# MoseleyBioinformaticsLab/pdb_eda

Measured on AMD Instinct MI355X. Metric: Mvoxels/s blob-labelled, higher is better.
Workload: dtype f32; 1 GPU; configs[1]: 256^3 synthetic CCP4 grid (gaussian-filtered noise, sigma_filter 1.5 voxels), fused green/red blob labelling at +-(mean+1.5*std), per-blob fp64 stats + dense int32 labels of both signs, map resident in HBM; labels=True, entries_per_rank=1

## Files before the change

### pdb_eda_amd/csrc/pdbeda_hip.hip

```cpp
#include <hip/hip_runtime.h>
#include <fcntl.h>
#include <sys/mman.h>
#include <sys/stat.h>
#include <unistd.h>
#include <cerrno>

#include <algorithm>
#include <chrono>
#include <thread>
#include <atomic>
#include <random>
#include <climits>
#include <cmath>
#include <cstdarg>
#include <cstdio>
#include <cstring>
#include <condition_variable>
#include <deque>
#include <map>
#include <mutex>
#include <string>
#include <vector>

#include "pdbeda_kernels.h"
// ... 808 lines not shown
    if (e != hipSuccess || why) {
        arena_put(ctx, m->arena);
        delete m;
        return why ? fail(ctx, PDBEDA_ERR_ARGUMENT, "reading %s: %s", path, why) : fail(ctx, PDBEDA_ERR_DEVICE, "map upload from file: %s", hipGetErrorString(e));
    }
    if (with_stats) {
        range_apply(m, range);
        if (mean) *mean = host[0];
        if (std) *std = host[1];
    }
    ctx->live_handles++;
    *out = m;
    return PDBEDA_OK;
}

extern "C" int pdbeda_map_upload_file(pdbeda_ctx *ctx, const char *path, int64_t offset, int byteswap, const pdbeda_geometry *geom, pdbeda_map **out) {
    return upload_file_impl(ctx, path, offset, byteswap, geom, out, nullptr, nullptr);
}
extern "C" int pdbeda_map_upload_file_stats(pdbeda_ctx *ctx, const char *path, int64_t offset, int byteswap, const pdbeda_geometry *geom, pdbeda_map **out,
                                            double *mean, double *std) {
    return upload_file_impl(ctx, path, offset, byteswap, geom, out, mean, std);
}

extern "C" int pdbeda_map_combine(pdbeda_map *a, pdbeda_map *b, double alpha, pdbeda_map **out) {
    if (!a || !b || !out) return PDBEDA_ERR_ARGUMENT;
    *out = nullptr;
    pdbeda_ctx *ctx = a->ctx;
    if (b->ctx != ctx) return fail(ctx, PDBEDA_ERR_ARGUMENT, "maps of different contexts");
    if (a->n_vox != b->n_vox || memcmp(a->geom.ncrs, b->geom.ncrs, sizeof a->geom.ncrs) != 0)
        return fail(ctx, PDBEDA_ERR_ARGUMENT, "maps of different shapes");
    HIP_TRY(ctx, hipSetDevice(ctx->device));
    pdbeda_map *m = new pdbeda_map();
    m->ctx = ctx;
    m->geom = a->geom;
    m->n_vox = a->n_vox;
    float *d = nullptr;
    int rc = arena_carve(ctx, "map combine", &m->arena, [&](Carver &cv) { cv.take(m->geom_dev, 1); cv.take(d, (size_t)m->n_vox); });
    if (rc) { delete m; return rc; }
    hipError_t e = h2d_one(ctx, m->geom_dev, &m->geom, sizeof(Geom));
    if (e == hipSuccess) {
        hipLaunchKernelGGL(k_map_combine, dim3(grid_for(m->n_vox / 4 + 1, 256, 4096)), dim3(256), 0, ctx->stream, a->dens, b->dens, alpha, m->n_vox, d);
        e = hipGetLastError();
    }
    if (e == hipSuccess) e = ctx_sync(ctx);
    if (e != hipSuccess) {
        arena_put(ctx, m->arena);
        delete m;
        return fail(ctx, PDBEDA_ERR_DEVICE, "map combine: %s", hipGetErrorString(e));
    }
    m->dens = d;
    m->own_dens = true;
    ctx->live_handles++;
    *out = m;
    return PDBEDA_OK;
}

extern "C" int pdbeda_map_download(pdbeda_map *m, float *density_out) {
    if (!m || !density_out) return PDBEDA_ERR_ARGUMENT;
    pdbeda_ctx *ctx = m->ctx;
    HIP_TRY(ctx, hipSetDevice(ctx->device));
    HIP_TRY(ctx, d2h(ctx, density_out, m->dens, sizeof(float) * (size_t)m->n_vox));
    HIP_TRY(ctx, ctx_sync(ctx));
    return PDBEDA_OK;
}

extern "C" int pdbeda_map_free(pdbeda_map *m) {
    if (!m) return PDBEDA_ERR_ARGUMENT;
    pdbeda_ctx *ctx = m->ctx;
    arena_put(ctx, m->arena);
    ctx->live_handles--;
    delete m;
    return PDBEDA_OK;
}

static int reduce_launch(pdbeda_map *m, int mode, const double *mean_dev, double cutoff, double scale, int take_sqrt, double *out_dev) {
    pdbeda_ctx *ctx = m->ctx;
    hipLaunchKernelGGL(k_reduce_partials, dim3(N_PARTIAL), dim3(256), 0, ctx->stream, m->dens, m->n_vox, mode, mean_dev, cutoff, ctx->partials);
    hipLaunchKernelGGL(k_reduce_final, dim3(1), dim3(256), 0, ctx->stream, ctx->partials, N_PARTIAL, scale, take_sqrt, out_dev);
    HIP_TRY(ctx, hipGetLastError());
    return 0;
}

static int range_enqueue(pdbeda_map *m, double *range_host ) {
    pdbeda_ctx *ctx = m->ctx;
    double *res = ctx->partials + 2 * N_PARTIAL + 4;
    { PROF(ctx, "k_range_partials"); hipLaunchKernelGGL(k_range_partials, dim3(N_PARTIAL), dim3(256), 0, ctx->stream, m->dens, m->n_vox, ctx->partials, ctx->partials + N_PARTIAL); }
    hipLaunchKernelGGL(k_range_final, dim3(1), dim3(256), 0, ctx->stream, ctx->partials, ctx->partials + N_PARTIAL, N_PARTIAL, res);
    HIP_TRY(ctx, hipGetLastError());
    if (range_host) HIP_TRY(ctx, d2h(ctx, range_host, res, 2 * sizeof(double)));
    return 0;
}
static void range_apply(pdbeda_map *m, const double range[2]) {
    if (!std::isfinite(range[0]) || !std::isfinite(range[1])) { m->fix_refused = true; return; }
    const double bound = std::max(range[0], 4194304.0 * range[1]);
    int S = 40;
    if (bound > 0.0 && std::isfinite(bound)) {
        int e = 0;
        (void)frexp(bound, &e);
        S = 61 - e;
    }
    S = std::max(-900, std::min(S, 900));
    m->fix_mul = ldexp(1.0, S);
}
static int map_fix_mul(pdbeda_map *m) {
    pdbeda_ctx *ctx = m->ctx;
    if (m->fix_mul == 0.0 && !m->fix_refused) {
        double range[2] = {0.0, 0.0};
        const int rc = range_enqueue(m, range);
        if (rc) return rc;
        HIP_TRY(ctx, ctx_sync(ctx));
        range_apply(m, range);
    }
    if (m->fix_refused) return fail(ctx, PDBEDA_ERR_ARGUMENT, "the map holds non-finite density values: blob sums are undefined");
    return 0;
}

extern "C" int pdbeda_map_invalidate(pdbeda_map *m) {
    if (!m) return PDBEDA_ERR_ARGUMENT;
    m->fix_mul = 0.0;
    m->fix_refused = false;
    return PDBEDA_OK;
}

static int stats_enqueue(pdbeda_map *m, double *chunk_sums, double host[2], double range[2], bool want_range, bool with_geom) {
    pdbeda_ctx *ctx = m->ctx;
    double *res = ctx->partials + 2 * N_PARTIAL;
    const int64_t n_full = m->n_vox / NP_CHUNK;
    const int64_t n_chunks = std::max<int64_t>(n_full, 1);
    hipStream_t st = ctx->stream;
    double *host_out = nullptr;
    if (want_range && copy_kernels()) host_out = reinterpret_cast<double *>(pinned_take(ctx, 6 * sizeof(double)));
    if (host_out) {
        pinned_deliver(ctx, (char *)host_out, host, 2 * sizeof(double));
        pinned_deliver(ctx, (char *)(host_out + 4), range, 2 * sizeof(double));
    }
    double *r_sum = want_range ? chunk_sums + n_chunks : nullptr, *r_max = want_range ? chunk_sums + 2 * n_chunks : nullptr;
    for (int mode = 0; mode < 2; ++mode) {
        const bool with_range = want_range && mode == 0;
        if (n_full > 0) { PROF(ctx, "k_np_chunk_sums"); hipLaunchKernelGGL(k_np_chunk_sums, dim3((unsigned)std::min<int64_t>(n_full, 1 << 16)), dim3(256), 0, st, m->dens, n_full, mode, res, chunk_sums,
                                                                           with_range ? r_sum : (double *)nullptr, with_range ? r_max : (double *)nullptr,
                                                                           m->geom, with_geom && mode == 0 ? m->geom_dev : (Geom *)nullptr); }
        { PROF(ctx, "k_np_final"); hipLaunchKernelGGL(k_np_final, dim3(1), dim3(256), 0, st, m->dens, m->n_vox, n_full, mode, res, chunk_sums, mode, res + mode,
                                                      with_range && n_full > 0 ? r_sum : (const double *)nullptr, with_range && n_full > 0 ? r_max : (const double *)nullptr,
                                                      with_range ? res + 4 : (double *)nullptr, want_range && mode == 1 ? res + 4 : (const double *)nullptr, mode == 1 ? host_out : (double *)nullptr); }
    }
    HIP_TRY(ctx, hipGetLastError());
    if (host_out) return 0;
    if (!want_range) {
        HIP_TRY(ctx, d2h(ctx, host, res, 2 * sizeof(double)));
        return 0;
    }
    if (char *stage = pinned_take(ctx, 6 * sizeof(double))) {
        HIP_TRY(ctx, stage_copy(ctx, stage, res, 6 * sizeof(double), false));
        pinned_deliver(ctx, stage, host, 2 * sizeof(double));
        pinned_deliver(ctx, stage + 4 * sizeof(double), range, 2 * sizeof(double));
        return 0;
    }
    HIP_TRY(ctx, d2h(ctx, host, res, 2 * sizeof(double)));
    HIP_TRY(ctx, d2h(ctx, range, res + 4, 2 * sizeof(double)));
    return 0;
}

extern "C" int pdbeda_map_stats(pdbeda_map *m, double *mean, double *std) {
    if (!m) return PDBEDA_ERR_ARGUMENT;
    pdbeda_ctx *ctx = m->ctx;
    HIP_TRY(ctx, hipSetDevice(ctx->device));
    const int64_t n_full = m->n_vox / NP_CHUNK;
    double host[2], range[2] = {0.0, 0.0};
    const bool want_range = m->fix_mul == 0.0 && !m->fix_refused;
    int rc = with_scratch(ctx, 24 * (size_t)std::max<int64_t>(n_full, 1), [&](char *base) -> int {
        return stats_enqueue(m, reinterpret_cast<double *>(base), host, range, want_range);
    });
    if (rc) return rc;
    if (want_range) range_apply(m, range);
    if (mean) *mean = host[0];
    if (std) *std = host[1];
    return PDBEDA_OK;
}

extern "C" int pdbeda_sum_of_abs(pdbeda_map *m, float cutoff, double *out) {
    if (!m || !out) return PDBEDA_ERR_ARGUMENT;
    pdbeda_ctx *ctx = m->ctx;
    HIP_TRY(ctx, hipSetDevice(ctx->device));
    double *res = ctx->partials + N_PARTIAL + 2;
    int rc = reduce_launch(m, 2, nullptr, (double)cutoff, 1.0, 0, res);
    if (rc) return rc;
    HIP_TRY(ctx, d2h(ctx, out, res, sizeof(double)));
    HIP_TRY(ctx, ctx_sync(ctx));
    return PDBEDA_OK;
}

extern "C" int pdbeda_abs_select_hist(pdbeda_map *a, pdbeda_map *b, double alpha, double cut_a, double cut_b, int which, int shift,
                                      unsigned long long prefix, unsigned long long prefix_mask, uint32_t *hist) {
    if (!a || !hist || shift < 0 || shift > 48 || (which != 0 && which != 1) || (which == 1 && !b)) return PDBEDA_ERR_ARGUMENT;
    pdbeda_ctx *ctx = a->ctx;
    if (b && (b->ctx != ctx || b->n_vox != a->n_vox || memcmp(a->geom.ncrs, b->geom.ncrs, sizeof a->geom.ncrs) != 0))
        return fail(ctx, PDBEDA_ERR_ARGUMENT, "maps of different contexts or shapes");
    HIP_TRY(ctx, hipSetDevice(ctx->device));
    const int64_t n = (int64_t)a->geom.unique_ncrs[0] * a->geom.unique_ncrs[1] * a->geom.unique_ncrs[2];
    return with_scratch(ctx, 65536 * sizeof(uint32_t), [&](char *base) -> int {
        unsigned int *d_hist = reinterpret_cast<unsigned int *>(base);
        HIP_TRY(ctx, hipMemsetAsync(d_hist, 0, 65536 * sizeof(uint32_t), ctx->stream));
        hipLaunchKernelGGL(k_abs_select_hist, dim3(grid_for(n, 256, 4096)), dim3(256), 0, ctx->stream, a->geom_dev, a->dens, b ? b->dens : nullptr,
                           alpha, cut_a, cut_b, which, shift, prefix, prefix_mask, d_hist);
        HIP_TRY(ctx, hipGetLastError());
        HIP_TRY(ctx, d2h(ctx, hist, d_hist, 65536 * sizeof(uint32_t)));
        return 0;
    });
}

extern "C" int pdbeda_point_density(pdbeda_map *m, const int32_t *crs, int64_t n, double *out) {
    if (!m || (n > 0 && (!crs || !out)) || n < 0) return PDBEDA_ERR_ARGUMENT;
    if (n == 0) return PDBEDA_OK;
    pdbeda_ctx *ctx = m->ctx;
    HIP_TRY(ctx, hipSetDevice(ctx->device));
    int32_t *d_crs = nullptr;
    double *d_out = nullptr;
    return with_scratch(ctx, "point density", [&](Carver &cv) { cv.take(d_crs, 3 * n); cv.take(d_out, n); }, [&]() -> int {
        const int32_t *in = pinned_in(ctx, crs, (size_t)(3 * n));
        if (!in) { HIP_TRY(ctx, h2d_one(ctx, d_crs, crs, (size_t)(12 * n))); in = d_crs; }
        double *res = pinned_out(ctx, out, (size_t)n);
        hipLaunchKernelGGL(k_point_density, dim3(grid_for(n, 256)), dim3(256), 0, ctx->stream, m->geom_dev, m->dens, in, n, res ? res : d_out, (uint8_t *)nullptr);
        if (!res) HIP_TRY(ctx, d2h(ctx, out, d_out, 8 * n));
        return 0;
    });
}

extern "C" int pdbeda_valid_crs(pdbeda_map *m, const int32_t *crs, int64_t n, uint8_t *out) {
    if (!m || (n > 0 && (!crs || !out)) || n < 0) return PDBEDA_ERR_ARGUMENT;
    if (n == 0) return PDBEDA_OK;
    pdbeda_ctx *ctx = m->ctx;
    HIP_TRY(ctx, hipSetDevice(ctx->device));
    int32_t *d_crs = nullptr;
    uint8_t *d_out = nullptr;
    return with_scratch(ctx, "valid crs", [&](Carver &cv) { cv.take(d_crs, 3 * n); cv.take(d_out, n); }, [&]() -> int {
        const int32_t *in = pinned_in(ctx, crs, (size_t)(3 * n));
        if (!in) { HIP_TRY(ctx, h2d_one(ctx, d_crs, crs, (size_t)(12 * n))); in = d_crs; }
        uint8_t *res = pinned_out(ctx, out, (size_t)n);
        hipLaunchKernelGGL(k_point_density, dim3(grid_for(n, 256)), dim3(256), 0, ctx->stream, m->geom_dev, m->dens, in, n, (double *)nullptr, res ? res : d_out);
        if (!res) HIP_TRY(ctx, d2h(ctx, out, d_out, n));
        return 0;
    });
}

extern "C" int pdbeda_crs2xyz(pdbeda_map *m, const int32_t *crs, int64_t n, double *xyz) {
    if (!m || (n > 0 && (!crs || !xyz)) || n < 0) return PDBEDA_ERR_ARGUMENT;
    if (n == 0) return PDBEDA_OK;
    pdbeda_ctx *ctx = m->ctx;
    HIP_TRY(ctx, hipSetDevice(ctx->device));
    int32_t *d_crs = nullptr;
    double *d_xyz = nullptr;
    return with_scratch(ctx, "crs2xyz", [&](Carver &cv) { cv.take(d_crs, 3 * n); cv.take(d_xyz, 3 * n); }, [&]() -> int {
        const int32_t *in = pinned_in(ctx, crs, (size_t)(3 * n));
        if (!in) { HIP_TRY(ctx, h2d_one(ctx, d_crs, crs, (size_t)(12 * n))); in = d_crs; }
        double *res = pinned_out(ctx, xyz, (size_t)(3 * n));
        hipLaunchKernelGGL(k_crs2xyz, dim3(grid_for(n, 256)), dim3(256), 0, ctx->stream, m->geom_dev, in, n, res ? res : d_xyz);
        if (!res) HIP_TRY(ctx, d2h(ctx, xyz, d_xyz, 24 * n));
        return 0;
    });
}

extern "C" int pdbeda_xyz2crs(pdbeda_map *m, const double *xyz, int64_t n, int32_t *crs) {
    if (!m || (n > 0 && (!crs || !xyz)) || n < 0) return PDBEDA_ERR_ARGUMENT;
    if (n == 0) return PDBEDA_OK;
    pdbeda_ctx *ctx = m->ctx;
    HIP_TRY(ctx, hipSetDevice(ctx->device));
    double *d_xyz = nullptr;
    int32_t *d_crs = nullptr;
    return with_scratch(ctx, "xyz2crs", [&](Carver &cv) { cv.take(d_xyz, 3 * n); cv.take(d_crs, 3 * n); }, [&]() -> int {
        const double *in = pinned_in(ctx, xyz, (size_t)(3 * n));
        if (!in) { HIP_TRY(ctx, h2d_one(ctx, d_xyz, xyz, (size_t)(24 * n))); in = d_xyz; }
        int32_t *res = pinned_out(ctx, crs, (size_t)(3 * n));
        hipLaunchKernelGGL(k_xyz2crs, dim3(grid_for(n, 256)), dim3(256), 0, ctx->stream, m->geom_dev, in, n, res ? res : d_crs);
        if (!res) HIP_TRY(ctx, d2h(ctx, crs, d_crs, 12 * n));
        return 0;
    });
}

static void job_carve(Job &job, Carver &cv, int n_vols, int64_t total_words, int64_t total_keys, int64_t max_runs,
                        int64_t max_blobs, size_t extra_labels, int32_t **labels_out, int64_t n_tiles = 0, int64_t max_comps = -1) {
    if (max_comps < 0) max_comps = max_runs;
    job.run_cap = (uint32_t)max_runs; job.comp_cap = (uint32_t)max_comps; job.blob_cap = (uint32_t)std::min<int64_t>(max_blobs, 0xffffffffll);
    job.n_vols = n_vols;
    job.total_words = total_words;
    job.key_words = (total_keys + 63) / 64;
    job.n_fine = (int32_t)((job.key_words + KEY_FINE - 1) / KEY_FINE);
    job.fine_shift = 4;
    while (((int64_t)KEY_GROUPS << job.fine_shift) < job.n_fine) job.fine_shift++;
    job.fine_per_group = 1 << job.fine_shift;
    job.n_groups = (job.n_fine + job.fine_per_group - 1) / job.fine_per_group;
    job.vols = cv.take<VolDesc>(std::max(n_vols, 1));
    job.ctr = cv.take<Counters>(1);
    job.mask = cv.take<uint64_t>(total_words);
    job.key_bits = cv.take<uint64_t>((size_t)(job.key_words + KEY_FINE - 1) / KEY_FINE * KEY_FINE);
    job.n_fine_alloc = (int32_t)((job.n_fine + job.fine_per_group - 1) / job.fine_per_group * job.fine_per_group);
    job.fine_count = cv.take<uint32_t>((size_t)std::max(job.n_fine_alloc / 2, 8));
    job.mid_count = cv.take<uint32_t>((size_t)(job.key_words + KEY_FINE - 1) / KEY_FINE * (KEY_FINE / 16));
    job.group_count = (n_tiles && job.fine_shift > 4) ? cv.take<uint32_t>(KEY_GROUPS) : nullptr;
    job.run_base = cv.take<uint32_t>(total_words);
    job.comps_are_runs = n_tiles ? 0 : 1;
    job.comp_of_run = n_tiles ? cv.take<uint32_t>(max_runs) : nullptr;
    job.label_of_comp = n_tiles ? cv.take<int32_t>(max_comps) : nullptr;
    job.word_comps = n_tiles ? cv.take<uint8_t>((size_t)n_tiles * 2 * 256 * 8) : nullptr;
    job.unit_done = n_tiles ? cv.take<uint32_t>((size_t)n_tiles) : nullptr;
    job.unit_flag = n_tiles ? cv.take<uint32_t>(4) : nullptr;
    job.tile_mode = n_tiles ? cv.take<uint8_t>(n_tiles) : nullptr;
    job.tile_runs = n_tiles ? cv.take<uint32_t>(n_tiles) : nullptr;
    job.root_mask = n_tiles ? cv.take<uint64_t>((size_t)n_tiles * 4) : nullptr;
    job.n_tiles = (int32_t)n_tiles;
    if (n_tiles) {
        const int64_t nt = n_tiles, nfc = job.n_fine_alloc / 2, nmid = (job.key_words + KEY_FINE - 1) / KEY_FINE * (KEY_FINE / 16);
        job.clear_bits = (int32_t)((job.key_words + nt - 1) / nt);
        job.clear_fine = (int32_t)((nfc + nt - 1) / nt);
        job.clear_mid = (int32_t)((nmid + nt - 1) / nt);
    }
    job.inbox = n_tiles ? cv.take<InboxEntry>((size_t)n_tiles * INBOX_CAP) : nullptr;
    job.inbox_count = n_tiles ? cv.take<uint32_t>((size_t)n_tiles * INBOX_STRIDE) : nullptr;
    job.vol_sign[0] = job.vol_sign[1] = 1;
    job.parent = cv.take<int32_t>(max_comps);
    job.kpar = n_tiles ? cv.take<unsigned long long>(max_comps) : nullptr;
    job.r_n = cv.take<uint32_t>(max_comps);
    job.r_sum = cv.take<long long>((size_t)7 * max_comps);
    job.r_sum_stride = max_comps;
    job.r_c = cv.take<long long>(max_comps);
    job.r_r = cv.take<long long>(max_comps);
    job.r_s = cv.take<long long>(max_comps);
    job.r_key = cv.take<unsigned long long>(max_comps);
    job.r_rank = cv.take<uint32_t>(max_comps);
    job.b_n = cv.take<int64_t>(max_blobs);
    job.b_key = cv.take<int64_t>(max_blobs);
    job.b_total = cv.take<double>(max_blobs);
    job.b_centroid = cv.take<double>(3 * max_blobs);
    job.b_center = cv.take<double>(3 * max_blobs);
    job.b_volume = cv.take<double>(max_blobs);
    job.b_group = cv.take<int32_t>(max_blobs);
    int32_t *lab = extra_labels ? cv.take<int32_t>(extra_labels) : nullptr;
    if (labels_out) *labels_out = lab;
}

static int engine_enqueue(pdbeda_ctx *ctx, pdbeda_map *m, Job &job, int64_t max_runs, bool labelled = false, bool unordered = false) {
    hipStream_t st = ctx->stream;
    const unsigned run_grid = grid_for(max_runs, 256, 2048);
    if (job.total_words > 0 && !labelled) {
        {
            PROF(ctx, "k_run_index");
            static const int force_wpb = [] { const char *e = getenv("PDBEDA_RUNINDEX_WPB"); return e ? atoi(e) : 0; }();
            if (force_wpb != 256 && (force_wpb == 64 || (job.total_words < 256ll * 2048 && job.total_words > 64ll * job.n_vols))) hipLaunchKernelGGL(k_run_index<64>, dim3(grid_for(job.total_words, 64, 1ll << 30)), dim3(256), 0, st, job, m->dens, m->geom_dev);
            else hipLaunchKernelGGL(k_run_index<256>, dim3(grid_for(job.total_words, 256, 1ll << 30)), dim3(256), 0, st, job, m->dens, m->geom_dev);
        }
        { PROF(ctx, "k_union"); hipLaunchKernelGGL(k_union, dim3(grid_for(job.total_words * 4, 256, 1ll << 30)), dim3(256), 0, st, job); }
        { PROF(ctx, "k_resolve"); hipLaunchKernelGGL(k_resolve, dim3(run_grid), dim3(256), 0, st, job, unordered ? 1 : 0); }
        if (!unordered) { PROF(ctx, "k_paint_keys"); hipLaunchKernelGGL(k_paint_keys, dim3(run_grid), dim3(256), 0, st, job); }
    }
    if (!unordered) { PROF(ctx, "k_emit"); hipLaunchKernelGGL(k_emit, dim3(job.total_words > 0 ? std::min(run_grid, 512u) : 1u), dim3(256), 0, st, job, m->geom_dev); }
    HIP_TRY(ctx, hipGetLastError());
    return 0;
}

static pdbeda_bloblist *new_list(pdbeda_ctx *ctx, pdbeda_map *m) {
    pdbeda_bloblist *bl = new pdbeda_bloblist();
    bl->ctx = ctx;
    bl->map = m;
    ctx->live_handles++;
    return bl;
}

template <int CW>
static void launch_tile_label(pdbeda_ctx *ctx, unsigned n_tiles, const Job &job, const float *dens, const Geom *geom_dev, const TileDims &td,
                              const JobInit &init, int pair_slots) {
    { PROF(ctx, "k_tile_label"); hipLaunchKernelGGL((k_tile_label<CW>), dim3(td.ctiles, td.rtiles, td.stiles), dim3(512), 0, ctx->stream, job, dens, geom_dev, td, init); }
    {
        PROF(ctx, "k_face_merge");
        if (td.ctiles > 1) hipLaunchKernelGGL((k_face_merge<CW, FM_THREADS_WIDE>), dim3(td.ctiles, td.rtiles, td.stiles), dim3(FM_THREADS_WIDE), 0, ctx->stream, job, dens, geom_dev, td, pair_slots);
        else hipLaunchKernelGGL((k_face_merge<CW, FM_THREADS>), dim3(td.ctiles, td.rtiles, td.stiles), dim3(FM_THREADS), 0, ctx->stream, job, dens, geom_dev, td, pair_slots);
    }
    if (job.unit_form) {
        { PROF(ctx, "k_unit_label"); hipLaunchKernelGGL((k_unit_label<CW>), dim3(td.ctiles, td.rtiles, td.stiles), dim3(512), 0, ctx->stream, job, dens, geom_dev, td); }
        { PROF(ctx, "k_unit_pairs"); hipLaunchKernelGGL((k_unit_pairs<CW>), dim3(td.ctiles, td.rtiles, td.stiles), dim3(512), 0, ctx->stream, job, td); }
    }
}

template <bool FUSED>
static void launch_labels(pdbeda_ctx *ctx, const Job &job, const TileDims &td, int32_t *labels_dev, const Geom *geom_dev) {
    switch (td.cw) {
        case 1: hipLaunchKernelGGL((k_labels_tiles<1, FUSED>), dim3(td.ctiles, td.rtiles, td.stiles), dim3(PDBEDA_LABELS_NT_THREADS), 0, ctx->stream, job, td, labels_dev, geom_dev); break;
        case 2: hipLaunchKernelGGL((k_labels_tiles<2, FUSED>), dim3(td.ctiles, td.rtiles, td.stiles), dim3(PDBEDA_LABELS_NT_THREADS), 0, ctx->stream, job, td, labels_dev, geom_dev); break;
        case 3: hipLaunchKernelGGL((k_labels_tiles<3, FUSED>), dim3(td.ctiles, td.rtiles, td.stiles), dim3(PDBEDA_LABELS_NT_THREADS), 0, ctx->stream, job, td, labels_dev, geom_dev); break;
        default: hipLaunchKernelGGL((k_labels_tiles<4, FUSED>), dim3(td.ctiles, td.rtiles, td.stiles), dim3(PDBEDA_LABELS_NT_THREADS), 0, ctx->stream, job, td, labels_dev, geom_dev); break;
    }
}

struct WholeMapJob {
    Job job;
    Arena arena;
    TileDims td;
    int32_t *labels_dev = nullptr;
    bool labels = false;
    size_t bytes = 0;
};
static int whole_map_enqueue(pdbeda_map *m, float cut_pos, float cut_neg, bool want_pos, bool want_neg, uint32_t flags, int tier, int unit_form, WholeMapJob *out) {
    pdbeda_ctx *ctx = m->ctx;
    HIP_TRY(ctx, hipSetDevice(ctx->device));
    const Geom &g = m->geom;
    const int n_planes = (want_pos ? 1 : 0) + (want_neg ? 1 : 0);
    const int uc = g.unique_ncrs[0], ur = g.unique_ncrs[1], us = g.unique_ncrs[2];
    const int row_words = (uc + 63) / 64;
    const int64_t words_pp = (int64_t)row_words * ur * us;
    const int64_t keys_pp = (int64_t)uc * ur * us;
    const int64_t total_words = words_pp * n_planes, total_keys = keys_pp * n_planes;
    const int64_t worst_blobs = (int64_t)((uc + 1) / 2) * ((ur + 1) / 2) * ((us + 1) / 2) * n_planes + 1;
    const bool labels = (flags & PDBEDA_FLAG_LABELS) != 0;
    const size_t lab_elems = labels ? (size_t)keys_pp : 0;

    TileDims td;
    td.ctiles = (row_words + 3) / 4;
    td.cw = (row_words + td.ctiles - 1) / td.ctiles;
    td.rtiles = (ur + TILE_R - 1) / TILE_R;
    td.stiles = (us + TILE_S - 1) / TILE_S;
    td.n_planes = n_planes;
    td.uc = uc; td.ur = ur; td.us = us; td.row_words = row_words;
    td.nc = g.ncrs[0]; td.nr = g.ncrs[1];
    td.cut[0] = want_pos ? cut_pos : cut_neg;
    td.sign[0] = want_pos ? 1 : -1;
    td.cut[1] = cut_neg;
    td.sign[1] = -1;
    const int64_t tiles_pp = (int64_t)td.ctiles * td.rtiles * td.stiles;
    if (tiles_pp >= (1ll << 31) || keys_pp >= (1ll << 31)) return fail(ctx, PDBEDA_ERR_ARGUMENT, "grid too large");
    if (td.rtiles > 65535 || td.stiles > 65535) return fail(ctx, PDBEDA_ERR_ARGUMENT, "grid too large");
    const int64_t tile_runs = tiles_pp * td.cw * 64 * 32, tile_comps = tiles_pp * CCAP;
    const int64_t worst_unit = (int64_t)((uc + 1) / 2) * ur * us * n_planes + 1;
    if (tile_runs + worst_unit >= (1ll << 31))
        return fail(ctx, PDBEDA_ERR_ARGUMENT, "grid too large for whole-map labelling: %d x %d x %d voxels need %lld run ids (limit 2^31: about 1100^3 for a fused job)",
                    uc, ur, us, (long long)(tile_runs + worst_unit));
    const int64_t unit_ids = tier == 0 ? std::min<int64_t>(worst_unit, std::max<int64_t>(65536, tile_runs / 4)) : worst_unit;
    const int64_t max_blobs = tier == 0 ? std::min<int64_t>(worst_blobs, std::max<int64_t>(4096, total_keys / 32)) : worst_blobs;
    const int64_t max_runs = tile_runs + unit_ids, max_comps = tile_comps + unit_ids;

    int rc_fix = map_fix_mul(m);
    if (rc_fix) return rc_fix;
    Job job;
    memset(&job, 0, sizeof job);
    job.fix_mul = m->fix_mul;
    size_t need = 0;
    Arena arena;
    int32_t *labels_dev = nullptr;
    int rc = arena_carve(ctx, "whole-map labelling", &arena, [&](Carver &cv) {
        job_carve(job, cv, n_planes, total_words, total_keys, max_runs, max_blobs, lab_elems, &labels_dev, tiles_pp, max_comps);
        need = cv.off;
    });
    if (rc) return rc;
    job.vol_sign[0] = td.sign[0];
    job.vol_sign[1] = td.sign[1];
    job.unit_form = unit_form;
    static std::atomic<uint32_t> g_epoch{[] {
        uint32_t seed;
        try { seed = (uint32_t)std::random_device{}(); }
        catch (...) { seed = (uint32_t)std::chrono::steady_clock::now().time_since_epoch().count() ^ ((uint32_t)getpid() * 2654435761u); }
        return seed | 1u;
    }()};
    do { job.epoch = g_epoch.fetch_add(1u); } while (job.epoch == 0u || job.epoch == 0xffffffffu);

    JobInit init;
    memset(&init, 0, sizeof init);
    for (int p = 0; p < n_planes; ++p) {
        VolDesc &v = init.v[p];
        v.dim[0] = uc; v.dim[1] = ur; v.dim[2] = us;
        v.org[0] = v.org[1] = v.org[2] = 0;
        v.row_words = row_words;
        v.group = p;
        v.word_base = words_pp * p;
        v.key_base = keys_pp * p;
    }
    init.runs0 = (unsigned)tile_runs;
    init.comps0 = (unsigned)tile_comps;
    hipStream_t st = ctx->stream;
    int pair_slots = PAIR_SLOTS;
    if (ctx->debug_edge_cap > 0) { pair_slots = 1; while (pair_slots * 2 <= std::min<int64_t>(ctx->debug_edge_cap, PAIR_SLOTS)) pair_slots *= 2; }
    switch (td.cw) {
        case 1: launch_tile_label<1>(ctx, (unsigned)tiles_pp, job, m->dens, m->geom_dev, td, init, pair_slots); break;
        case 2: launch_tile_label<2>(ctx, (unsigned)tiles_pp, job, m->dens, m->geom_dev, td, init, pair_slots); break;
        case 3: launch_tile_label<3>(ctx, (unsigned)tiles_pp, job, m->dens, m->geom_dev, td, init, pair_slots); break;
        default: launch_tile_label<4>(ctx, (unsigned)tiles_pp, job, m->dens, m->geom_dev, td, init, pair_slots); break;
    }
    { PROF(ctx, "k_resolve_tiles"); hipLaunchKernelGGL(k_resolve_tiles, dim3((unsigned)tiles_pp + 64u), dim3(256), 0, st, job, (int)tiles_pp); }
    if (job.group_count) { PROF(ctx, "k_group_counts"); hipLaunchKernelGGL(k_group_counts, dim3((unsigned)(job.n_groups + 255) / 256u), dim3(256), 0, st, job); }
    if (labels) {
        PROF(ctx, "k_labels_tiles");
        launch_labels<true>(ctx, job, td, labels_dev, m->geom_dev);
    } else {
        PROF(ctx, "k_emit_tiles");
        hipLaunchKernelGGL(k_emit_tiles, dim3(std::min<unsigned>(512u, ((unsigned)tiles_pp + 1u) / 2u)), dim3(256), 0, st, job, m->geom_dev);
    }
    hipError_t e = hipGetLastError();
    if (e != hipSuccess) { arena_put(ctx, arena); return fail(ctx, PDBEDA_ERR_DEVICE, "whole-map labelling launch: %s", hipGetErrorString(e)); }
    out->job = job; out->arena = arena; out->td = td; out->labels_dev = labels_dev; out->labels = labels; out->bytes = need;
    return PDBEDA_OK;
}

static int full_blobs_impl(pdbeda_map *m, float cut_pos, float cut_neg, bool want_pos, bool want_neg, uint32_t flags,
                           pdbeda_bloblist **out_pos, pdbeda_bloblist **out_neg) {
    pdbeda_ctx *ctx = m->ctx;
    WholeMapJob wj;
    const int tier = ctx->debug_worst_case_arena ? 1 : 0, form = tier;
    int rc = whole_map_enqueue(m, cut_pos, cut_neg, want_pos, want_neg, flags, tier, form, &wj);
    if (rc) return rc;
    const int n_planes = (want_pos ? 1 : 0) + (want_neg ? 1 : 0);
    pdbeda_bloblist *first = nullptr;
    for (int p = 0; p < n_planes; ++p) {
        pdbeda_bloblist *bl = new_list(ctx, m);
        bl->job = wj.job;
        bl->td = wj.td;
        bl->vol_lo = p;
        bl->vol_hi = p + 1;
        bl->whole_map = true;
        bl->sign = wj.td.sign[p];
        if (p == 0) { bl->arena = wj.arena; bl->owns_arena = true; first = bl; }
        else { bl->owns_arena = false; bl->sibling = first; first->sibling = bl; }
        bl->labels_dev = wj.labels_dev;
        bl->labels_done = wj.labels;
        bl->cut_pos = cut_pos; bl->cut_neg = cut_neg; bl->want_pos = want_pos; bl->want_neg = want_neg; bl->flags = flags; bl->tier = tier; bl->unit_form = form;
        bl->job_bytes = wj.bytes;
        if (bl->sign > 0) *out_pos = bl; else *out_neg = bl;
    }
    return PDBEDA_OK;
}

extern "C" int pdbeda_full_blobs(pdbeda_map *m, float cutoff, uint32_t flags, pdbeda_bloblist **out) {
    if (!m || !out) return PDBEDA_ERR_ARGUMENT;
    *out = nullptr;
    if (cutoff == 0.0f || cutoff != cutoff) return fail(m->ctx, PDBEDA_ERR_ARGUMENT, "cutoff must be non-zero (the reference returns None)");
    pdbeda_bloblist *dummy = nullptr;
    if (cutoff > 0) return full_blobs_impl(m, cutoff, 0.0f, true, false, flags, out, &dummy);
    return full_blobs_impl(m, 0.0f, cutoff, false, true, flags, &dummy, out);
}

extern "C" int pdbeda_full_blobs_pm(pdbeda_map *m, float cutoff_pos, float cutoff_neg, uint32_t flags, pdbeda_bloblist **green,
                                    pdbeda_bloblist **red) {
    if (!m || !green || !red) return PDBEDA_ERR_ARGUMENT;
    *green = *red = nullptr;
    if (!(cutoff_pos > 0.0f) || !(cutoff_neg < 0.0f)) return fail(m->ctx, PDBEDA_ERR_ARGUMENT, "need cutoff_pos > 0 > cutoff_neg");
    return full_blobs_impl(m, cutoff_pos, cutoff_neg, true, true, flags, green, red);
}

static pdbeda_bloblist *owner_of(pdbeda_bloblist *bl) { return bl->owns_arena ? bl : bl->sibling; }
static const int64_t SPEC_ROWS = 2048;
static int list_resolve_counts(pdbeda_bloblist *bl) {
    if (bl->have_counts) return 0;
    pdbeda_ctx *ctx = bl->ctx;
    HIP_TRY(ctx, hipSetDevice(ctx->device));
    Counters ctr;
    auto fetch = [&]() -> int {
        pdbeda_bloblist *ow = bl->whole_map ? owner_of(bl) : nullptr;
        const int64_t g = ow ? std::min<int64_t>((int64_t)bl->job.blob_cap, SPEC_ROWS) : 0;
        if (g > 0) {
            const Job &job = bl->job;
            ow->spec_rows = 0;
            ow->spec_n.resize((size_t)g); ow->spec_key.resize((size_t)g); ow->spec_total.resize((size_t)g); ow->spec_centroid.resize(3 * (size_t)g);
            ow->spec_center.resize(3 * (size_t)g); ow->spec_volume.resize((size_t)g); ow->spec_group.resize((size_t)g);
            const D2HItem parts[8] = {{&ctr, job.ctr, sizeof ctr}, {ow->spec_n.data(), job.b_n, (size_t)(8 * g)}, {ow->spec_total.data(), job.b_total, (size_t)(8 * g)},
                                      {ow->spec_centroid.data(), job.b_centroid, (size_t)(24 * g)}, {ow->spec_center.data(), job.b_center, (size_t)(24 * g)},
                                      {ow->spec_volume.data(), job.b_volume, (size_t)(8 * g)}, {ow->spec_key.data(), job.b_key, (size_t)(8 * g)},
                                      {ow->spec_group.data(), job.b_group, (size_t)(4 * g)}};
            HIP_TRY(ctx, d2h_many(ctx, parts, 8));
            HIP_TRY(ctx, ctx_sync(ctx));
            ow->spec_rows = g;
            return 0;
        }
        HIP_TRY(ctx, d2h(ctx, &ctr, bl->job.ctr, sizeof ctr));
        HIP_TRY(ctx, ctx_sync(ctx));
        return 0;
    };
    {
        const int rc_fetch = fetch();
        if (rc_fetch) return rc_fetch;
    }
    while (bl->whole_map && ctr.overflow != 0u) {
        pdbeda_bloblist *ow = owner_of(bl);
        if (!ow) return fail(ctx, PDBEDA_ERR_STATE, "whole-map labelling: a list without its job");
        const int tier = 1, form = 1;
        if (tier == ow->tier && form == ow->unit_form) return fail(ctx, PDBEDA_ERR_STATE, "whole-map labelling overflowed its worst-case arena");
        if (ow->voxels_done || bl->voxels_done) return fail(ctx, PDBEDA_ERR_STATE, "whole-map labelling: overflow noticed after the voxel lists were made");
        WholeMapJob wj;
        arena_put(ctx, ow->arena);
        int rc = whole_map_enqueue(ow->map, ow->cut_pos, ow->cut_neg, ow->want_pos, ow->want_neg, ow->flags, tier, form, &wj);
        if (rc) { ow->arena.base = nullptr; ow->arena.cap = 0; return rc; }
        ow->arena = wj.arena;
        pdbeda_bloblist *both[2] = {ow, ow->sibling};
        for (pdbeda_bloblist *l : both) {
            if (!l) continue;
            l->job = wj.job; l->td = wj.td; l->labels_dev = wj.labels_dev; l->labels_done = wj.labels;
            l->tier = tier; l->unit_form = form; l->reruns += 1; l->have_counts = false; l->job_bytes = wj.bytes; l->spec_rows = 0;
        }
        const int rc_fetch = fetch();
        if (rc_fetch) return rc_fetch;
    }
    if (!bl->whole_map && ctr.unit_wait_failed) return fail(ctx, PDBEDA_ERR_DEVICE, "sphere batch: the device's volumes outgrew what the host sized the job for");
    if (bl->vol_lo == 0 && bl->vol_hi == bl->job.n_vols) { bl->rank_lo = 0; bl->rank_hi = ctr.n_blobs; }
    else if (bl->whole_map && bl->job.n_vols == 2 && bl->vol_hi == bl->vol_lo + 1) {
        bl->rank_lo = bl->vol_lo == 0 ? 0 : ctr.n_blobs_vol0;
        bl->rank_hi = bl->vol_lo == 0 ? ctr.n_blobs_vol0 : ctr.n_blobs;
    } else return fail(ctx, PDBEDA_ERR_STATE, "blob list covers an unexpected volume range");
    bl->job_blobs = ctr.n_blobs;
    bl->have_counts = true;
    if (bl->whole_map && bl->job.n_vols == 2) {
        pdbeda_bloblist *ow = owner_of(bl);
        pdbeda_bloblist *both[2] = {ow, ow ? ow->sibling : nullptr};
        for (pdbeda_bloblist *l : both) {
            if (!l || l == bl || l->freed || l->have_counts || l->job.ctr != bl->job.ctr || l->vol_hi != l->vol_lo + 1) continue;
            l->rank_lo = l->vol_lo == 0 ? 0 : ctr.n_blobs_vol0;
            l->rank_hi = l->vol_lo == 0 ? ctr.n_blobs_vol0 : ctr.n_blobs;
            l->job_blobs = ctr.n_blobs;
            l->have_counts = true;
        }
    }
    return 0;
}

extern "C" int pdbeda_bloblist_counters(pdbeda_bloblist *bl, int64_t *out) {
    if (!bl || bl->freed || !out) return PDBEDA_ERR_ARGUMENT;
    pdbeda_ctx *ctx = bl->ctx;
    HIP_TRY(ctx, hipSetDevice(ctx->device));
    Counters c;
    HIP_TRY(ctx, d2h(ctx, &c, bl->job.ctr, sizeof c));
    HIP_TRY(ctx, ctx_sync(ctx));
    out[0] = c.n_runs; out[1] = c.n_comps; out[2] = bl->reruns; out[3] = c.n_blobs;
    out[4] = out[5] = out[6] = 0;
    out[7] = (int64_t)(bl->job_bytes ? bl->job_bytes : owner_of(bl)->arena.cap);
    if (bl->whole_map && bl->job.tile_mode) {
        const int64_t n_tiles = (int64_t)bl->td.ctiles * bl->td.rtiles * bl->td.stiles;
        std::vector<uint8_t> mode(n_tiles);
        HIP_TRY(ctx, d2h(ctx, mode.data(), bl->job.tile_mode, n_tiles));
        HIP_TRY(ctx, ctx_sync(ctx));
        for (uint8_t v : mode) { if (v == 1) ++out[4]; else if (v == 2) ++out[5]; else if (v == 3) ++out[6]; }
    }
    return PDBEDA_OK;
}


extern "C" int64_t pdbeda_bloblist_count(pdbeda_bloblist *bl) {
    if (!bl || bl->freed) return PDBEDA_ERR_ARGUMENT;
    int rc = list_resolve_counts(bl);
    if (rc) return rc;
    return bl->rank_hi - bl->rank_lo;
}

extern "C" int pdbeda_bloblist_stats(pdbeda_bloblist *bl, int64_t *n, double *total_density, double *centroid, double *coord_center,
                                     double *volume, int64_t *first_key, int32_t *group) {
    if (!bl || bl->freed) return PDBEDA_ERR_ARGUMENT;
    int rc = list_resolve_counts(bl);
    if (rc) return rc;
    pdbeda_ctx *ctx = bl->ctx;
    const Job &job = bl->job;
    const int64_t lo = bl->rank_lo, cnt = bl->rank_hi - bl->rank_lo;
    if (cnt == 0) return PDBEDA_OK;
    if (bl->whole_map) {
        const pdbeda_bloblist *ow = owner_of(bl);
        if (ow && ow->spec_rows >= lo + cnt && ow->job.ctr == job.ctr) {
            if (n) memcpy(n, ow->spec_n.data() + lo, (size_t)(8 * cnt));
            if (total_density) memcpy(total_density, ow->spec_total.data() + lo, (size_t)(8 * cnt));
            if (centroid) memcpy(centroid, ow->spec_centroid.data() + 3 * lo, (size_t)(24 * cnt));
            if (coord_center) memcpy(coord_center, ow->spec_center.data() + 3 * lo, (size_t)(24 * cnt));
            if (volume) memcpy(volume, ow->spec_volume.data() + lo, (size_t)(8 * cnt));
            if (first_key) memcpy(first_key, ow->spec_key.data() + lo, (size_t)(8 * cnt));
            if (group) memcpy(group, ow->spec_group.data() + lo, (size_t)(4 * cnt));
            return PDBEDA_OK;
        }
    }
    const D2HItem columns[7] = {{n, job.b_n + lo, (size_t)(8 * cnt)}, {total_density, job.b_total + lo, (size_t)(8 * cnt)},
                                {centroid, job.b_centroid + 3 * lo, (size_t)(24 * cnt)}, {coord_center, job.b_center + 3 * lo, (size_t)(24 * cnt)},
                                {volume, job.b_volume + lo, (size_t)(8 * cnt)}, {first_key, job.b_key + lo, (size_t)(8 * cnt)},
                                {group, job.b_group + lo, (size_t)(4 * cnt)}};
    HIP_TRY(ctx, d2h_many(ctx, columns, 7));
    HIP_TRY(ctx, ctx_sync(ctx));
    return PDBEDA_OK;
}

static int list_stats_one_trip(pdbeda_bloblist *bl, int64_t guess, std::vector<int64_t> &n, std::vector<double> &tot, std::vector<double> &cen,
                               std::vector<int32_t> &grp, const D2HItem *extra = nullptr) {
    pdbeda_ctx *ctx = bl->ctx;
    const Job &job = bl->job;
    guess = std::min<int64_t>(guess, (int64_t)job.blob_cap);
    const bool whole_job = !bl->whole_map && bl->vol_lo == 0 && bl->vol_hi == job.n_vols;
    const int64_t extra_bytes = extra ? (int64_t)extra->bytes + 64 : 0;
    if (!bl->have_counts && whole_job && guess > 0 && 44 * guess + 4096 + extra_bytes < (int64_t)pinned_room(ctx)) {
        HIP_TRY(ctx, hipSetDevice(ctx->device));
        n.resize((size_t)guess); tot.resize((size_t)guess); cen.resize(3 * (size_t)guess); grp.resize((size_t)guess);
        Counters ctr;
        const D2HItem parts[6] = {{&ctr, job.ctr, sizeof ctr}, {n.data(), job.b_n, (size_t)(8 * guess)}, {tot.data(), job.b_total, (size_t)(8 * guess)},
                                  {cen.data(), job.b_centroid, (size_t)(24 * guess)}, {grp.data(), job.b_group, (size_t)(4 * guess)},
                                  extra ? *extra : D2HItem{nullptr, nullptr, 0}};
        HIP_TRY(ctx, d2h_many(ctx, parts, 6));
        HIP_TRY(ctx, ctx_sync(ctx));
        if (ctr.unit_wait_failed) return fail(ctx, PDBEDA_ERR_DEVICE, "sphere batch: the device's volumes outgrew what the host sized the job for");
        bl->rank_lo = 0; bl->rank_hi = ctr.n_blobs; bl->job_blobs = ctr.n_blobs; bl->have_counts = true;
        if ((int64_t)ctr.n_blobs <= guess) {
            const size_t nb = ctr.n_blobs;
            n.resize(nb); tot.resize(nb); cen.resize(3 * nb); grp.resize(nb);
            return PDBEDA_OK;
        }
        extra = nullptr;
    }
    if (extra && extra->dst && extra->bytes) HIP_TRY(ctx, d2h(ctx, extra->dst, extra->src, extra->bytes));
    const int64_t nb = pdbeda_bloblist_count(bl);
    if (nb < 0) return (int)nb;
    n.resize((size_t)nb); tot.resize((size_t)nb); cen.resize(3 * (size_t)nb); grp.resize((size_t)nb);
    return pdbeda_bloblist_stats(bl, n.data(), tot.data(), cen.data(), nullptr, nullptr, nullptr, grp.data());
}


static int list_materialise_voxels(pdbeda_bloblist *bl) {
    pdbeda_bloblist *ow = owner_of(bl);
    if (ow->voxels_done) return 0;
    pdbeda_ctx *ctx = bl->ctx;
    HIP_TRY(ctx, hipSetDevice(ctx->device));
    {
        const int rc_counts = list_resolve_counts(bl);
        if (rc_counts) return rc_counts;
        ow = owner_of(bl);
    }
    Job &job = ow->job;
    const int64_t nb = bl->job_blobs;
    const int64_t max_vox = job.key_words * 64;
    int rc = arena_carve(ctx, "voxel lists", &ow->vox_arena, [&](Carver &cv) {
        cv.take(ow->offsets_dev, nb + 1);
        cv.take(ow->cursor_dev, std::max<int64_t>(nb, 1));
        cv.take(ow->crs_dev, 3 * std::max<int64_t>(max_vox, 1));
    });
    if (rc) return rc;
    hipStream_t st = ctx->stream;
    hipLaunchKernelGGL(k_blob_offsets, dim3(1), dim3(1024), 0, st, job, ow->offsets_dev, ow->cursor_dev);
    if (job.total_words > 0)
        hipLaunchKernelGGL(k_voxel_lists, dim3(grid_for(job.total_words * 64, 256, 8192)), dim3(256), 0, st, job, ow->offsets_dev,
                           ow->cursor_dev, ow->crs_dev);
    HIP_TRY(ctx, hipGetLastError());
    ow->voxels_done = true;
    return 0;
}

extern "C" int64_t pdbeda_bloblist_num_voxels(pdbeda_bloblist *bl) {
    if (!bl || bl->freed) return PDBEDA_ERR_ARGUMENT;
    int rc = list_resolve_counts(bl);
    if (rc) return rc;
    if (bl->n_voxels >= 0) return bl->n_voxels;
    rc = list_materialise_voxels(bl);
    if (rc) return rc;
    pdbeda_ctx *ctx = bl->ctx;
    pdbeda_bloblist *ow = owner_of(bl);
    int64_t off[2] = {0, 0};
    HIP_TRY(ctx, d2h(ctx, &off[0], ow->offsets_dev + bl->rank_lo, 8));
    HIP_TRY(ctx, d2h(ctx, &off[1], ow->offsets_dev + bl->rank_hi, 8));
    HIP_TRY(ctx, ctx_sync(ctx));
    bl->n_voxels = off[1] - off[0];
    return bl->n_voxels;
}

extern "C" int pdbeda_bloblist_voxels(pdbeda_bloblist *bl, int32_t *crs, int64_t *blob_offsets) {
    if (!bl || bl->freed) return PDBEDA_ERR_ARGUMENT;
    int64_t nv = pdbeda_bloblist_num_voxels(bl);
    if (nv < 0) return (int)nv;
    pdbeda_ctx *ctx = bl->ctx;
    pdbeda_bloblist *ow = owner_of(bl);
    const int64_t cnt = bl->rank_hi - bl->rank_lo;
    std::vector<int64_t> off(cnt + 1);
    HIP_TRY(ctx, d2h(ctx, off.data(), ow->offsets_dev + bl->rank_lo, 8 * (cnt + 1))); HIP_TRY(ctx, ctx_sync(ctx));
    const int64_t base = off[0];
    if (blob_offsets)
        for (int64_t i = 0; i <= cnt; ++i) blob_offsets[i] = off[i] - base;
    if (crs && nv > 0) HIP_TRY(ctx, d2h(ctx, crs, ow->crs_dev + 3 * base, 12 * nv)); HIP_TRY(ctx, ctx_sync(ctx));
    return PDBEDA_OK;
}

static int list_moments_compute(pdbeda_bloblist *bl) {
    const int64_t nv = pdbeda_bloblist_num_voxels(bl);
    if (nv < 0) return (int)nv;
    pdbeda_ctx *ctx = bl->ctx;
    const int64_t cnt = bl->rank_hi - bl->rank_lo;
    if (cnt == 0 || nv == 0) { bl->shape_done = true; return PDBEDA_OK; }
    if (cnt >= (1ll << 31) || nv >= (1ll << 31)) return fail(ctx, PDBEDA_ERR_ARGUMENT, "blob moments: a list of 2^31 blobs or voxels, or more");
    if (!bl->whole_map && nv >= (1ll << 24)) return fail(ctx, PDBEDA_ERR_ARGUMENT, "blob moments: a sphere / list batch of 2^24 voxels or more");
    pdbeda_map *m = bl->map;
    HIP_TRY(ctx, hipSetDevice(ctx->device));
    if (int rc = map_fix_mul(m)) return rc;
    pdbeda_bloblist *ow = owner_of(bl);
    const size_t nb = (size_t)cnt;
    BlobShapeArgs a;
    unsigned long long *d_widest = nullptr;
    int32_t *d_i = nullptr;
    long long *d_l = nullptr;
// ... 1826 lines not shown
```

### pdb_eda_amd/csrc/pdbeda_kernels.h

```cpp
#pragma once
#include "pdbeda_device.h"

namespace pdbeda {

struct VolDesc {
    int32_t dim[3];
    int32_t org[3];
    int32_t row_words;
    int32_t group;
    int64_t word_base;
    int64_t key_base;
};

struct FixSums {
    long long rho, c_lo, c_hi, r_lo, r_hi, s_lo, s_hi;
};
__device__ inline long long fix_of(double v, double mul) { return __double2ll_rn(v * mul); }
__device__ inline void fix_limbs(__int128 v, long long &lo, long long &hi) {
    lo = (long long)(unsigned long long)((unsigned __int128)v & 0xffffffffu);
    hi = (long long)(v >> 32);
}
__device__ inline double fix_moment(long long lo, long long hi) { return (double)hi * 4294967296.0 + (double)lo; }
__device__ inline FixSums fix_sums(long long F, long long m_c, long long m_r, long long m_s, long long c0, long long r0, long long s0) {
    FixSums o;
    o.rho = F;
    fix_limbs((__int128)F * c0 + m_c, o.c_lo, o.c_hi);
    fix_limbs((__int128)F * r0 + m_r, o.r_lo, o.r_hi);
    fix_limbs((__int128)F * s0 + m_s, o.s_lo, o.s_hi);
    return o;
}
__device__ inline void fix_add(FixSums &a, const FixSums &b) {
    a.rho += b.rho; a.c_lo += b.c_lo; a.c_hi += b.c_hi; a.r_lo += b.r_lo; a.r_hi += b.r_hi; a.s_lo += b.s_lo; a.s_hi += b.s_hi;
}
__device__ inline void fix_atomic_add(FixSums *dst, const FixSums &v) {
    atomicAdd((unsigned long long *)&dst->rho, (unsigned long long)v.rho);
    atomicAdd((unsigned long long *)&dst->c_lo, (unsigned long long)v.c_lo);
    atomicAdd((unsigned long long *)&dst->c_hi, (unsigned long long)v.c_hi);
    atomicAdd((unsigned long long *)&dst->r_lo, (unsigned long long)v.r_lo);
    atomicAdd((unsigned long long *)&dst->r_hi, (unsigned long long)v.r_hi);
    atomicAdd((unsigned long long *)&dst->s_lo, (unsigned long long)v.s_lo);
    atomicAdd((unsigned long long *)&dst->s_hi, (unsigned long long)v.s_hi);
}
template <typename JobRef> __device__ inline FixSums fix_load(const JobRef &job, uint32_t i) {
    const long long *p = job.r_sum + i;
    const int64_t s = job.r_sum_stride;
    FixSums o;
    o.rho = p[0]; o.c_lo = p[s]; o.c_hi = p[2 * s]; o.r_lo = p[3 * s]; o.r_hi = p[4 * s]; o.s_lo = p[5 * s]; o.s_hi = p[6 * s];
    return o;
}
template <typename JobRef> __device__ inline void fix_store(const JobRef &job, uint32_t i, const FixSums &v) {
    long long *p = job.r_sum + i;
    const int64_t s = job.r_sum_stride;
    p[0] = v.rho; p[s] = v.c_lo; p[2 * s] = v.c_hi; p[3 * s] = v.r_lo; p[4 * s] = v.r_hi; p[5 * s] = v.s_lo; p[6 * s] = v.s_hi;
}
template <typename JobRef> __device__ inline void fix_fold(const JobRef &job, uint32_t i, const FixSums &v) {
    unsigned long long *p = (unsigned long long *)(job.r_sum + i);
    const int64_t s = job.r_sum_stride;
    atomicAdd(p, (unsigned long long)v.rho);
    atomicAdd(p + s, (unsigned long long)v.c_lo); atomicAdd(p + 2 * s, (unsigned long long)v.c_hi);
    atomicAdd(p + 3 * s, (unsigned long long)v.r_lo); atomicAdd(p + 4 * s, (unsigned long long)v.r_hi);
    atomicAdd(p + 5 * s, (unsigned long long)v.s_lo); atomicAdd(p + 6 * s, (unsigned long long)v.s_hi);
}
__device__ inline FixSums fix_zero() { FixSums z; z.rho = z.c_lo = z.c_hi = z.r_lo = z.r_hi = z.s_lo = z.s_hi = 0; return z; }

struct Counters {
    unsigned int n_runs;
    unsigned int n_comps;
    unsigned int n_blobs;
    unsigned int n_blobs_vol0;
    unsigned int unit_wait_failed;
    unsigned int unit_tiles[3];
    unsigned int overflow;
    unsigned long long n_voxels;
    long long total_words;
    long long total_keys;
};

struct Job {
    VolDesc *vols;
    int32_t n_vols;
    int64_t total_words;
    int64_t key_words;
    uint64_t *mask;
    uint32_t *run_base;
    uint64_t *key_bits;
    uint32_t *fine_count;
    int32_t n_fine, n_fine_alloc, fine_per_group;
    Counters *ctr;
    int32_t comps_are_runs;
    uint32_t *comp_of_run;
    int32_t *label_of_comp;
    uint8_t *word_comps;
    uint32_t *unit_done;
    uint32_t *unit_flag;
    uint32_t epoch;
    uint8_t *tile_mode;
    uint32_t *tile_runs;
    struct InboxEntry *inbox;
    uint32_t *inbox_count;
    int32_t vol_sign[2];
    int32_t *parent;
    uint32_t *r_n;
    long long *r_sum;
    int64_t r_sum_stride;
    double fix_mul;
    long long *r_c, *r_r, *r_s;
    unsigned long long *r_key;
    uint32_t *r_rank;
    int64_t *b_n, *b_key;
    double *b_total, *b_centroid, *b_center, *b_volume;
    int32_t *b_group;
    uint64_t *root_mask;
    int32_t n_tiles;
    unsigned long long *kpar;
    uint32_t *mid_count;
    int32_t fine_shift, n_groups;
    uint32_t run_cap, comp_cap, blob_cap;
    int32_t clear_bits, clear_fine, clear_mid;
    uint32_t *group_count;
    int32_t unit_form;
};

struct InboxEntry {
    uint32_t local, n;
    FixSums sum;
    unsigned long long c, r, s;
};
constexpr int INBOX_STRIDE = 32;
constexpr int INBOX_CAP = 192;

constexpr int TILE_COMPS = 256;
constexpr int KEY_FINE = 32;
constexpr int KEY_GROUPS = 1024;
constexpr int WAVE = 64;

__device__ inline int lane_id() { return threadIdx.x & 63; }

__device__ inline int find_vol(const VolDesc *vols, int n, int64_t word) {
    int lo = 0, hi = n - 1;
    while (lo < hi) {
        int mid = (lo + hi + 1) >> 1;
        if (vols[mid].word_base <= word) lo = mid; else hi = mid - 1;
    }
    return lo;
}
__device__ inline int find_vol_by_key(const VolDesc *vols, int n, int64_t key) {
    int lo = 0, hi = n - 1;
    while (lo < hi) {
        int mid = (lo + hi + 1) >> 1;
        if (vols[mid].key_base <= key) lo = mid; else hi = mid - 1;
    }
    return lo;
}


__device__ inline double wave_incl_scan(double x, int lane) {
#pragma unroll
    for (int d = 1; d < 64; d <<= 1) {
        double y = __shfl_up(x, d);
        if (lane >= d) x += y;
    }
    return x;
}

template <typename JobRef>
__device__ inline void word_run_records_of(const JobRef &job, const VolDesc &vd, uint64_t mw, int lane, double rho, int cl0, int rl, int sl,
                                           int rawc0, int rawr, int raws, uint32_t rec0);
template <typename JobRef>
__device__ inline void word_run_records(const JobRef &job, const Geom &g, const float *__restrict__ dens, const VolDesc &vd, uint64_t mw,
                                        int lane, int cl0, int rl, int sl, int rawc0, int rawr, int raws, uint32_t rec0) {
    const bool bit = (mw >> lane) & 1ull;
    const double rho = bit ? (double)fetch_wrapped(g, dens, rawc0 + lane, rawr, raws) : 0.0;
    word_run_records_of(job, vd, mw, lane, rho, cl0, rl, sl, rawc0, rawr, raws, rec0);
}
template <typename JobRef>
__device__ inline void word_run_records_of(const JobRef &job, const VolDesc &vd, uint64_t mw, int lane, double rho, int cl0, int rl, int sl,
                                           int rawc0, int rawr, int raws, uint32_t rec0) {
    const double rl_ = rho * (double)lane;
    const double p1 = wave_incl_scan(rho, lane);
    const double p2 = wave_incl_scan(rl_, lane);
    const uint64_t starts = run_starts(mw);
    const bool is_start = (starts >> lane) & 1ull;
    const int e = is_start ? run_end_of(mw, lane) : lane;
    const double p1e = __shfl(p1, e);
    const double p2e = __shfl(p2, e);
    if (is_start) {
        const int len = e - lane + 1;
        const double s_rho = p1e - (p1 - rho);
        const double s_rl = p2e - (p2 - rl_);
        const uint32_t idx = rec0 + (uint32_t)popc64(starts & bits_below(lane));
        job.parent[idx] = (int32_t)idx;
        job.r_n[idx] = (uint32_t)len;
        fix_store(job, idx, fix_sums(fix_of(s_rho, job.fix_mul), fix_of(s_rl, job.fix_mul), 0, 0, rawc0, rawr, raws));
        const long long a = (long long)rawc0 + lane;
        job.r_c[idx] = (long long)len * a + (long long)len * (len - 1) / 2;
        job.r_r[idx] = (long long)len * rawr;
        job.r_s[idx] = (long long)len * raws;
        const int64_t key_in = ((int64_t)(cl0 + lane) * vd.dim[1] + rl) * vd.dim[2] + sl;
        job.r_key[idx] = (unsigned long long)(vd.key_base + key_in);
        if (job.kpar) job.kpar[idx] = ((unsigned long long)(((uint32_t)vd.group << 31) | (uint32_t)key_in) << 32) | idx;
    }
}

constexpr int NARROW_ROW = 16;
template <typename JobRef>
__device__ inline void narrow_run_records(const JobRef &job, const Geom &g, const float *__restrict__ dens, const VolDesc &vd, uint64_t mw,
                                          int rl, int sl, uint32_t rec0) {
    const int rawc0 = vd.org[0], rawr = vd.org[1] + rl, raws = vd.org[2] + sl;
    float v[NARROW_ROW];
#pragma unroll
    for (int k = 0; k < NARROW_ROW; ++k) v[k] = ((mw >> k) & 1ull) ? fetch_wrapped(g, dens, rawc0 + k, rawr, raws) : 0.0f;
    uint64_t todo = run_starts(mw);
    uint32_t idx = rec0;
    while (todo) {
        const int a = ctz64(todo);
        todo &= todo - 1;
        const int b = run_end_of(mw, a), len = b - a + 1;
        double s_rho = 0.0, s_rl = 0.0;
#pragma unroll
        for (int k = 0; k < NARROW_ROW; ++k)
            if (k >= a && k <= b) { s_rho += (double)v[k]; s_rl += (double)v[k] * (double)k; }
        job.parent[idx] = (int32_t)idx;
        job.r_n[idx] = (uint32_t)len;
        fix_store(job, idx, fix_sums(fix_of(s_rho, job.fix_mul), fix_of(s_rl, job.fix_mul), 0, 0, rawc0, rawr, raws));
        const long long first = (long long)rawc0 + a;
        job.r_c[idx] = (long long)len * first + (long long)len * (len - 1) / 2;
        job.r_r[idx] = (long long)len * rawr;
        job.r_s[idx] = (long long)len * raws;
        const int64_t key_in = ((int64_t)a * vd.dim[1] + rl) * vd.dim[2] + sl;
        job.r_key[idx] = (unsigned long long)(vd.key_base + key_in);
        if (job.kpar) job.kpar[idx] = ((unsigned long long)(((uint32_t)vd.group << 31) | (uint32_t)key_in) << 32) | idx;
        ++idx;
    }
}

constexpr int SPARSE_BITS = 16;
template <typename JobRef>
__device__ inline void sparse_run_records(const JobRef &job, const Geom &g, const float *__restrict__ dens, const VolDesc &vd, uint64_t mw,
                                          int wq, int rl, int sl, uint32_t rec0) {
    const int rawc0 = vd.org[0] + wq * 64, rawr = vd.org[1] + rl, raws = vd.org[2] + sl;
    float v[SPARSE_BITS];
    int pos[SPARSE_BITS];
    {
        uint64_t t = mw;
#pragma unroll
        for (int k = 0; k < SPARSE_BITS; ++k) {
            const bool have = t != 0ull;
            pos[k] = have ? ctz64(t) : 64;
            v[k] = have ? fetch_wrapped(g, dens, rawc0 + pos[k], rawr, raws) : 0.0f;
            t &= t - 1ull;
        }
    }
    uint32_t idx = rec0;
    int first = -1, prev = -2;
    double s_rho = 0.0, s_rl = 0.0;
    auto flush = [&]() {
        const int len = prev - first + 1;
        job.parent[idx] = (int32_t)idx;
        job.r_n[idx] = (uint32_t)len;
        fix_store(job, idx, fix_sums(fix_of(s_rho, job.fix_mul), fix_of(s_rl, job.fix_mul), 0, 0, rawc0, rawr, raws));
        const long long a0 = (long long)rawc0 + first;
        job.r_c[idx] = (long long)len * a0 + (long long)len * (len - 1) / 2;
        job.r_r[idx] = (long long)len * rawr;
        job.r_s[idx] = (long long)len * raws;
        const int64_t key_in = ((int64_t)(wq * 64 + first) * vd.dim[1] + rl) * vd.dim[2] + sl;
        job.r_key[idx] = (unsigned long long)(vd.key_base + key_in);
        if (job.kpar) job.kpar[idx] = ((unsigned long long)(((uint32_t)vd.group << 31) | (uint32_t)key_in) << 32) | idx;
        ++idx;
    };
#pragma unroll
    for (int k = 0; k < SPARSE_BITS; ++k) {
        if (pos[k] < 64) {
            if (pos[k] != prev + 1) {
                if (first >= 0) flush();
                first = pos[k]; s_rho = 0.0; s_rl = 0.0;
            }
            s_rho += (double)v[k];
            s_rl += (double)v[k] * (double)pos[k];
            prev = pos[k];
        }
    }
    if (first >= 0) flush();
}

template <int WPB>
__global__ void __launch_bounds__(256) k_run_index(Job job, const float *__restrict__ dens, const Geom *__restrict__ gp) {
    static_assert(WPB == 256 || WPB == 64, "a word per thread of the block, or of its first wave");
    constexpr int SCAN_WAVES = WPB / 64, PER_WAVE = WPB / 4;
    __shared__ uint64_t s_mask[WPB];
    __shared__ uint32_t s_off[WPB];
    __shared__ VolDesc s_vd[WPB];
    __shared__ int s_row[WPB][3];
    __shared__ uint32_t s_wsum[4];
    __shared__ uint32_t s_base;
    const int tid = threadIdx.x, lane = tid & 63, wv = tid >> 6;
    const int64_t chunk0 = (int64_t)blockIdx.x * WPB;
    const int64_t w = chunk0 + tid;
    const bool mine = tid < WPB && w < job.total_words;
    const uint64_t m = mine ? job.mask[w] : 0ull;
    const uint32_t cnt = (uint32_t)popc64(run_starts(m));
    uint32_t x = cnt;
#pragma unroll
    for (int d = 1; d < 64; d <<= 1) {
        uint32_t y = __shfl_up(x, d);
        if (lane >= d) x += y;
    }
    if (lane == 63) s_wsum[wv] = x;
    if (tid < WPB) s_mask[tid] = m;
    __syncthreads();
    if (tid == 0) {
        uint32_t tot = 0;
        for (int k = 0; k < SCAN_WAVES; ++k) tot += s_wsum[k];
        s_base = tot ? atomicAdd(&job.ctr->n_runs, tot) : 0u;
    }
    __syncthreads();
    uint32_t wpre = 0;
    for (int k = 0; k < wv && k < SCAN_WAVES; ++k) wpre += s_wsum[k];
    const uint32_t off = s_base + wpre + x - cnt;
    if (mine) job.run_base[w] = off;
    VolDesc my_vd;
    int wq = 0, rl = 0, sl = 0;
    bool narrow = false, sparse = false;
    if (m != 0ull) {
        my_vd = job.vols[find_vol(job.vols, job.n_vols, w)];
        const int64_t rem = w - my_vd.word_base;
        wq = (int)(rem % my_vd.row_words);
        const int64_t row = rem / my_vd.row_words;
        rl = (int)(row % my_vd.dim[1]);
        sl = (int)(row / my_vd.dim[1]);
        narrow = my_vd.dim[0] <= NARROW_ROW;
        sparse = !narrow && popc64(m) <= SPARSE_BITS;
        if (narrow || sparse) s_mask[tid] = 0ull;
        else { s_off[tid] = off; s_vd[tid] = my_vd; s_row[tid][0] = wq; s_row[tid][1] = rl; s_row[tid][2] = sl; }
    }
    __syncthreads();

    const Geom &g = *gp;
    if (narrow) narrow_run_records(job, g, dens, my_vd, m, rl, sl, off);
    else if (sparse) sparse_run_records(job, g, dens, my_vd, m, wq, rl, sl, off);
    uint64_t todo = 0ull;
    {
        const bool live = lane < PER_WAVE && s_mask[wv * PER_WAVE + lane] != 0ull;
        todo = __ballot(live);
    }
    auto fetch = [&](int slot) -> double {
        const uint64_t mw = s_mask[slot];
        const VolDesc &vd = s_vd[slot];
        return ((mw >> lane) & 1ull) ? (double)fetch_wrapped(g, dens, vd.org[0] + s_row[slot][0] * 64 + lane, vd.org[1] + s_row[slot][1], vd.org[2] + s_row[slot][2]) : 0.0;
    };
    double rho_next = todo ? fetch(wv * PER_WAVE + ctz64(todo)) : 0.0;
    while (todo) {
        const int slot = wv * PER_WAVE + ctz64(todo);
        todo &= todo - 1;
        const double rho = rho_next;
        if (todo) rho_next = fetch(wv * PER_WAVE + ctz64(todo));
        const VolDesc &vd = s_vd[slot];
        const int q = s_row[slot][0], r = s_row[slot][1], t = s_row[slot][2];
        word_run_records_of(job, vd, s_mask[slot], lane, rho, q * 64, r, t, vd.org[0] + q * 64, vd.org[1] + r, vd.org[2] + t, s_off[slot]);
    }
}

__device__ inline int uf_load(const int32_t *p, int x) {
    return __hip_atomic_load(p + x, __ATOMIC_RELAXED, __HIP_MEMORY_SCOPE_WORKGROUP);
}
__device__ inline int uf_find(int32_t *p, int x) {
    int q;
    while ((q = uf_load(p, x)) != x) {
        const int gp = uf_load(p, q);
        if (gp != q) atomicMin(p + x, gp);
        x = gp;
    }
    return x;
}
__device__ inline void uf_unite2(int32_t *p, int a, int b) {
    while (true) {
        int qa = uf_load(p, a), qb = uf_load(p, b);
        while (qa != a || qb != b) {
            const int ga = qa != a ? uf_load(p, qa) : qa, gb = qb != b ? uf_load(p, qb) : qb;
            if (qa != a && ga != qa) atomicMin(p + a, ga);
            if (qb != b && gb != qb) atomicMin(p + b, gb);
            a = ga; b = gb;
            qa = uf_load(p, a); qb = uf_load(p, b);
        }
        if (a == b) return;
        if (a < b) { const int t = a; a = b; b = t; }
        const int old = atomicMin(p + a, b);
        if (old == a) return;
        a = old;
    }
}

__device__ inline void uf_hook(int32_t *p, int a, int b) {
#pragma unroll
    for (int level = 0; level < 4; ++level) {
        if (a == b) return;
        if (a < b) { const int t = a; a = b; b = t; }
        const int old = atomicMin(p + a, b);
        if (old == a || old == b) return;
        a = old;
    }
    uf_unite2(p, a, b);
}

__device__ inline void uf_unite(int32_t *p, int a, int b) {
    while (true) {
        a = uf_find(p, a);
        b = uf_find(p, b);
        if (a == b) return;
        if (a < b) { int t = a; a = b; b = t; }
        int old = atomicMin(p + a, b);
        if (old == a) return;
        a = old;
    }
}

typedef unsigned long long kp_t;
constexpr kp_t KP_UNUSED = ~0ull;
__device__ __forceinline__ uint32_t kp_id(kp_t v) { return (uint32_t)v; }
__device__ inline kp_t kuf_load(const kp_t *p, uint32_t id) {
    return __hip_atomic_load(p + id, __ATOMIC_RELAXED, __HIP_MEMORY_SCOPE_WORKGROUP);
}
__device__ inline kp_t kuf_find_from(kp_t *p, kp_t x) {
    kp_t q;
    while ((q = kuf_load(p, kp_id(x))) != x) {
        const kp_t gp = kuf_load(p, kp_id(q));
        if (gp != q) atomicMin(p + kp_id(x), gp);
        x = gp;
    }
    return x;
}
__device__ inline void kuf_unite_vals(kp_t *p, kp_t a, kp_t b) {
    while (true) {
        kp_t qa = kuf_load(p, kp_id(a)), qb = kuf_load(p, kp_id(b));
        while (qa != a || qb != b) {
            const kp_t ga = qa != a ? kuf_load(p, kp_id(qa)) : qa, gb = qb != b ? kuf_load(p, kp_id(qb)) : qb;
            if (qa != a && ga != qa) atomicMin(p + kp_id(a), ga);
            if (qb != b && gb != qb) atomicMin(p + kp_id(b), gb);
            a = ga; b = gb;
            qa = kuf_load(p, kp_id(a)); qb = kuf_load(p, kp_id(b));
        }
        if (a == b) return;
        if (a < b) { const kp_t t = a; a = b; b = t; }
        const kp_t old = atomicMin(p + kp_id(a), b);
        if (old == a) return;
        a = old;
    }
}
__device__ inline void kuf_hook_vals(kp_t *p, kp_t a, kp_t b) {
#pragma unroll
    for (int level = 0; level < 4; ++level) {
        if (a == b) return;
        if (a < b) { const kp_t t = a; a = b; b = t; }
        const kp_t old = atomicMin(p + kp_id(a), b);
        if (old == a || old == b) return;
        a = old;
    }
    kuf_unite_vals(p, a, b);
}
__device__ inline void kuf_unite(kp_t *p, uint32_t ia, uint32_t ib) {
    kuf_unite_vals(p, kuf_load(p, ia), kuf_load(p, ib));
}

__device__ inline uint32_t run_of_bit(uint64_t nm, uint32_t base, int p, int *start_out) {
    int st = run_start_of(nm, p);
    *start_out = st;
    return base + (uint32_t)popc64(run_starts(nm) & bits_below(st));
}

__global__ void __launch_bounds__(256) k_union(Job job) {
    const int64_t t = (int64_t)blockIdx.x * blockDim.x + threadIdx.x;
    const int64_t w = t >> 2;
    const int nb = (int)(t & 3);
    if (w >= job.total_words) return;
    const uint64_t m = job.mask[w];
    if (m == 0ull) return;
    const VolDesc vd = job.vols[find_vol(job.vols, job.n_vols, w)];
    const int64_t rem = w - vd.word_base;
    const int wq = (int)(rem % vd.row_words);
    const int64_t row = rem / vd.row_words;
    const int rl = (int)(row % vd.dim[1]);
    const int sl = (int)(row / vd.dim[1]);
    uint64_t nmask[3];
    uint32_t nbase[3];
    {
        const int dr = nb == 3 ? 1 : (nb == 2 ? 0 : -1), ds = nb == 0 ? 0 : -1;
        const int r2 = rl + dr, s2 = sl + ds;
        const bool row_ok = r2 >= 0 && r2 < vd.dim[1] && s2 >= 0;
        const int64_t rowbase = vd.word_base + ((int64_t)(row_ok ? s2 : sl) * vd.dim[1] + (row_ok ? r2 : rl)) * vd.row_words;
#pragma unroll
        for (int d = 0; d < 3; ++d) {
            const int w2 = wq + d - 1;
            const bool ok = row_ok && w2 >= 0 && w2 < vd.row_words;
            const int64_t at = ok ? rowbase + w2 : w;
            const uint64_t v = job.mask[at];
            nbase[d] = job.run_base[at];
            nmask[d] = ok ? v : 0ull;
        }
    }
    const bool with_prev = nb == 0 && wq > 0;
    const uint64_t pm = with_prev ? job.mask[w - 1] : 0ull;
    const uint32_t pbase = job.run_base[with_prev ? w - 1 : w];
    const uint32_t base = job.run_base[w];
    if (!(nmask[0] | nmask[1] | nmask[2] | (pm >> 63))) return;
    uint64_t todo = run_starts(m);
    uint32_t k = 0;
    while (todo) {
        const int a = ctz64(todo);
        todo &= todo - 1;
        const int b = run_end_of(m, a);
        const int me = (int)(base + k);
        ++k;
        if (a == 0 && (pm >> 63)) {
            int st;
            uf_unite2(job.parent, me, (int)run_of_bit(pm, pbase, 63, &st));
        }
#pragma unroll
        for (int d = 0; d < 3; ++d) {
            const uint64_t nm = nmask[d];
            int lo = a - 1 - 64 * (d - 1), hi = b + 1 - 64 * (d - 1);
            if (nm == 0ull || hi < 0 || lo > 63) continue;
            if (lo < 0) lo = 0;
            if (hi > 63) hi = 63;
            uint64_t hit = nm & (bits_below(hi + 1) & ~bits_below(lo));
            while (hit) {
                const int p = ctz64(hit);
                int st;
                const uint32_t other = run_of_bit(nm, nbase[d], p, &st);
                uf_unite2(job.parent, me, (int)other);
                hit &= ~bits_below(run_end_of(nm, st) + 1);
            }
        }
    }
}

template <typename JobRef>
__device__ inline uint32_t n_components(const JobRef &job) { return job.comps_are_runs ? job.ctr->n_runs : job.ctr->n_comps; }

__device__ inline void resolve_wave(const Job &job, uint32_t i, bool valid, int lane, bool slots = false) {
    int root = -1;
    bool is_root = false;
    if (valid) {
        root = uf_find(job.parent, (int)i);
        if (root == (int)i) { root = -1; is_root = true; } else job.parent[i] = root;
    }
    if (slots) {
        const unsigned long long roots = __ballot(is_root);
        if (roots) {
            uint32_t first = 0;
            if (lane == ctz64(roots)) first = atomicAdd(&job.ctr->n_blobs, (uint32_t)popc64(roots));
            first = __shfl(first, ctz64(roots));
            if (is_root) job.r_rank[i] = first + (uint32_t)popc64(roots & bits_below(lane));
        }
    }
    uint32_t n = 0;
    FixSums sum = fix_zero();
    unsigned long long c = 0, r = 0, sv = 0, key = ~0ull;
    if (root >= 0) {
        n = job.r_n[i]; sum = fix_load(job, i);
        c = (unsigned long long)job.r_c[i]; r = (unsigned long long)job.r_r[i]; sv = (unsigned long long)job.r_s[i]; key = job.r_key[i];
    }
    unsigned long long todo = __ballot(root >= 0);
    while (todo) {
        const int first = ctz64(todo);
        const int r0 = __shfl(root, first);
        const bool mine = root == r0;
        const unsigned long long group = __ballot(mine);
        todo &= ~group;
        uint32_t gn = mine ? n : 0u;
        FixSums g_sum = mine ? sum : fix_zero();
        unsigned long long g_c = mine ? c : 0ull, g_r = mine ? r : 0ull, g_s = mine ? sv : 0ull, g_key = mine ? key : ~0ull;
        if (group & (group - 1)) {
#pragma unroll
            for (int d = 32; d > 0; d >>= 1) {
                gn += __shfl_xor(gn, d);
                g_sum.rho += __shfl_xor(g_sum.rho, d);
                g_sum.c_lo += __shfl_xor(g_sum.c_lo, d); g_sum.c_hi += __shfl_xor(g_sum.c_hi, d);
                g_sum.r_lo += __shfl_xor(g_sum.r_lo, d); g_sum.r_hi += __shfl_xor(g_sum.r_hi, d);
                g_sum.s_lo += __shfl_xor(g_sum.s_lo, d); g_sum.s_hi += __shfl_xor(g_sum.s_hi, d);
                g_c += __shfl_xor(g_c, d); g_r += __shfl_xor(g_r, d); g_s += __shfl_xor(g_s, d);
                const unsigned long long k2 = __shfl_xor(g_key, d);
                g_key = k2 < g_key ? k2 : g_key;
            }
        }
        if (lane == first) {
            atomicAdd(&job.r_n[r0], gn);
            fix_fold(job, (uint32_t)r0, g_sum);
            atomicAdd((unsigned long long *)&job.r_c[r0], g_c);
            atomicAdd((unsigned long long *)&job.r_r[r0], g_r);
            atomicAdd((unsigned long long *)&job.r_s[r0], g_s);
            atomicMin(&job.r_key[r0], g_key);
        }
    }
}
__global__ void __launch_bounds__(256) k_resolve(Job job, int slots) {
    const uint32_t n_runs = n_components(job);
    const int lane = lane_id();
    const uint32_t stride = gridDim.x * blockDim.x;
    for (uint32_t i0 = blockIdx.x * blockDim.x + (threadIdx.x & ~63u); i0 < n_runs; i0 += stride)
        resolve_wave(job, i0 + (uint32_t)lane, i0 + (uint32_t)lane < n_runs, lane, slots != 0);
}

template <typename JobRef>
__device__ __forceinline__ void paint_key(const JobRef &job, unsigned long long key) {
    const uint32_t f = (uint32_t)((key >> 6) / KEY_FINE);
    const uint32_t cell = (uint32_t)(key >> 8);
    atomicOr((unsigned long long *)&job.key_bits[key >> 6], 1ull << (key & 63));
    atomicAdd(&job.mid_count[cell >> 2], 1u << ((cell & 3u) * 8u));
    atomicAdd(&job.fine_count[f >> 1], 1u << ((f & 1u) * 16u));
}

__global__ void __launch_bounds__(256) k_paint_keys(Job job) {
    const uint32_t n_runs = n_components(job);
    for (uint32_t i = blockIdx.x * blockDim.x + threadIdx.x; i < n_runs; i += gridDim.x * blockDim.x) {
        const int32_t par = job.parent[i];
        const uint32_t cnt = job.r_n[i];
        const unsigned long long key = job.r_key[i];
        if (par != (int32_t)i || cnt == 0u) continue;
        paint_key(job, key);
    }
}

template <int CTRL, int ROW_MASK = 0xf>
__device__ __forceinline__ uint32_t dpp0(uint32_t x) {
    return (uint32_t)__builtin_amdgcn_update_dpp(0, (int)x, CTRL, ROW_MASK, 0xf, true);
}
constexpr int DPP_ROW_SHR = 0x110, DPP_WAVE_SHR1 = 0x138, DPP_ROW_BCAST15 = 0x142, DPP_ROW_BCAST31 = 0x143;
__device__ __forceinline__ uint32_t half_scan(uint32_t x) {
    x += dpp0<DPP_ROW_SHR + 1>(x);
    x += dpp0<DPP_ROW_SHR + 2>(x);
    x += dpp0<DPP_ROW_SHR + 4>(x);
    x += dpp0<DPP_ROW_SHR + 8>(x);
    x += dpp0<DPP_ROW_BCAST15, 0xa>(x);
    return x;
}

__device__ __forceinline__ uint32_t wave_scan(uint32_t x) {
    x = half_scan(x);
    x += dpp0<DPP_ROW_BCAST31, 0xc>(x);
    return x;
}
__device__ __forceinline__ uint32_t sum_u16x8(const uint4 q) {
    const uint32_t a = (q.x & 0xffffu) + (q.x >> 16), b = (q.y & 0xffffu) + (q.y >> 16), c = (q.z & 0xffffu) + (q.z >> 16), d = (q.w & 0xffffu) + (q.w >> 16);
    return (a + b) + (c + d);
}
__device__ __forceinline__ uint32_t sum_u16_first(const uint4 q, int take) {
    const uint32_t w[4] = {q.x, q.y, q.z, q.w};
    uint32_t acc = 0;
#pragma unroll
    for (int k = 0; k < 4; ++k) acc += (2 * k < take ? (w[k] & 0xffffu) : 0u) + (2 * k + 1 < take ? (w[k] >> 16) : 0u);
    return acc;
}

template <int NT>
struct RankTableLoads {
    static constexpr int PER = KEY_GROUPS / NT;
    uint4 q[2 * PER];
    uint32_t v[PER];
    bool summed;
};
template <int NT = 256, typename JobRef = Job>
__device__ __forceinline__ void rank_table_issue(const JobRef &job, RankTableLoads<NT> &ld) {
    constexpr int PER = KEY_GROUPS / NT;
    const int tid = threadIdx.x;
    const int G = job.fine_per_group, n_groups = job.n_groups, Q = G / 8;
    const uint4 *fine4 = reinterpret_cast<const uint4 *>(job.fine_count);
    ld.summed = Q != 2;
    if (Q == 2) {
#pragma unroll
        for (int k = 0; k < PER; ++k) {
            const int e = tid * PER + k;
            ld.q[2 * k] = e < n_groups ? fine4[(size_t)e * 2] : make_uint4(0, 0, 0, 0);
            ld.q[2 * k + 1] = e < n_groups ? fine4[(size_t)e * 2 + 1] : make_uint4(0, 0, 0, 0);
        }
    } else if (job.group_count) {
        const uint32_t *gc = job.group_count;
#pragma unroll
        for (int k = 0; k < PER; ++k) {
            const int e = tid * PER + k;
            ld.v[k] = e < n_groups ? gc[e] : 0u;
        }
    } else {
#pragma unroll
        for (int k = 0; k < PER; ++k) {
            const int e = tid * PER + k;
            uint32_t acc = 0;
            if (e < n_groups)
                for (int j = 0; j < Q; ++j) acc += sum_u16x8(fine4[(size_t)e * Q + j]);
            ld.v[k] = acc;
        }
    }
}
template <int NT = 256>
__device__ __forceinline__ uint32_t rank_table_finish(RankTableLoads<NT> &ld, uint32_t *s_pre , uint32_t *s_wave ) {
    constexpr int PER = KEY_GROUPS / NT;
    const int tid = threadIdx.x, lane = tid & 63, wv = tid >> 6;
    if (!ld.summed) {
#pragma unroll
        for (int k = 0; k < PER; ++k) ld.v[k] = sum_u16x8(ld.q[2 * k]) + sum_u16x8(ld.q[2 * k + 1]);
    }
    uint32_t mine = 0;
#pragma unroll
    for (int k = 0; k < PER; ++k) mine += ld.v[k];
    const uint32_t x = wave_scan(mine);
    if (lane == 63) s_wave[wv] = x;
    __syncthreads();
    uint32_t pre = x - mine, total = 0;
#pragma unroll
    for (int k = 0; k < NT / 64; ++k) { const uint32_t w = s_wave[k]; pre += k < wv ? w : 0u; total += w; }
#pragma unroll
    for (int k = 0; k < PER; ++k) { s_pre[tid * PER + k] = pre; pre += ld.v[k]; }
    __syncthreads();
    return total;
}
template <int NT = 256, typename JobRef = Job>
__device__ inline uint32_t rank_table_lds(const JobRef &job, uint32_t *s_pre , uint32_t *s_wave ) {
    RankTableLoads<NT> ld;
    rank_table_issue<NT>(job, ld);
    return rank_table_finish<NT>(ld, s_pre, s_wave);
}

__global__ void __launch_bounds__(256) k_group_counts(Job job) {
    const int e = (int)(blockIdx.x * blockDim.x + threadIdx.x);
    if (e >= job.n_groups) return;
    const int Q = job.fine_per_group / 8;
    const uint4 *fine4 = reinterpret_cast<const uint4 *>(job.fine_count) + (size_t)e * Q;
    uint32_t acc = 0;
    for (int j = 0; j < Q; j += 4) {
        const uint4 a = fine4[j], b = fine4[j + 1], c = fine4[j + 2], d = fine4[j + 3];
        acc += (sum_u16x8(a) + sum_u16x8(b)) + (sum_u16x8(c) + sum_u16x8(d));
    }
    job.group_count[e] = acc;
}

struct RankLoads {
    uint4 q0, q1;
    uint2 mid;
    ulonglong2 b0, b1;
};
template <typename JobRef>
__device__ __forceinline__ void rank_issue(const JobRef &job, unsigned long long key, RankLoads &ld) {
    const uint32_t kw = (uint32_t)(key >> 6), f = kw / (uint32_t)KEY_FINE, e = f >> 4;
    const uint4 *fine4 = reinterpret_cast<const uint4 *>(job.fine_count) + (size_t)e * 2;
    ld.q0 = fine4[0]; ld.q1 = fine4[1];
    ld.mid = reinterpret_cast<const uint2 *>(job.mid_count)[f];
    const ulonglong2 *bits2 = reinterpret_cast<const ulonglong2 *>(job.key_bits + (kw & ~3u));
    ld.b0 = bits2[0]; ld.b1 = bits2[1];
}
__device__ __forceinline__ uint32_t rank_finish(const uint32_t *s_pre, unsigned long long key, const RankLoads &ld) {
    const uint32_t kw = (uint32_t)(key >> 6), f = kw / (uint32_t)KEY_FINE, e = f >> 4;
    const int nf = (int)(f & 15u), cell = (int)((kw & (uint32_t)(KEY_FINE - 1)) >> 2), wi = (int)(kw & 3u);
    uint32_t rank = s_pre[e] + sum_u16_first(ld.q0, nf) + sum_u16_first(ld.q1, nf - 8);
    const uint32_t lo = cell >= 4 ? ld.mid.x : (ld.mid.x & ((1u << (8 * cell)) - 1u));
    const uint32_t hi = cell > 4 ? (ld.mid.y & ((1u << (8 * (cell - 4))) - 1u)) : 0u;
    rank += __builtin_amdgcn_sad_u8(lo, 0u, 0u) + __builtin_amdgcn_sad_u8(hi, 0u, 0u);
    const uint64_t below = bits_below((int)(key & 63));
    const uint64_t w[4] = {ld.b0.x, ld.b0.y, ld.b1.x, ld.b1.y};
#pragma unroll
    for (int k = 0; k < 4; ++k) rank += (uint32_t)popc64(k < wi ? w[k] : (k == wi ? w[k] & below : 0ull));
    return rank;
}
template <typename JobRef>
__device__ inline uint32_t rank_of_key(const JobRef &job, const uint32_t *s_pre, unsigned long long key) {
    const int shift = job.fine_shift;
    if (shift == 4) {
        RankLoads ld;
        rank_issue(job, key, ld);
        return rank_finish(s_pre, key, ld);
    }
    const uint32_t kw = (uint32_t)(key >> 6), f = kw / (uint32_t)KEY_FINE, e = f >> shift;
    const int Q = 1 << (shift - 3);
    uint32_t rank = s_pre[e];
    const uint4 *fine4 = reinterpret_cast<const uint4 *>(job.fine_count) + (size_t)e * Q;
    const int nf = (int)(f - (e << shift));
    const uint2 mid = reinterpret_cast<const uint2 *>(job.mid_count)[f];
    const ulonglong2 *bits2 = reinterpret_cast<const ulonglong2 *>(job.key_bits + (kw & ~3u));
    const int cell = (int)((kw & (uint32_t)(KEY_FINE - 1)) >> 2);
    const int wi = (int)(kw & 3u);
    const ulonglong2 b0 = bits2[0], b1 = bits2[1];
    for (int k = 0; k * 8 < nf; ++k) rank += sum_u16_first(fine4[k], nf - k * 8);
    {
        const uint32_t lo = cell >= 4 ? mid.x : (mid.x & ((1u << (8 * cell)) - 1u));
        const uint32_t hi = cell > 4 ? (mid.y & ((1u << (8 * (cell - 4))) - 1u)) : 0u;
        rank += __builtin_amdgcn_sad_u8(lo, 0u, 0u) + __builtin_amdgcn_sad_u8(hi, 0u, 0u);
    }
    const uint64_t below = bits_below((int)(key & 63));
    const uint64_t w[4] = {b0.x, b0.y, b1.x, b1.y};
#pragma unroll
    for (int k = 0; k < 4; ++k) rank += (uint32_t)popc64(k < wi ? w[k] : (k == wi ? w[k] & below : 0ull));
    return rank;
}

__device__ __forceinline__ int nth_set_bit(uint64_t m, int k) {
    int pos = 0;
#pragma unroll
    for (int w = 32; w > 0; w >>= 1) {
        const int c = popc64(m & ((1ull << w) - 1ull));
        if (k >= c) { k -= c; m >>= w; pos += w; }
    }
    return pos;
}

template <typename JobRef>
__device__ __forceinline__ void emit_row_ranked(const JobRef &job, const Geom &g, bool whole_map, int64_t key_base1, uint32_t id, uint32_t n_vox,
                                                unsigned long long first_key, const FixSums &fs, long long ic, long long ir, long long is, uint32_t rank) {
    const double tot_q = (double)fs.rho, rc = fix_moment(fs.c_lo, fs.c_hi), rr = fix_moment(fs.r_lo, fs.r_hi), rs = fix_moment(fs.s_lo, fs.s_hi);
    const double tot = tot_q / job.fix_mul;
    const int vi = whole_map ? ((int64_t)first_key >= key_base1 ? 1 : 0) : find_vol_by_key(job.vols, job.n_vols, (int64_t)first_key);
    if (whole_map) job.label_of_comp[id] = job.vol_sign[vi] > 0 ? 1 + (int32_t)rank : -1 - (int32_t)rank;
    const VolDesc vd = job.vols[vi];
    job.r_rank[id] = rank;
    if (rank >= job.blob_cap) return;
    const double n = (double)n_vox;
    double wc[3] = {rc / tot_q, rr / tot_q, rs / tot_q};
    double cc[3] = {(double)ic / n, (double)ir / n, (double)is / n};
    double xyz[3];
    crs2xyz_frac(g, wc, xyz);
    job.b_centroid[3 * rank + 0] = xyz[0];
    job.b_centroid[3 * rank + 1] = xyz[1];
    job.b_centroid[3 * rank + 2] = xyz[2];
    crs2xyz_frac(g, cc, xyz);
    job.b_center[3 * rank + 0] = xyz[0];
    job.b_center[3 * rank + 1] = xyz[1];
    job.b_center[3 * rank + 2] = xyz[2];
    job.b_n[rank] = (int64_t)n_vox;
    job.b_total[rank] = tot;
    job.b_volume[rank] = g.unit_volume * n;
    job.b_key[rank] = (int64_t)first_key - vd.key_base;
    job.b_group[rank] = vd.group;
}
template <typename JobRef>
__device__ __forceinline__ void emit_row(const JobRef &job, const Geom &g, const uint32_t *s_pre, bool whole_map, int64_t key_base1, uint32_t id,
                                         uint32_t n_vox, unsigned long long first_key, const FixSums &fs, long long ic, long long ir, long long is) {
    emit_row_ranked(job, g, whole_map, key_base1, id, n_vox, first_key, fs, ic, ir, is, rank_of_key(job, s_pre, first_key));
}

template <typename JobRef>
__device__ inline void emit_ids(const JobRef &job, const Geom &g, const uint32_t *s_pre, bool whole_map, int64_t key_base1, uint32_t first, uint32_t n_comp,
                                uint32_t block, uint32_t n_blocks) {
    const uint32_t stride = n_blocks * blockDim.x;
    uint32_t i = first + block * blockDim.x + threadIdx.x;
    int32_t par = i < n_comp ? job.parent[i] : -1;
    uint32_t cnt = i < n_comp ? job.r_n[i] : 0u;
    unsigned long long key = i < n_comp ? job.r_key[i] : 0ull;
    for (; i < n_comp; i += stride) {
        const bool root = par == (int32_t)i && cnt != 0u;
        const uint32_t nx = i + stride;
        const int32_t par_next = nx < n_comp ? job.parent[nx] : -1;
        const uint32_t cnt_next = nx < n_comp ? job.r_n[nx] : 0u;
        const unsigned long long key_next = nx < n_comp ? job.r_key[nx] : 0ull;
        if (root) emit_row(job, g, s_pre, whole_map, key_base1, i, cnt, key, fix_load(job, i), job.r_c[i], job.r_r[i], job.r_s[i]);
        par = par_next;
        cnt = cnt_next;
        key = key_next;
    }
}

__global__ void __launch_bounds__(256) k_emit(Job job, const Geom *__restrict__ gp) {
    __shared__ uint32_t s_pre[KEY_GROUPS];
    __shared__ uint32_t s_wave[4];
    const uint32_t total = rank_table_lds(job, s_pre, s_wave);
    emit_ids(job, *gp, s_pre, false, INT64_MAX, 0u, n_components(job), blockIdx.x, gridDim.x);
    if (blockIdx.x == 0 && threadIdx.x == 0) {
        job.ctr->n_blobs = total;
        job.ctr->n_blobs_vol0 = total;
        if (total > job.blob_cap) atomicOr(&job.ctr->overflow, 2u);
    }
}

__global__ void __launch_bounds__(256) k_emit_tiles(Job job, const Geom *__restrict__ gp) {
    __shared__ uint32_t s_pre[KEY_GROUPS];
    __shared__ uint32_t s_wave[4];
    __shared__ unsigned long long s_acc[2][10][TILE_COMPS];
    __shared__ uint32_t s_accn[2][TILE_COMPS];
    const int half = threadIdx.x >> 7, k0 = threadIdx.x & 127;
    const int n_tiles = job.n_tiles;
    int tile = (int)blockIdx.x * 2 + half;
    uint64_t rm[4] = {0ull, 0ull, 0ull, 0ull};
    uint32_t n_in = 0;
    if (tile < n_tiles) {
#pragma unroll
        for (int q = 0; q < 4; ++q) rm[q] = job.root_mask[(size_t)tile * 4 + q];
        n_in = job.inbox_count[(size_t)tile * INBOX_STRIDE];
    }
    const int64_t key_base1 = job.n_vols > 1 ? job.vols[1].key_base : INT64_MAX;
    const uint32_t total = rank_table_lds(job, s_pre, s_wave);
    const Geom &g = *gp;
    for (int t0 = (int)blockIdx.x * 2; t0 < n_tiles; t0 += (int)gridDim.x * 2) {
        tile = t0 + half;
        n_in = min(n_in, (uint32_t)INBOX_CAP);
        const int next = tile + (int)gridDim.x * 2;
        uint64_t nm[4] = {0ull, 0ull, 0ull, 0ull};
        uint32_t n_in_next = 0;
        if (next < n_tiles) {
#pragma unroll
            for (int q = 0; q < 4; ++q) nm[q] = job.root_mask[(size_t)next * 4 + q];
            n_in_next = job.inbox_count[(size_t)next * INBOX_STRIDE];
        }
        InboxEntry e0, e1;
        const bool have0 = (uint32_t)k0 < n_in, have1 = (uint32_t)k0 + 128u < n_in;
        if (have0) e0 = job.inbox[(size_t)tile * INBOX_CAP + k0];
        if (have1) e1 = job.inbox[(size_t)tile * INBOX_CAP + k0 + 128];
        if (n_in != 0u) {
#pragma unroll
            for (int f = 0; f < 10; ++f) { s_acc[half][f][k0] = 0ull; s_acc[half][f][k0 + 128] = 0ull; }
            s_accn[half][k0] = 0u; s_accn[half][k0 + 128] = 0u;
        }
        __syncthreads();
        auto absorb = [&](const InboxEntry &e) {
            const uint32_t l = e.local;
            atomicAdd(&s_accn[half][l], e.n);
            atomicAdd(&s_acc[half][0][l], (unsigned long long)e.sum.rho);
// ... 1308 lines not shown
```

### pdb_eda_amd/csrc/pdbeda_tile.h

```cpp
#pragma once
#include "pdbeda_kernels.h"
#include <type_traits>

namespace pdbeda {

constexpr int TILE_R = 8, TILE_S = 8;
constexpr int RCAP = 1408;
constexpr int RCAP_DENSE = 4096;
constexpr int CCAP = 256;
static_assert(CCAP == TILE_COMPS, "k_emit walks the tiles' component ranges");
constexpr int VCAP = 3584;
constexpr int FACE_K = 7;

struct TileDims {
    int cw;
    int ctiles, rtiles, stiles;
    int n_planes;
    int uc, ur, us, row_words;
    int nc, nr;
    float cut[2];
    int sign[2];
};

__host__ __device__ inline int64_t tile_index(const TileDims &td, int plane, int wq, int r, int s) {
    return (((int64_t)plane * td.stiles + (s >> 3)) * td.rtiles + (r >> 3)) * td.ctiles + wq / td.cw;
}

struct JobInit {
    VolDesc v[2];
    unsigned int runs0, comps0;
};

__device__ inline uint32_t mbcnt_lt(uint64_t mask) {
    return __builtin_amdgcn_mbcnt_hi((uint32_t)(mask >> 32), __builtin_amdgcn_mbcnt_lo((uint32_t)mask, 0u));
}

__device__ inline uint32_t mbcnt_lt_add(uint64_t mask, uint32_t add) {
    return __builtin_amdgcn_mbcnt_hi((uint32_t)(mask >> 32), __builtin_amdgcn_mbcnt_lo((uint32_t)mask, add));
}

__device__ __forceinline__ uint32_t wave_writelane(uint32_t old, uint32_t sval, int sel) {
    asm("v_writelane_b32 %0, %1, %2" : "+v"(old) : "s"(__builtin_amdgcn_readfirstlane((int)sval)), "n"(sel));
    return old;
}

__device__ __forceinline__ void wave_lds_sync() {
    __builtin_amdgcn_fence(__ATOMIC_RELEASE, "wavefront");
    __builtin_amdgcn_wave_barrier();
    __builtin_amdgcn_fence(__ATOMIC_ACQUIRE, "wavefront");
}

__device__ __forceinline__ void lds_barrier() { asm volatile("s_waitcnt lgkmcnt(0)\n\ts_barrier" ::: "memory"); }

template <typename JobRef>
__device__ inline void mark_comps_unused(const JobRef &job, uint32_t cb, uint32_t from, int tid, int nt) {
    unsigned long long *kpar = job.kpar;
    uint32_t *r_n = job.r_n;
    for (uint32_t i = from + tid; i < (uint32_t)CCAP; i += nt) {
        kpar[cb + i] = KP_UNUSED;
        r_n[cb + i] = 0u;
    }
}

typedef const Job __attribute__((address_space(4))) *JobKernarg;
#define PDBEDA_LATE_JOB(name)                                                      \
    JobKernarg name##_p = (JobKernarg)__builtin_amdgcn_kernarg_segment_ptr();      \
    asm volatile("" : "+s"(name##_p));                                             \
    const Job __attribute__((address_space(4))) &name = *name##_p

__device__ __forceinline__ void kernarg_prefetch() {
    JobKernarg ka = (JobKernarg)__builtin_amdgcn_kernarg_segment_ptr();
    uint32_t d0, d1, d2, d3, d4, d5, d6, d7;
    asm volatile("s_load_dword %0, %8, 0x0\n\ts_load_dword %1, %8, 0x40\n\ts_load_dword %2, %8, 0x80\n\ts_load_dword %3, %8, 0xc0\n\t"
                 "s_load_dword %4, %8, 0x100\n\ts_load_dword %5, %8, 0x140\n\ts_load_dword %6, %8, 0x180\n\ts_load_dword %7, %8, 0x1c0\n\t"
                 "s_waitcnt lgkmcnt(0)"
                 : "=&s"(d0), "=&s"(d1), "=&s"(d2), "=&s"(d3), "=&s"(d4), "=&s"(d5), "=&s"(d6), "=&s"(d7) : "s"(ka) : "memory");
}
static_assert(sizeof(Job) + sizeof(TileDims) + 16 > 0x1c0 && sizeof(Job) + sizeof(TileDims) + 16 <= 0x200, "eight 64-byte lines of kernel arguments");

template <int CW, typename JobRef>
__device__ void unit_label_tile(const JobRef &job, const float *__restrict__ dens, const Geom *__restrict__ gp, const TileDims &td,
                                int w0, int r0, int s0, unsigned char *scratch) {
    constexpr int QU = 16 * CW;
    uint64_t *s_m = reinterpret_cast<uint64_t *>(scratch);
    uint32_t *s_off = reinterpret_cast<uint32_t *>(scratch + 512);
    uint32_t *s_base = reinterpret_cast<uint32_t *>(scratch + 768);
    const int tid = threadIdx.x, lane = tid & 63, wv = tid >> 6, n_waves = (int)(blockDim.x >> 6);
    const Geom &g = *gp;
    const int ur = td.ur, us = td.us, row_words = td.row_words;
    const int64_t plane_words = (int64_t)row_words * ur * us;
    for (int q = 0; q < td.n_planes; ++q) {
        const VolDesc vd = job.vols[q];
        for (int quarter = 0; quarter < 4; ++quarter) {
            const int u = quarter * QU + tid;
            const int my_wl = u % CW, my_rowl = (u / CW) & 63;
            const int my_rl = my_rowl & 7, my_sl = my_rowl >> 3;
            const bool my_valid = (tid < QU) && (r0 + my_rl < ur) && (s0 + my_sl < us) && (w0 + my_wl < row_words);
            const int64_t my_word = (int64_t)q * plane_words + ((int64_t)(s0 + my_sl) * ur + (r0 + my_rl)) * row_words + (w0 + my_wl);
            const uint64_t m = my_valid ? job.mask[my_word] : 0ull;
            const uint32_t cnt = (uint32_t)popc64(run_starts(m));
            uint32_t x = (wv == 0) ? cnt : 0u;
#pragma unroll
            for (int d = 1; d < 64; d <<= 1) {
                const uint32_t y = __shfl_up(x, d);
                if (lane >= d) x += y;
            }
            if (tid < 64) { s_m[tid] = (tid < QU) ? m : 0ull; s_off[tid] = x - cnt; }
            if (tid == 63) {
                s_base[0] = x ? atomicAdd(&job.ctr->n_runs, x) : 0u;
                s_base[1] = x ? atomicAdd(&job.ctr->n_comps, x) : 0u;
                s_base[2] = (s_base[0] + x > job.run_cap || s_base[1] + x > job.comp_cap) ? 1u : 0u;
                if (s_base[2]) atomicOr(&job.ctr->overflow, 1u);
            }
            __syncthreads();
            const uint32_t run_first = s_base[0], comp_first = s_base[1];
            const bool no_room = s_base[2] != 0u;
            if (my_valid) job.run_base[my_word] = no_room ? 0u : run_first + s_off[tid];
            for (int j = wv; j < QU && !no_room; j += n_waves) {
                const uint64_t mw = s_m[j];
                if (mw == 0ull) continue;
                const int uu = quarter * QU + j;
                const int wl = uu % CW, rowl = (uu / CW) & 63;
                const int r = r0 + (rowl & 7), s = s0 + (rowl >> 3), c0 = (w0 + wl) * 64;
                const uint32_t run0 = run_first + s_off[j], comp0 = comp_first + s_off[j];
                word_run_records(job, g, dens, vd, mw, lane, c0, r, s, c0, r, s, comp0);
                const uint64_t starts = run_starts(mw);
                if ((starts >> lane) & 1ull) {
                    const uint32_t k = (uint32_t)popc64(starts & bits_below(lane));
                    job.comp_of_run[run0 + k] = comp0 + k;
                }
            }
            __syncthreads();
        }
    }
}

template <int CW>
__global__ void __launch_bounds__(512, 8) k_tile_label(Job job, const float *__restrict__ dens, const Geom *__restrict__ gp, TileDims td, JobInit init) {
    constexpr int NT = 512, NW = 8;
    constexpr int NU = 64 * CW;
    constexpr int USEC = 8 * CW;
    constexpr int CHU = USEC < 16 ? USEC : ((CW == 3) ? 12 : 16);
    constexpr int VREG = VCAP / NW;
    constexpr uint32_t ROOT16 = 0x8000u;
    static_assert(USEC % CHU == 0 && CHU % CW == 0, "chunks are whole rows");
    const int tid = threadIdx.x, lane = tid & 63, wv = tid >> 6;
    const int wvs = __builtin_amdgcn_readfirstlane(wv);
    __shared__ uint64_t s_mask[2][256];
    __shared__ __attribute__((aligned(16))) uint32_t s_pv[RCAP + VCAP];
    static_assert(RCAP_DENSE <= RCAP + VCAP && RCAP_DENSE <= 32768 && RCAP_DENSE <= 64 * 4 * 32, "parent slots of a dense tile; 15-bit component numbers; the tile's own run id range");
    uint32_t *s_parent = s_pv;
    float *s_val = reinterpret_cast<float *>(s_pv + RCAP);
    __shared__ __attribute__((aligned(16))) unsigned char s_blob[CCAP * 48];
    unsigned long long *s_rho = reinterpret_cast<unsigned long long *>(s_blob), *s_rho_c = s_rho + CCAP, *s_rho_r = s_rho + 2 * CCAP, *s_rho_s = s_rho + 3 * CCAP;
    unsigned long long *s_pk = reinterpret_cast<unsigned long long *>(s_rho + 4 * CCAP);
    uint32_t *s_crel = reinterpret_cast<uint32_t *>(s_pk + CCAP), *s_key = s_crel + CCAP;
    __shared__ __attribute__((aligned(16))) uint32_t s_wtot[NW];
    __shared__ uint32_t s_ub[2][256];
    __shared__ uint32_t s_ncomp;
    __shared__ uint64_t s_sg[2][64];
    __shared__ uint16_t s_nb[2][64];
    __shared__ uint32_t s_gtot[2];

    const int uc = td.uc, ur = td.ur, us = td.us;
    const int nc = td.nc, nr = td.nr;
    const int ct = (int)blockIdx.x, rt = (int)blockIdx.y, st = (int)blockIdx.z;
    const uint32_t bid = ((uint32_t)st * (uint32_t)td.rtiles + (uint32_t)rt) * (uint32_t)td.ctiles + (uint32_t)ct;
    const int w0 = ct * CW, r0 = rt * TILE_R, s0 = st * TILE_S;
    const int row_words = (uc + 63) >> 6;
    const int n_planes = td.n_planes;

    {
        PDBEDA_LATE_JOB(pj);
        if (tid == 0) s_ncomp = 0;
        if (bid == 0 && tid == 0) {
            pj.vols[0] = init.v[0];
            if (td.n_planes > 1) pj.vols[1] = init.v[1];
            Counters c;
            memset(&c, 0, sizeof c);
            c.n_runs = init.runs0;
            c.n_comps = init.comps0;
            *pj.ctr = c;
            __hip_atomic_store(&pj.unit_flag[1], pj.epoch, __ATOMIC_RELEASE, __HIP_MEMORY_SCOPE_AGENT);
        }
    }
    for (int i = tid; i < RCAP; i += NT) s_parent[i] = (uint32_t)i;

    const uint64_t t_in = __builtin_amdgcn_s_memrealtime();
    __builtin_amdgcn_s_setprio(3);
    {
        const bool interior = (r0 + TILE_R <= ur) && (s0 + TILE_S <= us) && ((w0 + CW) * 64 <= uc);
        uint32_t vcnt = 0;
        uint32_t rtot = 0;
        const uint32_t vreg = (uint32_t)wvs * VREG;
        const float c0 = td.cut[0], c1 = td.cut[1];
        auto stream = [&](auto interior_tag, auto pos_tag, auto two_tag) {
            constexpr bool INTERIOR = decltype(interior_tag)::value, POS = decltype(pos_tag)::value, TWO = decltype(two_tag)::value;
#pragma unroll 1
            for (int chunk = 0; chunk < USEC / CHU; ++chunk) {
                const int u0 = wvs * USEC + chunk * CHU;
                const int rowl0 = u0 / CW;
                const float *cbase = dens + ((int64_t)(s0 + (rowl0 >> 3)) * nr + (r0 + (rowl0 & 7))) * nc + w0 * 64 + lane;
                float v[CHU];
#pragma unroll
                for (int jj = 0; jj < CHU; ++jj) {
                    const float *ptr = cbase + (int64_t)(jj / CW) * nc + (jj % CW) * 64;
                    if (INTERIOR) {
                        v[jj] = *ptr;
                    } else {
                        const int rowl = rowl0 + jj / CW;
                        const bool in = (r0 + (rowl & 7) < ur) && (s0 + (rowl >> 3) < us) && ((w0 + jj % CW) * 64 + lane < uc);
                        v[jj] = in ? *ptr : 0.0f;
                    }
                }
                uint32_t k0lo = 0, k0hi = 0, k1lo = 0, k1hi = 0;
#pragma unroll
                for (int jj = 0; jj < CHU; ++jj) {
                    const int u = u0 + jj;
                    const int wl = u % CW, rowl = u / CW;
                    const float x = v[jj];
                    bool hit0 = POS ? x >= c0 : x <= c0;
                    bool hit1 = TWO && x <= c1;
                    if (!INTERIOR) {
                        const bool in = (r0 + (rowl & 7) < ur) && (s0 + (rowl >> 3) < us) && ((w0 + wl) * 64 + lane < uc);
                        hit0 = hit0 && in;
                        hit1 = hit1 && in;
                    }
                    const uint64_t b0 = __ballot(hit0);
                    const uint64_t b1 = __ballot(hit1);
                    const uint64_t bb = b0 | b1;
                    const uint32_t nv = (uint32_t)popc64(bb);
                    if (hit0 || hit1) s_val[vreg + min(mbcnt_lt_add(bb, vcnt), (uint32_t)(VREG - 1))] = x;
                    vcnt += nv;
                    k0lo = wave_writelane(k0lo, (uint32_t)b0, jj);
                    k0hi = wave_writelane(k0hi, (uint32_t)(b0 >> 32), jj);
                    k1lo = wave_writelane(k1lo, (uint32_t)b1, jj);
                    k1hi = wave_writelane(k1hi, (uint32_t)(b1 >> 32), jj);
                }
                if (lane < CHU) {
                    const uint64_t k0 = ((uint64_t)k0hi << 32) | k0lo, k1 = ((uint64_t)k1hi << 32) | k1lo;
                    s_mask[0][u0 + lane] = k0;
                    s_mask[1][u0 + lane] = k1;
                    rtot += (uint32_t)popc64(run_starts(k0)) + (uint32_t)popc64(run_starts(k1));
                }
            }
        };
        const bool pos = td.sign[0] > 0;
        if (n_planes > 1) {
            if (interior) stream(std::true_type{}, std::true_type{}, std::true_type{}); else stream(std::false_type{}, std::true_type{}, std::true_type{});
        } else if (interior) {
            if (pos) stream(std::true_type{}, std::true_type{}, std::false_type{}); else stream(std::true_type{}, std::false_type{}, std::false_type{});
        } else {
            if (pos) stream(std::false_type{}, std::true_type{}, std::false_type{}); else stream(std::false_type{}, std::false_type{}, std::false_type{});
        }
        rtot += dpp0<DPP_ROW_SHR + 1>(rtot);
        rtot += dpp0<DPP_ROW_SHR + 2>(rtot);
        rtot += dpp0<DPP_ROW_SHR + 4>(rtot);
        rtot += dpp0<DPP_ROW_SHR + 8>(rtot);
        if (lane == 15) s_wtot[wvs] = rtot | (vcnt > (uint32_t)VREG ? 0x80000000u : 0u);
    }
    __syncthreads();
    {
        const uint32_t dt = (uint32_t)(__builtin_amdgcn_s_memrealtime() - t_in);
        if (dt > 1000u) __builtin_amdgcn_s_setprio(3);
        else if (dt > 850u) __builtin_amdgcn_s_setprio(2);
        else if (dt > 650u) __builtin_amdgcn_s_setprio(1);
        else __builtin_amdgcn_s_setprio(0);
    }

    const int q = lane >> 5, usec = lane & 31;
    const bool act = usec < USEC;
    const int rl = usec / CW, wl = usec % CW;
    const int u = wvs * USEC + (act ? usec : 0);
    uint32_t wbase = 0, n_runs = 0;
    bool from_global = false;
    {
        const uint32_t raw = lane < NW ? s_wtot[lane] : 0u;
        const uint32_t v = (raw & 0x7fffffffu) | ((raw >> 31) << 16);
        uint32_t x = v;
        x += dpp0<DPP_ROW_SHR + 1>(x);
        x += dpp0<DPP_ROW_SHR + 2>(x);
        x += dpp0<DPP_ROW_SHR + 4>(x);
        const uint32_t all = (uint32_t)__builtin_amdgcn_readlane((int)x, NW - 1);
        const uint32_t upto = (uint32_t)__builtin_amdgcn_readlane((int)x, wvs), mine = (uint32_t)__builtin_amdgcn_readlane((int)v, wvs);
        n_runs = all & 0xffffu;
        from_global = (all >> 16) != 0u;
        wbase = (upto - mine) & 0xffffu;
    }
    const uint64_t m = act ? s_mask[q][u] : 0ull, mo = act ? s_mask[q ^ 1][u] : 0ull;
    const bool my_valid = act && q < n_planes && (r0 + rl < ur) && (s0 + wvs < us) && (w0 + wl < row_words);
    const int64_t plane_words = (int64_t)row_words * ur * us;
    const int64_t my_word = (int64_t)q * plane_words + ((int64_t)(s0 + wvs) * ur + (r0 + rl)) * row_words + (w0 + wl);
    const int64_t tile_id = (int64_t)bid;

    if (n_runs > (uint32_t)RCAP && n_runs <= (uint32_t)RCAP_DENSE) {
        from_global = true;
        for (uint32_t i = (uint32_t)RCAP + tid; i < n_runs; i += NT) s_parent[i] = i;
        __syncthreads();
    }
    if (n_runs == 0 || n_runs > (uint32_t)RCAP_DENSE) {
        PDBEDA_LATE_JOB(lj);
        if (my_valid) { lj.mask[my_word] = m; lj.run_base[my_word] = 0u; }
        if (tid == 0) { lj.tile_mode[tile_id] = n_runs ? 1 : 0; lj.tile_runs[bid] = 0u; if (n_runs) { lj.unit_flag[0] = lj.epoch; lj.unit_flag[2] = lj.epoch; } }
        mark_comps_unused(lj, (uint32_t)bid * CCAP, 0u, tid, NT);
        return;
    }

    const uint64_t SA = run_starts(m);
    const uint32_t packed = (uint32_t)popc64(SA) | ((uint32_t)popc64(m | mo) << 22);
    const uint32_t incl = half_scan(packed), excl = incl - packed;
    const uint32_t half0 = (uint32_t)__builtin_amdgcn_readlane((int)incl, 31);
    const uint32_t my_base = wbase + (q ? (half0 & 0x7ffu) : 0u) + (excl & 0x7ffu);
    const uint32_t vb = (uint32_t)wvs * VREG + (excl >> 22);

    const int gq = wvs >> 2, grel = wvs & 3;
    if (gq < n_planes) {
        constexpr int ECAPW = CCAP * 48 / 4 / NW;
        uint32_t *g_edge = reinterpret_cast<uint32_t *>(s_blob) + wvs * ECAPW;
        const int gi = lane / CW, gwl = lane % CW;
        const bool gact = gi < 16;
        const int R = gi & 3, S = (gi >> 2) & 3;
        auto MK = [&](int sec, int row) -> uint64_t { return s_mask[gq][sec * USEC + row * CW + gwl]; };
        const uint64_t a = gact ? MK(2 * S, 2 * R) : 0ull, b = gact ? MK(2 * S, 2 * R + 1) : 0ull;
        const uint64_t c = gact ? MK(2 * S + 1, 2 * R) : 0ull, d = gact ? MK(2 * S + 1, 2 * R + 1) : 0ull;
        const uint64_t G = (a | b) | (c | d);
        const uint64_t SG = run_starts(G);
        const uint32_t gcnt = (uint32_t)popc64(SG);
        const uint32_t gincl = wave_scan(gcnt);
        const uint32_t gtot = (uint32_t)__builtin_amdgcn_readlane((int)gincl, 63);
        const uint32_t nbase = (gq ? n_runs - gtot : 0u) + gincl - gcnt;
        if (grel == 0) {
            s_sg[gq][lane] = SG;
            s_nb[gq][lane] = (uint16_t)nbase;
            if (lane == 0) s_gtot[gq] = gtot;
        }
        const int dR = grel == 1 ? 0 : (grel == 3 ? 1 : -1), dS = grel == 0 ? 0 : -1;
        const int R2 = R + dR, S2 = S + dS;
        const bool has = gact && R2 >= 0 && R2 < 4 && S2 >= 0;
        const int R2c = has ? R2 : R, S2c = has ? S2 : S;
        uint64_t a2 = MK(2 * S2c, 2 * R2c), b2 = MK(2 * S2c, 2 * R2c + 1), c2 = MK(2 * S2c + 1, 2 * R2c), d2 = MK(2 * S2c + 1, 2 * R2c + 1);
        if (!has) { a2 = 0ull; b2 = 0ull; c2 = 0ull; d2 = 0ull; }
        const uint64_t SG2 = run_starts((a2 | b2) | (c2 | d2));
        const uint32_t nbase2 = (uint32_t)__shfl((int)nbase, lane + (dS * 4 + dR) * CW);
        const uint64_t FA = grel == 0 ? (a | c) : (grel == 1 ? (a | b) : (grel == 2 ? a : b));
        const uint64_t FB = grel == 0 ? (b2 | d2) : (grel == 1 ? (c2 | d2) : (grel == 2 ? d2 : c2));
        const uint32_t hbits = (uint32_t)(G >> 63) | ((uint32_t)(FA >> 63) << 1) | ((uint32_t)(FB >> 63) << 2);
        const uint32_t upb = dpp0<DPP_WAVE_SHR1>(hbits);
        const uint32_t car = gwl > 0 ? upb : 0u;
        const uint64_t E = (run_starts(FA) & (FB | (FB << 1) | (uint64_t)((car >> 2) & 1u))) | (run_starts(FB) & ((FA << 1) | (uint64_t)((car >> 1) & 1u)));
        const bool same_row = grel == 3 && (G & 1ull) && (car & 1u);
        const uint32_t ecount = (uint32_t)popc64(E) + (same_row ? 1u : 0u);
        const uint32_t eincl = wave_scan(ecount);
        const uint32_t etot = (uint32_t)__builtin_amdgcn_readlane((int)eincl, 63);
        const uint32_t mb1 = nbase - 1u, bb1 = nbase2 - 1u;
        if (etot <= (uint32_t)ECAPW) {
            uint32_t epos = eincl - ecount;
            if (same_row) g_edge[epos++] = (nbase << 16) | mb1;
            uint64_t todo = E;
            while (todo) {
                const uint64_t below = todo - 1, upto = todo ^ below;
                todo &= below;
                g_edge[epos++] = ((mb1 + (uint32_t)popc64(SG & upto)) << 16) | (bb1 + (uint32_t)popc64(SG2 & upto));
            }
            wave_lds_sync();
            for (uint32_t e = lane; e < etot; e += 64) {
                const uint32_t pk = g_edge[e], x = pk >> 16, y = pk & 0xffffu;
                const uint32_t old = atomicMin(&s_parent[x], y);
                if (old != x) lds_unite(s_parent, old, y);
            }
        } else {
            if (same_row) lds_unite(s_parent, nbase, mb1);
            uint64_t todo = E;
            while (todo) {
                const uint64_t below = todo - 1, upto = todo ^ below;
                todo &= below;
                lds_unite(s_parent, mb1 + (uint32_t)popc64(SG & upto), bb1 + (uint32_t)popc64(SG2 & upto));
            }
        }
    } else if (grel == 0 && lane == 0) {
        s_gtot[1] = 0u;
    }
    __syncthreads();
    for (uint32_t i = tid; i < (uint32_t)CCAP; i += NT) {
        s_rho[i] = 0ull; s_rho_c[i] = 0ull; s_rho_r[i] = 0ull; s_rho_s[i] = 0ull;
        s_pk[i] = 0ull; s_crel[i] = 0u; s_key[i] = 0xffffffffu;
    }
    uint16_t *s_half = reinterpret_cast<uint16_t *>(s_parent);
    const uint32_t n_node0 = s_gtot[0], n_nodes = n_node0 + s_gtot[1], node_skip = n_runs - n_nodes;
    for (uint32_t i = tid; i < n_nodes; i += NT) {
        const uint32_t id = i < n_node0 ? i : i + node_skip;
        if (s_half[2 * id] == id) s_half[2 * id] = (uint16_t)(ROOT16 | atomicAdd(&s_ncomp, 1u));
    }
    {
        const uint32_t dw = (uint32_t)u | ((uint32_t)q << 8);
        uint64_t todo = SA;
        uint32_t id = my_base;
        while (todo) {
            s_half[2 * id + 1] = (uint16_t)(dw | ((uint32_t)ctz64(todo) << 9));
            todo &= todo - 1;
            ++id;
        }
        if (act) s_ub[q][u] = vb | (my_base << 16);
    }
    PDBEDA_LATE_JOB(lj);
    const uint32_t cb = (uint32_t)bid * CCAP, rb = (uint32_t)bid * (uint32_t)(NU * 32);
    {
        if (my_valid) { lj.mask[my_word] = m; lj.run_base[my_word] = rb + my_base; }
    }
    __syncthreads();
    const uint32_t n_comp = s_ncomp;
    const bool wide = n_comp > (uint32_t)CCAP;
    uint32_t gb = cb;
    if (wide) {
        uint32_t *s_gb = s_wtot;
        if (tid == 0) {
            unsigned spins = 0;
            bool ready = true;
            while (__hip_atomic_load(&lj.unit_flag[1], __ATOMIC_ACQUIRE, __HIP_MEMORY_SCOPE_AGENT) != lj.epoch) {
                if (++spins > (1u << 16)) { ready = false; break; }
                __builtin_amdgcn_s_sleep(8);
            }
            uint32_t first = 0xffffffffu;
            if (ready) {
                first = atomicAdd(&lj.ctr->n_comps, n_comp);
                if (first + n_comp > lj.comp_cap) { atomicOr(&lj.ctr->overflow, 1u); first = 0xffffffffu; }
            }
            s_gb[0] = first;
        }
        __syncthreads();
        gb = s_gb[0];
        if (gb == 0xffffffffu) {
            if (my_valid) lj.run_base[my_word] = 0u;
            if (tid == 0) { lj.tile_mode[tile_id] = 3; lj.tile_runs[bid] = 0u; lj.unit_flag[0] = lj.epoch; lj.unit_flag[2] = lj.epoch; }
            mark_comps_unused(lj, cb, 0u, tid, NT);
            return;
        }
    }
    uint32_t *comp_of_run = lj.comp_of_run + rb;
    uint8_t *word_comps = lj.word_comps + (size_t)bid * (2 * 256 * 8);
    const int64_t keys_pp = (int64_t)uc * ur * us;
    for (uint32_t pass0 = 0;; pass0 += (uint32_t)CCAP) {
        {
            const int ctile = w0 * 64;
            const uint32_t urus = (uint32_t)ur * (uint32_t)us;
            const double fix_mul = lj.fix_mul;
            for (uint32_t i = tid; i < n_runs; i += NT) {
                const uint32_t desc = s_half[2 * i + 1];
                const int ru = (int)(desc & 0xffu), rq = (int)((desc >> 8) & 1u), a = (int)(desc >> 9);
                const int rsl = ru / USEC, rrl = (ru % USEC) / CW, rwl = ru % CW;
                const int gl = ((rsl >> 1) * 4 + (rrl >> 1)) * CW + rwl;
                uint32_t x = (uint32_t)s_nb[rq][gl] + (uint32_t)popc64(s_sg[rq][gl] & ((2ull << a) - 1ull)) - 1u;
                do x = s_half[2 * x]; while (!(x & ROOT16));
                const uint32_t comp_all = x & 0x7fffu;
                if (wide && comp_all - pass0 >= (uint32_t)CCAP) continue;
                const uint32_t comp = comp_all - pass0;
                const uint64_t rm = s_mask[rq][ru];
                const uint32_t ub = s_ub[rq][ru];
                const uint64_t inv = ~(rm >> a);
                const int len = inv ? ctz64(inv) : 64;
                double S = 0.0, T = 0.0;
                if (!from_global) {
                    const uint32_t off = (ub & 0xffffu) + (uint32_t)popc64((rm | s_mask[rq ^ 1][ru]) & bits_below(a));
                    int k = 0;
                    for (; k + 2 <= len; k += 2) {
                        const float v0 = s_val[off + k], v1 = s_val[off + k + 1];
                        S += (double)v0; T += S;
                        S += (double)v1; T += S;
                    }
                    if (k < len) { S += (double)s_val[off + k]; T += S; }
                } else {
                    const float *rowptr = dens + ((int64_t)(s0 + rsl) * nr + (r0 + rrl)) * nc + ctile + rwl * 64;
                    for (int k = 0; k < len; ++k) { S += (double)rowptr[a + k]; T += S; }
                }
                const int p0 = rwl * 64 + a;
                const long long F = fix_of(S, fix_mul), Fc = fix_of((double)p0 * S + ((double)len * S - T), fix_mul);
                atomicAdd(&s_rho[comp], (unsigned long long)F);
                atomicAdd(&s_rho_c[comp], (unsigned long long)Fc);
                atomicAdd(&s_rho_r[comp], (unsigned long long)(F * rrl));
                atomicAdd(&s_rho_s[comp], (unsigned long long)(F * rsl));
                atomicMin(&s_key[comp], ((uint32_t)rq << 31) | ((uint32_t)(ctile + p0) * urus + (uint32_t)(r0 + rrl) * (uint32_t)us + (uint32_t)(s0 + rsl)));
                const uint32_t ulen = (uint32_t)len;
                atomicAdd(&s_pk[comp], (unsigned long long)ulen | ((unsigned long long)(ulen * (uint32_t)rrl) << 20) | ((unsigned long long)(ulen * (uint32_t)rsl) << 40));
                atomicAdd(&s_crel[comp], ulen * (uint32_t)p0 + ulen * (ulen - 1u) / 2u);
                comp_of_run[i] = gb + comp_all;
                const uint32_t kw = i - (ub >> 16);
                uint8_t *rec = word_comps + ((desc & 0x1ffu) << 3);
                if (kw < (uint32_t)FACE_K) rec[kw] = (uint8_t)comp;
                if (a + len == 64) rec[7] = (uint8_t)comp;
            }
            if (tid == 0 && pass0 == 0u) {
                lj.tile_mode[tile_id] = wide ? 2 : 0;
                if (wide) *lj.unit_flag = lj.epoch;
            }
        }
        __syncthreads();
        const uint32_t n_here = n_comp - pass0 < (uint32_t)CCAP ? n_comp - pass0 : (uint32_t)CCAP;
        for (uint32_t i = tid; i < n_here; i += NT) {
            const uint32_t g = gb + pass0 + i;
            const unsigned long long pk = s_pk[i];
            const long long n = (long long)(pk & 0xfffffull);
            lj.r_n[g] = (uint32_t)n;
            fix_store(lj, g, fix_sums((long long)s_rho[i], (long long)s_rho_c[i], (long long)s_rho_r[i], (long long)s_rho_s[i], w0 * 64, r0, s0));
            lj.r_c[g] = (long long)s_crel[i] + n * (w0 * 64);
            lj.r_r[g] = (long long)((pk >> 20) & 0xfffffull) + n * r0;
            lj.r_s[g] = (long long)(pk >> 40) + n * s0;
            const uint32_t key = s_key[i];
            lj.r_key[g] = (unsigned long long)((key >> 31) ? keys_pp : 0) + (key & 0x7fffffffu);
            lj.kpar[g] = ((unsigned long long)key << 32) | g;
            if (wide) lj.parent[g] = (int32_t)g;
        }
        if (pass0 + (uint32_t)CCAP >= n_comp) break;
        __syncthreads();
        for (uint32_t i = tid; i < (uint32_t)CCAP; i += NT) {
            s_rho[i] = 0ull; s_rho_c[i] = 0ull; s_rho_r[i] = 0ull; s_rho_s[i] = 0ull;
            s_pk[i] = 0ull; s_crel[i] = 0u; s_key[i] = 0xffffffffu;
        }
        __syncthreads();
    }
    mark_comps_unused(lj, cb, wide ? 0u : n_comp, tid, NT);
    if (tid == 0) lj.tile_runs[bid] = n_runs;
}

struct NbWords {
    uint64_t m[13];
    uint32_t base[13];
};

enum { PAIRS_ALL = 0, PAIRS_WIDE = 1, PAIRS_UNIT = 2 };
template <typename JobRef>
__device__ inline bool load_cross_tile(const JobRef &job, const TileDims &td, int64_t w, uint64_t m, NbWords &nw, uint32_t &my_base, int which = PAIRS_ALL) {
    const int plane = (job.n_vols > 1 && w >= job.vols[1].word_base) ? 1 : 0;
    const VolDesc vd = job.vols[plane];
    const int64_t rem = w - vd.word_base;
    const int wq = (int)(rem % vd.row_words);
    const int64_t row = rem / vd.row_words;
    const int rl = (int)(row % vd.dim[1]);
    const int sl = (int)(row / vd.dim[1]);
    const uint32_t my_mode = job.tile_mode[tile_index(td, 0, wq, rl, sl)];
    const bool in_lds = my_mode == 0u || my_mode == 2u;
    if (which == PAIRS_WIDE && (my_mode & 1u)) return false;
    const bool edge = ((rl & 7) == 0 && rl > 0) || ((sl & 7) == 0 && sl > 0) || ((rl & 7) == 7 && rl + 1 < vd.dim[1] && sl > 0) ||
                      (wq % td.cw == 0 && wq > 0) || (wq % td.cw == td.cw - 1 && wq + 1 < vd.row_words && (rl > 0 || sl > 0));
    if (!edge && in_lds) return false;
    auto wanted = [&](uint32_t nm) {
        if (which == PAIRS_ALL) return true;
        if (which == PAIRS_UNIT) return ((my_mode | nm) & 1u) != 0u;
        return (my_mode == 2u || nm == 2u) && (nm & 1u) == 0u;
    };
    const bool all_nb = which == PAIRS_ALL || (which == PAIRS_UNIT && (my_mode & 1u));
    bool want[13];
    int64_t at[13];
    want[0] = (m & 1ull) && wq > 0 && (!in_lds || (wq % td.cw == 0));
    if (want[0] && !all_nb) want[0] = wanted(job.tile_mode[tile_index(td, 0, wq - 1, rl, sl)]);
    at[0] = w - 1;
#pragma unroll
    for (int nb = 0; nb < 4; ++nb) {
        const int dr = nb == 2 ? 0 : (nb == 3 ? 1 : -1);
        const int ds = nb == 0 ? 0 : -1;
        const int r2 = rl + dr, s2 = sl + ds;
        const bool row_ok = r2 >= 0 && r2 < vd.dim[1] && s2 >= 0;
        const bool row_same_tile = ((r2 >> 3) == (rl >> 3)) && ((s2 >> 3) == (sl >> 3));
        const int64_t rowbase = vd.word_base + ((int64_t)s2 * vd.dim[1] + r2) * vd.row_words;
#pragma unroll
        for (int dw = -1; dw <= 1; ++dw) {
            const int w2 = wq + dw;
            const int i = 1 + nb * 3 + (dw + 1);
            bool ok = row_ok && w2 >= 0 && w2 < vd.row_words;
            if (ok && in_lds && row_same_tile && (w2 / td.cw == wq / td.cw)) ok = false;
            if (dw < 0 && !(m & 1ull)) ok = false;
            if (dw > 0 && !(m >> 63)) ok = false;
            if (ok && !all_nb) ok = wanted(job.tile_mode[tile_index(td, 0, w2, r2, s2)]);
            want[i] = ok;
            at[i] = rowbase + w2;
        }
    }
    bool any = false;
#pragma unroll
    for (int i = 0; i < 13; ++i) {
        const int64_t a = want[i] ? at[i] : w;
        nw.m[i] = job.mask[a];
        nw.base[i] = job.run_base[a];
    }
    my_base = job.run_base[w];
#pragma unroll
    for (int i = 0; i < 13; ++i) {
        if (!want[i]) nw.m[i] = 0ull;
        any = any || nw.m[i] != 0ull;
    }
    return any;
}

template <typename F>
__device__ inline void cross_tile_pairs(uint64_t m, uint32_t my_base, const NbWords &nw, F &&emit) {
    const uint64_t mstarts = run_starts(m);
    const uint64_t dil = m | (m << 1) | (m >> 1);
    if (nw.m[0] >> 63) {
        const uint64_t pm = nw.m[0];
        emit(my_base, nw.base[0] + (uint32_t)popc64(run_starts(pm) & bits_below(run_start_of(pm, 63))));
    }
#pragma unroll
    for (int i = 1; i < 13; ++i) {
        const int dw = (i - 1) % 3 - 1;
        const uint64_t nm = nw.m[i];
        uint64_t hit = dw == 0 ? (nm & dil) : dw < 0 ? (nm & (1ull << 63)) : (nm & 1ull);
        while (hit) {
            const int qb = ctz64(hit);
            const int stb = run_start_of(nm, qb);
            const int enb = run_end_of(nm, stb);
            hit &= ~bits_below(enb + 1);
            const uint32_t other = nw.base[i] + (uint32_t)popc64(run_starts(nm) & bits_below(stb));
            int lo = stb - 1 + 64 * dw, hi = enb + 1 + 64 * dw;
            if (lo < 0) lo = 0;
            if (hi > 63) hi = 63;
            uint64_t mine = m & (bits_below(hi + 1) & ~bits_below(lo));
            while (mine) {
                const int pa = ctz64(mine);
                const int sta = run_start_of(m, pa);
                mine &= ~bits_below(run_end_of(m, sta) + 1);
                emit(my_base + (uint32_t)popc64(mstarts & bits_below(sta)), other);
            }
        }
    }
}

constexpr int PAIR_SLOTS = 1024;
constexpr int FM_THREADS = 384, FM_THREADS_WIDE = 512;
constexpr int FACE_PAIRS = 46;

template <typename JobRef>
__device__ void unit_edges_word(const JobRef &job, const TileDims &td, const VolDesc &v0, int plane, int sl, int r, int wq, int which) {
    const int rw = v0.row_words;
    const int64_t w = (int64_t)plane * rw * v0.dim[1] * v0.dim[2] + ((int64_t)sl * v0.dim[1] + r) * rw + wq;
    const uint64_t m = job.mask[w];
    if (m == 0ull) return;
    NbWords nw;
    uint32_t my_base;
    if (!load_cross_tile(job, td, w, m, nw, my_base, which)) return;
    cross_tile_pairs(m, my_base, nw, [&](uint32_t a, uint32_t b) { kuf_unite(job.kpar, job.comp_of_run[a], job.comp_of_run[b]); });
}

template <int CW, int NTH>
__global__ void __launch_bounds__(NTH, 8) k_face_merge(Job job_arg, const float *__restrict__ dens, const Geom *__restrict__ gp, TileDims td, int pair_slots) {
    kernarg_prefetch();
    PDBEDA_LATE_JOB(lj);
    const bool any_unit = *lj.unit_flag == lj.epoch;
    static_assert(FACE_K == 7, "a word's component record is one 64-bit load: seven runs and the run at the last bit");
    __shared__ unsigned long long s_set[PAIR_SLOTS], s_pairs[PAIR_SLOTS];
    __shared__ uint32_t s_wsum[NTH / 64];
    constexpr int KPH = 128;
    __shared__ kp_t s_kp[5][KPH];
    const int tid = threadIdx.x, lane = tid & 63;
    const int ur = td.ur, us = td.us, row_words = td.row_words;
    const int ct = (int)blockIdx.x, rt = (int)blockIdx.y, st = (int)blockIdx.z;
    const int tile = (st * td.rtiles + rt) * td.ctiles + ct;
    const int w0 = ct * CW;
    const int64_t plane_words = (int64_t)row_words * ur * us;
    const unsigned long long *comps64 = reinterpret_cast<const unsigned long long *>(lj.word_comps);
    auto word_at = [&](int q, int r, int s, int wq) { return (int64_t)q * plane_words + ((int64_t)s * ur + r) * row_words + wq; };
    auto comps_at = [&](uint32_t tl, int q, int r, int s, int wl) { return ((size_t)tl * 2 + q) * 256 + ((s & 7) * TILE_R + (r & 7)) * CW + wl; };
    auto comp_by_run = [&](int64_t w, uint32_t k) { return lj.comp_of_run[lj.run_base[w] + k]; };

    const int fq = tid / (FACE_PAIRS * 4), frem = tid % (FACE_PAIRS * 4), ft = frem >> 2, fwl = frem & 3;
    int rl = 0, sl = 0, dr = 0, ds = -1;
    bool task = tid < 2 * FACE_PAIRS * 4 && fq < td.n_planes && fwl < CW && w0 + fwl < row_words;
    if (ft < 8) { rl = 0; sl = ft; dr = -1; ds = 0; }
    else if (ft < 16) { rl = 0; sl = ft - 8; dr = -1; }
    else if (ft < 23) { rl = ft - 15; sl = 0; dr = -1; }
    else if (ft < 31) { rl = ft - 23; sl = 0; dr = 0; }
    else if (ft < 39) { rl = ft - 31; sl = 0; dr = 1; }
    else { rl = 7; sl = ft - 38; dr = 1; }
    const int r = rt * TILE_R + rl, s = st * TILE_S + sl, r2 = r + dr, s2 = s + ds;
    if (r >= ur || s >= us || r2 < 0 || r2 >= ur || s2 < 0) task = false;
    const uint32_t tile_b = task ? (uint32_t)(((s2 >> 3) * td.rtiles + (r2 >> 3)) * td.ctiles + ct) : 0u;
    const int64_t wA = task ? word_at(fq, r, s, w0 + fwl) : 0, wB = task ? word_at(fq, r2, s2, w0 + fwl) : 0;
    uint64_t mA = 0ull, mB = 0ull;
    unsigned long long cA = 0ull, cB = 0ull;
    uint32_t modes = 0u;
    if (task) {
        mA = lj.mask[wA]; mB = lj.mask[wB];
        cA = comps64[comps_at((uint32_t)tile, fq, r, s, fwl)]; cB = comps64[comps_at(tile_b, fq, r2, s2, fwl)];
        modes = (uint32_t)lj.tile_mode[tile] | (uint32_t)lj.tile_mode[tile_b];
    }
    uint32_t tiles5[5];
    {
        const int drs[5] = {0, -1, -1, 0, 1}, dss[5] = {0, 0, -1, -1, -1};
#pragma unroll
        for (int j = 0; j < 5; ++j) {
            const int r5 = rt + drs[j], s5 = st + dss[j];
            tiles5[j] = (r5 >= 0 && r5 < td.rtiles && s5 >= 0) ? (uint32_t)((s5 * td.rtiles + r5) * td.ctiles + ct) : 0xffffffffu;
        }
    }
    constexpr int KPL = (5 * KPH + NTH - 1) / NTH;
    kp_t kp_pre[KPL];
#pragma unroll
    for (int k = 0; k < KPL; ++k) {
        const int e = tid + k * NTH, j = e / KPH;
        const uint32_t t5 = j == 0 ? tiles5[0] : (j == 1 ? tiles5[1] : (j == 2 ? tiles5[2] : (j == 3 ? tiles5[3] : tiles5[4])));
        kp_pre[k] = (e < 5 * KPH && t5 != 0xffffffffu) ? kuf_load(lj.kpar, t5 * (uint32_t)CCAP + (uint32_t)(e % KPH)) : KP_UNUSED;
    }
    {
        const int64_t key_words = lj.key_words;
        const int64_t lo = (int64_t)lj.clear_bits * tile, hi = lo + lj.clear_bits < key_words ? lo + lj.clear_bits : key_words;
        for (int64_t i = lo + tid; i < hi; i += NTH) lj.key_bits[i] = 0ull;
        const int64_t nfc = lj.n_fine_alloc / 2;
        const int64_t clo = (int64_t)lj.clear_fine * tile, chi = clo + lj.clear_fine < nfc ? clo + lj.clear_fine : nfc;
        for (int64_t i = clo + tid; i < chi; i += NTH) lj.fine_count[i] = 0u;
        const int64_t nmid = (key_words + KEY_FINE - 1) / KEY_FINE * (KEY_FINE / 16);
        const int64_t mlo = (int64_t)lj.clear_mid * tile, mhi = mlo + lj.clear_mid < nmid ? mlo + lj.clear_mid : nmid;
        for (int64_t i = mlo + tid; i < mhi; i += NTH) lj.mid_count[i] = 0u;
        if (tid == 0) lj.inbox_count[(size_t)tile * INBOX_STRIDE] = 0u;
    }
    for (int i = tid; i < pair_slots; i += NTH) s_set[i] = 0ull;
#pragma unroll
    for (int k = 0; k < KPL; ++k) {
        const int e = tid + k * NTH;
        if (e < 5 * KPH) (&s_kp[0][0])[e] = kp_pre[k];
    }
    lds_barrier();
    auto val_of = [&](uint32_t id) -> kp_t {
        const uint32_t t = id / (uint32_t)CCAP;
#pragma unroll
        for (int j = 0; j < 5; ++j)
            if (t == tiles5[j] && (id % (uint32_t)CCAP) < (uint32_t)KPH) return s_kp[j][id % (uint32_t)CCAP];
        return kuf_load(lj.kpar, id);
    };
    const uint32_t slot_mask = (uint32_t)pair_slots - 1u;
    auto add_pair = [&](uint32_t ca, uint32_t cb) {
        const uint32_t lo = ca < cb ? ca : cb, hi = ca < cb ? cb : ca;
        const unsigned long long key = ((unsigned long long)lo << 32) | hi;
        uint32_t h = (uint32_t)((key * 0x9E3779B97F4A7C15ull) >> 40) & slot_mask;
        for (int probe = 0; probe < 8; ++probe, h = (h + 1u) & slot_mask) {
            const unsigned long long old = atomicCAS(&s_set[h], 0ull, key);
            if (old == 0ull || old == key) return;
        }
        kuf_hook_vals(lj.kpar, val_of(lo), val_of(hi));
    };
    {
        if (modes != 0u) { mA = 0ull; mB = 0ull; }
        const uint64_t SA = mA & ~(mA << 1), SB = mB & ~(mB << 1);
        const uint32_t pack = (uint32_t)(mA >> 63) | ((uint32_t)(mB >> 63) << 1) | ((uint32_t)(cA >> 56) << 8) | ((uint32_t)(cB >> 56) << 16);
        uint32_t prev = dpp0<DPP_WAVE_SHR1>(pack);
        if (fwl == 0) prev = 0u;
        const uint64_t carA = prev & 1u, carB = (prev >> 1) & 1u;
        uint64_t todo = (SA & (mB | (mB << 1) | carB)) | (SB & ((mA << 1) | carA));
        const uint32_t baseA = (uint32_t)tile * CCAP, baseB = tile_b * CCAP;
        uint32_t last_a = ~0u, last_b = ~0u;
        while (todo) {
            const int p = ctz64(todo);
            todo &= todo - 1ull;
            const uint64_t upto = (2ull << p) - 1ull;
            const uint32_t ka = (uint32_t)popc64(SA & upto), kb = (uint32_t)popc64(SB & upto);
            uint32_t ca, cb;
            if (ka == 0u) ca = baseA + ((prev >> 8) & 0xffu);
            else ca = ka <= (uint32_t)FACE_K ? baseA + (uint32_t)((cA >> ((ka - 1u) * 8u)) & 0xffull) : comp_by_run(wA, ka - 1u);
            if (kb == 0u) cb = baseB + ((prev >> 16) & 0xffu);
            else cb = kb <= (uint32_t)FACE_K ? baseB + (uint32_t)((cB >> ((kb - 1u) * 8u)) & 0xffull) : comp_by_run(wB, kb - 1u);
            if (ca != last_a || cb != last_b) {
                add_pair(ca, cb);
                last_a = ca; last_b = cb;
            }
        }
    }
    const int cq = (tid - 384) >> 6, crl = lane & 7, csl = lane >> 3;
    const int cr = rt * TILE_R + crl, cs = st * TILE_S + csl;
    const bool ctask = NTH > 384 && tid >= 384 && ct > 0 && cq < td.n_planes && cr < ur && cs < us;
    const uint32_t *mask32 = reinterpret_cast<const uint32_t *>(lj.mask);
    uint32_t m0 = 0u, c0 = 0u, cmodes = 0u, hi9[9], c9[9], mode9[9];
#pragma unroll
    for (int k = 0; k < 9; ++k) { hi9[k] = 0u; c9[k] = 0u; mode9[k] = 0u; }
    auto tile9 = [&](int k) { return (uint32_t)((((cs + k / 3 - 1) >> 3) * td.rtiles + ((cr + k % 3 - 1) >> 3)) * td.ctiles + ct - 1); };
    if (ctask) {
        m0 = mask32[2 * word_at(cq, cr, cs, w0)];
        c0 = lj.word_comps[comps_at((uint32_t)tile, cq, cr, cs, 0) * 8];
        cmodes = lj.tile_mode[tile];
#pragma unroll
        for (int k = 0; k < 9; ++k) {
            const int r9 = cr + k % 3 - 1, s9 = cs + k / 3 - 1;
            if (r9 < 0 || r9 >= ur || s9 < 0 || s9 >= us) continue;
            hi9[k] = mask32[2 * word_at(cq, r9, s9, w0 - 1) + 1];
            c9[k] = lj.word_comps[comps_at(tile9(k), cq, r9, s9, CW - 1) * 8 + 7];
            mode9[k] = lj.tile_mode[tile9(k)];
        }
    }
    if (ctask && (m0 & 1u) && cmodes == 0u) {
        const uint32_t ca = (uint32_t)tile * CCAP + c0;
        uint32_t last_b = ~0u;
#pragma unroll
        for (int k = 0; k < 9; ++k) {
            if (!(hi9[k] >> 31) || mode9[k] != 0u) continue;
            const uint32_t cb = tile9(k) * CCAP + c9[k];
            if (cb != last_b) { add_pair(ca, cb); last_b = cb; }
        }
    }
    lds_barrier();
    {
        constexpr int MAXPER = (PAIR_SLOTS + NTH - 1) / NTH;
        const int per = (pair_slots + NTH - 1) / NTH;
        unsigned long long mine[MAXPER];
        uint32_t cnt = 0;
#pragma unroll
        for (int k = 0; k < MAXPER; ++k) {
            const int slot = tid * per + k;
            mine[k] = (k < per && slot < pair_slots) ? s_set[slot] : 0ull;
            cnt += mine[k] != 0ull ? 1u : 0u;
        }
        const uint32_t x = wave_scan(cnt);
        if (lane == 63) s_wsum[tid >> 6] = x;
        lds_barrier();
        uint32_t at = x - cnt;
        for (int k = 0; k < (tid >> 6); ++k) at += s_wsum[k];
#pragma unroll
        for (int k = 0; k < MAXPER; ++k)
            if (mine[k] != 0ull) s_pairs[at++] = mine[k];
        lds_barrier();
    }
    uint32_t n_pairs = 0;
#pragma unroll
    for (int k = 0; k < NTH / 64; ++k) n_pairs += s_wsum[k];
    for (uint32_t k = tid; k < n_pairs; k += NTH) {
        const unsigned long long key = s_pairs[k];
        kuf_hook_vals(lj.kpar, val_of((uint32_t)(key >> 32)), val_of((uint32_t)key));
    }
    if (any_unit) {
        const VolDesc v0 = lj.vols[0];
        constexpr int NU = 64 * CW;
        for (int k = tid; k < td.n_planes * NU; k += NTH) {
            const int plane = k / NU, u = k % NU, wl = u % CW, rowl = u / CW;
            const int r = rt * TILE_R + (rowl & 7), s = st * TILE_S + (rowl >> 3), wq = w0 + wl;
            if (r < ur && s < us && wq < row_words) unit_edges_word(lj, td, v0, plane, s, r, wq, PAIRS_WIDE);
        }
        if (lj.unit_form == 0 && tid == 0 && lj.unit_flag[2] == lj.epoch) atomicOr(&lj.ctr->overflow, 4u);
    }
}

template <int CW>
__global__ void __launch_bounds__(512) k_unit_label(Job job_arg, const float *__restrict__ dens, const Geom *__restrict__ gp, TileDims td) {
    PDBEDA_LATE_JOB(lj);
    __shared__ __attribute__((aligned(16))) unsigned char s_scratch[1024];
    const int ct = (int)blockIdx.x, rt = (int)blockIdx.y, st = (int)blockIdx.z;
    const int tile = (st * td.rtiles + rt) * td.ctiles + ct;
    if ((lj.tile_mode[tile] & 1) == 0) return;
    unit_label_tile<CW>(lj, dens, gp, td, ct * CW, rt * TILE_R, st * TILE_S, s_scratch);
}
template <int CW>
__global__ void __launch_bounds__(512) k_unit_pairs(Job job_arg, TileDims td) {
    PDBEDA_LATE_JOB(lj);
    const int tid = threadIdx.x;
    const int ct = (int)blockIdx.x, rt = (int)blockIdx.y, st = (int)blockIdx.z;
    if (__hip_atomic_load(&lj.ctr->overflow, __ATOMIC_RELAXED, __HIP_MEMORY_SCOPE_AGENT) != 0u) return;
    const VolDesc v0 = lj.vols[0];
    constexpr int NU = 64 * CW;
    for (int k = tid; k < td.n_planes * NU; k += 512) {
        const int plane = k / NU, u = k % NU, wl = u % CW, rowl = u / CW;
        const int r = rt * TILE_R + (rowl & 7), s = st * TILE_S + (rowl >> 3), wq = ct * CW + wl;
        if (r < td.ur && s < td.us && wq < td.row_words) unit_edges_word(lj, td, v0, plane, s, r, wq, PAIRS_UNIT);
    }
}

constexpr int RSLOTS = 256;
__global__ void __launch_bounds__(256) k_resolve_tiles(Job job, int n_tiles) {
    static_assert(CCAP == 256, "one thread per component id of a tile");
    const int tid = threadIdx.x;
    auto fold = [&](uint32_t root, uint32_t n, const FixSums &sum, unsigned long long c, unsigned long long r, unsigned long long s) {
        atomicAdd(&job.r_n[root], n);
        fix_fold(job, root, sum);
        atomicAdd((unsigned long long *)&job.r_c[root], c);
        atomicAdd((unsigned long long *)&job.r_r[root], r);
        atomicAdd((unsigned long long *)&job.r_s[root], s);
    };
    auto paint = [&](unsigned long long key) { paint_key(job, key); };
    __shared__ int s_root[RSLOTS];
    __shared__ FixSums s_f[RSLOTS];
    __shared__ unsigned long long s_i[3][RSLOTS];
    __shared__ uint32_t s_cnt[RSLOTS];
    auto clear_table = [&]() {
        for (int k = tid; k < RSLOTS; k += 256) {
            s_root[k] = -1;
            s_f[k] = fix_zero();
            s_i[0][k] = 0ull; s_i[1][k] = 0ull; s_i[2][k] = 0ull; s_cnt[k] = 0u;
        }
    };
    auto table_add = [&](int root, uint32_t n, const FixSums &sum, unsigned long long c, unsigned long long r, unsigned long long s) {
        uint32_t h = ((uint32_t)root * 2654435761u) >> 24;
        while (true) {
            const int old = atomicCAS(&s_root[h], -1, root);
            if (old == -1 || old == root) break;
            h = (h + 1u) & (RSLOTS - 1);
        }
        atomicAdd(&s_cnt[h], n);
        fix_atomic_add(&s_f[h], sum);
        atomicAdd(&s_i[0][h], c);
        atomicAdd(&s_i[1][h], r);
        atomicAdd(&s_i[2][h], s);
    };
    if ((int)blockIdx.x >= n_tiles) {
        if (job.ctr->overflow != 0u) return;
        const uint32_t n_comp = n_components(job), stride = (gridDim.x - (uint32_t)n_tiles) * 256u;
        for (uint32_t base = (uint32_t)n_tiles * CCAP + (blockIdx.x - (uint32_t)n_tiles) * 256u; base < n_comp; base += stride) {
            clear_table();
            const uint32_t i = base + tid;
            int root = -1;
            if (i < n_comp) {
                const kp_t rp = kuf_find_from(job.kpar, kuf_load(job.kpar, i));
                if (kp_id(rp) == i) paint(job.r_key[i]);
                else { root = (int)kp_id(rp); job.parent[i] = root; job.kpar[i] = rp; }
            }
            __syncthreads();
            if (root >= 0)
                table_add(root, job.r_n[i], fix_load(job, i), (unsigned long long)job.r_c[i], (unsigned long long)job.r_r[i], (unsigned long long)job.r_s[i]);
            __syncthreads();
            for (int k = tid; k < RSLOTS; k += 256)
                if (s_root[k] >= 0) fold((uint32_t)s_root[k], s_cnt[k], s_f[k], s_i[0][k], s_i[1][k], s_i[2][k]);
            __syncthreads();
        }
        return;
    }
    const uint32_t i = (uint32_t)blockIdx.x * CCAP + tid;
    const kp_t p0 = kuf_load(job.kpar, i);
    uint32_t n_i = 0;
    FixSums v_sum = fix_zero();
    unsigned long long v_c = 0, v_r = 0, v_s = 0, v_key = 0;
    if (tid < 128 || p0 != KP_UNUSED) {
        n_i = job.r_n[i];
        v_sum = fix_load(job, i);
        v_c = (unsigned long long)job.r_c[i]; v_r = (unsigned long long)job.r_r[i]; v_s = (unsigned long long)job.r_s[i]; v_key = job.r_key[i];
    }
    __shared__ int s_any;
    clear_table();
    if (tid == 0) s_any = 0;
    lds_barrier();
    const bool used = n_i > 0u && p0 != KP_UNUSED;
    const bool is_root = used && kp_id(p0) == i;
    const bool member = used && !is_root;
    int root = (int)i;
    if (member) {
        const kp_t rp = kuf_find_from(job.kpar, p0);
        root = (int)kp_id(rp);
        job.kpar[i] = rp;
    }
    job.parent[i] = root;
    {
        const unsigned long long rbits = __ballot(is_root);
        if ((tid & 63) == 0) job.root_mask[(size_t)blockIdx.x * 4 + (tid >> 6)] = rbits;
    }
    if (is_root) paint(v_key);
    if (member) { table_add(root, n_i, v_sum, v_c, v_r, v_s); s_any = 1; }
    lds_barrier();
    if (s_any == 0) return;
    for (int k = tid; k < RSLOTS; k += 256) {
        if (s_root[k] < 0) continue;
        const uint32_t root = (uint32_t)s_root[k], rtile = root / CCAP;
        uint32_t pos = INBOX_CAP;
        if (rtile < (uint32_t)n_tiles) pos = atomicAdd(&job.inbox_count[(size_t)rtile * INBOX_STRIDE], 1u);
        if (pos < (uint32_t)INBOX_CAP) {
            InboxEntry e;
            e.local = root % CCAP; e.n = s_cnt[k];
            e.sum = s_f[k];
            e.c = s_i[0][k]; e.r = s_i[1][k]; e.s = s_i[2][k];
            job.inbox[(size_t)rtile * INBOX_CAP + pos] = e;
        } else {
            fold(root, s_cnt[k], s_f[k], s_i[0][k], s_i[1][k], s_i[2][k]);
        }
    }
}

constexpr int LCAP = 4096;
#ifndef PDBEDA_LABELS_NT_THREADS
#define PDBEDA_LABELS_NT_THREADS 512
#endif
template <int CW, bool FUSED>
__global__ void __launch_bounds__(PDBEDA_LABELS_NT_THREADS, FUSED ? 8 : 1) k_labels_tiles(Job job_arg, TileDims td, int32_t *__restrict__ labels, const Geom *__restrict__ gp) {
    kernarg_prefetch();
    PDBEDA_LATE_JOB(lj);
    constexpr int NU = 64 * CW;
    constexpr int NTL = PDBEDA_LABELS_NT_THREADS, RPW = 64 / (NTL / 64);
    __shared__ int32_t s_lab[CCAP];
    __shared__ __attribute__((aligned(16))) uint2 s_mh[2 * 256];
    __shared__ __attribute__((aligned(16))) uint2 s_sb[2][2 * 256];
    __shared__ __attribute__((aligned(16))) unsigned char s_pc[(LCAP + 8) > 4 * KEY_GROUPS ? (LCAP + 8) : 4 * KEY_GROUPS];
    uint8_t *s_comp8 = s_pc;
    uint32_t *s_pre = reinterpret_cast<uint32_t *>(s_pc);
    __shared__ unsigned long long s_acc[FUSED ? 10 : 1][FUSED ? CCAP : 1];
    __shared__ uint32_t s_accn[FUSED ? CCAP : 1];
    __shared__ uint32_t s_wave[NTL / 64];
    __shared__ uint32_t s_vol0;
    const int tid = threadIdx.x, lane = tid & 63, wv = tid >> 6;
    const int wvs = __builtin_amdgcn_readfirstlane(wv);
    const int uc = td.uc, ur = td.ur, us = td.us, row_words = td.row_words;
    const int ct = (int)blockIdx.x, rt = (int)blockIdx.y, st = (int)blockIdx.z;
    const uint32_t bid = ((uint32_t)st * (uint32_t)td.rtiles + (uint32_t)rt) * (uint32_t)td.ctiles + (uint32_t)ct;
    const int w0 = ct * CW, r0 = rt * TILE_R, s0 = st * TILE_S;
    const int64_t plane_words = (int64_t)row_words * ur * us;
    const uint32_t rb = (uint32_t)bid * (uint32_t)(NU * 32), cb = (uint32_t)bid * CCAP;
    static_assert(NTL == 512 && LCAP == 4096, "two unconditional comp loads per thread cover the first 1024 runs");
    constexpr int CPRE = 2;
    uint32_t c_pre[CPRE];
#pragma unroll
    for (int k = 0; k < CPRE; ++k) c_pre[k] = lj.comp_of_run[rb + tid + NTL * k];
    const uint32_t c_pack = ((c_pre[0] - cb) & 0xffu) | (((c_pre[1] - cb) & 0xffu) << 8);
    int32_t lab_pre = 0;
    int32_t vol0 = 0;
    if (!FUSED) {
        lab_pre = tid < CCAP ? lj.label_of_comp[lj.parent[cb + tid]] : 0;
        vol0 = lj.n_vols > 1 ? (int32_t)lj.ctr->n_blobs_vol0 : 0;
    }
    kp_t kp = KP_UNUSED;
    const int64_t key_base1 = (FUSED && td.n_planes > 1) ? (int64_t)uc * ur * us : INT64_MAX;
    uint32_t n_in = 0;
    const uint32_t jd = cb + (uint32_t)(tid & 255);
    uint32_t rec_n = 0;
    FixSums rec_f = fix_zero();
    long long rec_c = 0, rec_r = 0, rec_s = 0;
    if (FUSED) {
        kp = kuf_load(lj.kpar, jd);
        n_in = lj.inbox_count[(size_t)bid * INBOX_STRIDE];
    }
    auto own_list = [&](int32_t lab) { return lab < 0 ? lab + vol0 : lab; };
    const bool unit = lj.tile_mode[(int64_t)bid] != 0;
    const uint32_t n_runs_raw = lj.tile_runs[bid];
    const uint32_t n_runs = unit ? 0u : n_runs_raw;
    const bool fast = !unit && n_runs <= (uint32_t)LCAP;
    const int pwl = tid % CW, prowl = (tid / CW) & 63;
    const int pr = r0 + (prowl & 7), ps = s0 + (prowl >> 3);
    const bool pvalid = tid < NU && pr < ur && ps < us && w0 + pwl < row_words;
    const int64_t pw = ((int64_t)ps * ur + pr) * row_words + (w0 + pwl);
    uint64_t m[2] = {0ull, 0ull};
    uint32_t base[2] = {0u, 0u};
    if (tid < 256) {
#pragma unroll
        for (int p = 0; p < 2; ++p) {
            const bool has = pvalid && p < td.n_planes;
            m[p] = has ? lj.mask[pw + p * plane_words] : 0ull;
            base[p] = has ? lj.run_base[pw + p * plane_words] : 0u;
        }
    }
    uint32_t total_blobs = 0, blobs_vol0 = 0;
    bool my_root = false;
    auto write_mask_tables = [&]() {
        if (tid < 256) {
            s_mh[2 * tid] = make_uint2((uint32_t)m[0], (uint32_t)m[1]);
            s_mh[2 * tid + 1] = make_uint2((uint32_t)(m[0] >> 32), (uint32_t)(m[1] >> 32));
#pragma unroll
            for (int p = 0; p < 2; ++p) {
                const uint64_t starts = run_starts(m[p]);
                const uint32_t slo = (uint32_t)starts, shi = (uint32_t)(starts >> 32), before = base[p] - rb - 1u;
                s_sb[p][2 * tid] = make_uint2(slo, before);
                s_sb[p][2 * tid + 1] = make_uint2(shi, before + (uint32_t)__popc(slo));
            }
        }
    };
    auto label_of_value = [&](kp_t v) -> int32_t {
        const uint32_t key32 = (uint32_t)(v >> 32);
        const int plane = (int)(key32 >> 31);
        const unsigned long long key = (unsigned long long)(plane ? key_base1 : 0) + (key32 & 0x7fffffffu);
        const int32_t rank = (int32_t)rank_of_key(lj, s_pre, key);
        return lj.vol_sign[plane] > 0 ? 1 + rank : -1 - rank;
    };
    if (FUSED) {
        static_assert(10 * CCAP == 5 * NTL, "five accumulator words per thread");
#pragma unroll
        for (int k = 0; k < 5; ++k) (&s_acc[0][0])[tid + NTL * k] = 0ull;
        if (tid < CCAP) s_accn[tid] = 0u;
        total_blobs = rank_table_lds<NTL>(lj, s_pre, s_wave);
        n_in = min(n_in, (uint32_t)INBOX_CAP);
        write_mask_tables();
        static_assert(INBOX_CAP <= 256, "an inbox entry per thread of the lower half");
        const bool used = kp != KP_UNUSED;
        static_assert(sizeof(InboxEntry) == 88, "eleven words");
        const bool have = (uint32_t)(tid & 255) < n_in;
        const unsigned long long *ew = reinterpret_cast<const unsigned long long *>(lj.inbox + (size_t)bid * INBOX_CAP + (tid & 255));
        my_root = tid >= 256 && used && kp_id(kp) == jd;
        if (tid < 256) {
            unsigned long long e_head = 0ull, e_w[4] = {0ull, 0ull, 0ull, 0ull};
            if (have) {
                e_head = ew[0];
#pragma unroll
                for (int k = 0; k < 4; ++k) e_w[k] = ew[1 + k];
            }
            const bool vol0_lane = tid == 255 && key_base1 != INT64_MAX;
            int32_t raw = 0;
            if (used || vol0_lane) {
                const uint32_t key32 = (uint32_t)(kp >> 32);
                const int plane = used ? (int)(key32 >> 31) : 1;
                const unsigned long long key = (unsigned long long)(plane ? key_base1 : 0) + (used ? (key32 & 0x7fffffffu) : 0u);
                const int32_t rank = (int32_t)rank_of_key(lj, s_pre, key);
                if (used) raw = lj.vol_sign[plane] > 0 ? 1 + rank : -1 - rank;
                else s_vol0 = (uint32_t)rank;
            }
            if (vol0_lane && used) s_vol0 = rank_of_key(lj, s_pre, (unsigned long long)key_base1);
            if (tid == 255 && key_base1 == INT64_MAX) s_vol0 = total_blobs;
            s_lab[tid] = raw;
            if (have) {
                const uint32_t l = (uint32_t)e_head;
                atomicAdd(&s_accn[l], (uint32_t)(e_head >> 32));
#pragma unroll
                for (int k = 0; k < 4; ++k) atomicAdd(&s_acc[k][l], e_w[k]);
            }
        } else {
            unsigned long long e_head = 0ull, e_w[6] = {0ull, 0ull, 0ull, 0ull, 0ull, 0ull};
            if (have) {
                e_head = ew[0];
#pragma unroll
                for (int k = 0; k < 6; ++k) e_w[k] = ew[5 + k];
            }
            if (my_root) {
                rec_n = lj.r_n[jd];
                rec_f = fix_load(lj, jd);
                rec_c = lj.r_c[jd]; rec_r = lj.r_r[jd]; rec_s = lj.r_s[jd];
            }
            if (have) {
                const uint32_t l = (uint32_t)e_head;
#pragma unroll
                for (int k = 0; k < 6; ++k) atomicAdd(&s_acc[4 + k][l], e_w[k]);
            }
        }
        __syncthreads();
        blobs_vol0 = s_vol0;
        vol0 = key_base1 != INT64_MAX ? (int32_t)blobs_vol0 : 0;
    }
    {
        if (!FUSED) write_mask_tables();
        if (tid < CCAP) s_lab[tid] = own_list(FUSED ? s_lab[tid] : lab_pre);
        if (!FUSED || fast) {
#pragma unroll
            for (int k = 0; k < CPRE; ++k) s_comp8[tid + NTL * k] = (uint8_t)(c_pack >> (8 * k));
        }
        if (fast)
            for (uint32_t i = tid + CPRE * NTL; i < n_runs; i += NTL) s_comp8[i] = (uint8_t)(lj.comp_of_run[rb + i] - cb);
    }
    __syncthreads();
    if (FUSED) {
        if (my_root) {
            const int l = tid - 256;
            if (n_in != 0u) {
                rec_n += s_accn[l];
                rec_f.rho += (long long)s_acc[0][l];
                rec_f.c_lo += (long long)s_acc[1][l]; rec_f.c_hi += (long long)s_acc[2][l];
                rec_f.r_lo += (long long)s_acc[3][l]; rec_f.r_hi += (long long)s_acc[4][l];
                rec_f.s_lo += (long long)s_acc[5][l]; rec_f.s_hi += (long long)s_acc[6][l];
                rec_c += (long long)s_acc[7][l]; rec_r += (long long)s_acc[8][l]; rec_s += (long long)s_acc[9][l];
            }
            const uint32_t key32 = (uint32_t)(kp >> 32);
            const unsigned long long key = (unsigned long long)((key32 >> 31) ? key_base1 : 0) + (key32 & 0x7fffffffu);
            const int32_t lab = s_lab[l];
            emit_row_ranked(lj, *gp, true, key_base1, jd, rec_n, key, rec_f, rec_c, rec_r, rec_s, (uint32_t)(lab > 0 ? lab - 1 : vol0 - 1 - lab));
        }
        if (bid == 0 && tid == 0) {
            lj.ctr->n_blobs = total_blobs;
            lj.ctr->n_blobs_vol0 = blobs_vol0;
            if (total_blobs > lj.blob_cap) atomicOr(&lj.ctr->overflow, 2u);
        }
    }
    const int hsel = lane >> 3, sh = (lane & 7) * 4;
    const uint32_t lowm = (1u << sh) - 1u;
    const int c = w0 * 64 + lane * 4;
    const bool inside = (r0 + TILE_R <= ur) && (s0 + TILE_S <= us) && ((w0 + CW) * 64 <= uc) && (uc & 3) == 0;
    const bool ids_ran_out = unit && lj.ctr->overflow != 0u;
    auto label_of_run = [&](uint32_t run) -> int32_t {
        if (ids_ran_out) return 0;
        const uint32_t comp = lj.comp_of_run[run];
        if (FUSED) return own_list(label_of_value(kuf_load(lj.kpar, comp)));
        return own_list(lj.label_of_comp[lj.parent[comp]]);
    };
    auto rows = [&](auto fast_tag, auto inside_tag) {
        constexpr bool FAST = decltype(fast_tag)::value, INSIDE = decltype(inside_tag)::value;
        auto group = [&](int p, unsigned nib, int hidx, int32_t (&o)[4]) {
            const uint2 sb = s_sb[p][hidx];
            const unsigned snib = (sb.x >> sh) & 0xfu;
            const unsigned upto_first = (2u << __builtin_ctz(nib)) - 1u;
            const uint32_t run = sb.y + (uint32_t)__popc(sb.x & lowm) + (uint32_t)__popc(snib & upto_first);
            const unsigned s2 = snib & ~upto_first;
            const unsigned from2 = 0u - (s2 & (0u - s2));
            const unsigned abits = nib & ~from2, bbits = nib & from2;
            int32_t la, lb;
            if (FAST) { la = s_lab[s_comp8[run]]; lb = s_lab[s_comp8[run + 1u]]; }
            else {
                la = label_of_run(run + rb);
                lb = s2 ? label_of_run(run + rb + 1u) : 0;
            }
#pragma unroll
            for (int k = 0; k < 4; ++k)
                o[k] |= (__builtin_amdgcn_sbfe((int)abits, k, 1) & la) | (__builtin_amdgcn_sbfe((int)bbits, k, 1) & lb);
        };
        constexpr int ROW_UNROLL = FAST ? RPW : 1;
#pragma unroll ROW_UNROLL
        for (int rr = 0; rr < RPW; ++rr) {
            const int rowl = wvs * RPW + rr;
            const int r = r0 + (rowl & 7), s = s0 + (rowl >> 3);
            if (!INSIDE && (r >= ur || s >= us)) continue;
            if (hsel >= 2 * CW || (!INSIDE && c >= uc)) continue;
            const int hidx = rowl * (2 * CW) + hsel;
            const uint2 mh = s_mh[hidx];
            const unsigned nib0 = (mh.x >> sh) & 0xfu, nib1 = (mh.y >> sh) & 0xfu;
            int32_t out[4] = {0, 0, 0, 0};
            {
                const bool second = nib0 == 0u;
                const unsigned nib = second ? nib1 : nib0;
                if (nib) group(second ? 1 : 0, nib, hidx, out);
            }
            if (__ballot(nib0 != 0u && nib1 != 0u)) {
                if (nib0 != 0u && nib1 != 0u) group(1, nib1, hidx, out);
            }
            int32_t *dst = labels + ((int64_t)s * ur + r) * uc + c;
            if (INSIDE || (c + 3 < uc && ((uc & 3) == 0))) {
                typedef int v4i __attribute__((ext_vector_type(4)));
                const v4i o4 = {out[0], out[1], out[2], out[3]};
                __builtin_nontemporal_store(o4, reinterpret_cast<v4i *>(dst));
            } else {
#pragma unroll
                for (int q = 0; q < 4; ++q)
                    if (c + q < uc) dst[q] = out[q];
            }
        }
    };
    if (fast) { if (inside) rows(std::true_type{}, std::true_type{}); else rows(std::true_type{}, std::false_type{}); }
    else { if (inside) rows(std::false_type{}, std::true_type{}); else rows(std::false_type{}, std::false_type{}); }
    if (FUSED) {
        const bool any_unit = *lj.unit_flag == lj.epoch;
        if (any_unit) {
            __syncthreads();
            rank_table_lds<NTL>(lj, s_pre, s_wave);
            const uint32_t n_comp = n_components(lj), first = (uint32_t)lj.n_tiles * (uint32_t)TILE_COMPS;
            if (n_comp > first && lj.ctr->overflow == 0u) emit_ids(lj, *gp, s_pre, true, key_base1, first, n_comp, bid, (uint32_t)lj.n_tiles);
        }
    }
}

__global__ void k_labels_decode(const int32_t *__restrict__ signed_labels, int64_t n, int sign, int32_t *__restrict__ out) {
    for (int64_t i = (int64_t)blockIdx.x * blockDim.x + threadIdx.x; i < n; i += (int64_t)gridDim.x * blockDim.x) {
        const int32_t v = signed_labels[i];
        out[i] = sign > 0 ? (v > 0 ? v - 1 : -1) : (v < 0 ? -v - 1 : -1);
    }
}

}
```

Measured before the change: 228,700 Mvoxels/s.

## Maintain blob-key presence tables incrementally during union-find and rank in resolve

Key presence bits and counts are now painted by each component as it is created, and unpainted whenever a root is demoted during union (via a callback threaded through the union-find hooks). Clearing of the key tables moves into the tile-label kernel. The rank table and final labels can then be computed in k_resolve_tiles, which is reordered to run after the group counts, instead of inside the label-writing kernel. The label kernel reads precomputed labels and folds the inbox per wave rather than ranking keys itself. The cost is extra atomic XOR and add traffic on every component creation and demotion, plus an extra rank-table build in the resolve kernel.

```diff
diff --git a/pdb_eda_amd/csrc/pdbeda_hip.hip b/pdb_eda_amd/csrc/pdbeda_hip.hip
--- a/pdb_eda_amd/csrc/pdbeda_hip.hip
+++ b/pdb_eda_amd/csrc/pdbeda_hip.hip
@@ -1134,7 +1134,7 @@
     job.comp_of_run = n_tiles ? cv.take<uint32_t>(max_runs) : nullptr;
     job.label_of_comp = n_tiles ? cv.take<int32_t>(max_comps) : nullptr;
     job.word_comps = n_tiles ? cv.take<uint8_t>((size_t)n_tiles * 2 * 256 * 8) : nullptr;
-    job.unit_done = n_tiles ? cv.take<uint32_t>((size_t)n_tiles) : nullptr;
+    job.wide_ids = n_tiles ? cv.take<uint32_t>((size_t)n_tiles * 2) : nullptr;
     job.unit_flag = n_tiles ? cv.take<uint32_t>(4) : nullptr;
     job.tile_mode = n_tiles ? cv.take<uint8_t>(n_tiles) : nullptr;
     job.tile_runs = n_tiles ? cv.take<uint32_t>(n_tiles) : nullptr;
@@ -1314,8 +1314,8 @@
         case 3: launch_tile_label<3>(ctx, (unsigned)tiles_pp, job, m->dens, m->geom_dev, td, init, pair_slots); break;
         default: launch_tile_label<4>(ctx, (unsigned)tiles_pp, job, m->dens, m->geom_dev, td, init, pair_slots); break;
     }
-    { PROF(ctx, "k_resolve_tiles"); hipLaunchKernelGGL(k_resolve_tiles, dim3((unsigned)tiles_pp + 64u), dim3(256), 0, st, job, (int)tiles_pp); }
     if (job.group_count) { PROF(ctx, "k_group_counts"); hipLaunchKernelGGL(k_group_counts, dim3((unsigned)(job.n_groups + 255) / 256u), dim3(256), 0, st, job); }
+    { PROF(ctx, "k_resolve_tiles"); hipLaunchKernelGGL(k_resolve_tiles, dim3((unsigned)tiles_pp + 64u), dim3(256), 0, st, job, (int)tiles_pp, (long long)(n_planes > 1 ? keys_pp : INT64_MAX)); }
     if (labels) {
         PROF(ctx, "k_labels_tiles");
         launch_labels<true>(ctx, job, td, labels_dev, m->geom_dev);
diff --git a/pdb_eda_amd/csrc/pdbeda_kernels.h b/pdb_eda_amd/csrc/pdbeda_kernels.h
--- a/pdb_eda_amd/csrc/pdbeda_kernels.h
+++ b/pdb_eda_amd/csrc/pdbeda_kernels.h
@@ -91,7 +91,7 @@
     uint32_t *comp_of_run;
     int32_t *label_of_comp;
     uint8_t *word_comps;
-    uint32_t *unit_done;
+    uint32_t *wide_ids;
     uint32_t *unit_flag;
     uint32_t epoch;
     uint8_t *tile_mode;
@@ -429,7 +429,8 @@
     }
     return x;
 }
-__device__ inline void kuf_unite_vals(kp_t *p, kp_t a, kp_t b) {
+template <typename F>
+__device__ inline void kuf_unite_vals(kp_t *p, kp_t a, kp_t b, F &&demoted) {
     while (true) {
         kp_t qa = kuf_load(p, kp_id(a)), qb = kuf_load(p, kp_id(b));
         while (qa != a || qb != b) {
@@ -442,23 +443,26 @@
         if (a == b) return;
         if (a < b) { const kp_t t = a; a = b; b = t; }
         const kp_t old = atomicMin(p + kp_id(a), b);
-        if (old == a) return;
+        if (old == a) { demoted(a); return; }
         a = old;
     }
 }
-__device__ inline void kuf_hook_vals(kp_t *p, kp_t a, kp_t b) {
+template <typename F>
+__device__ inline void kuf_hook_vals(kp_t *p, kp_t a, kp_t b, F &&demoted) {
 #pragma unroll
     for (int level = 0; level < 4; ++level) {
         if (a == b) return;
         if (a < b) { const kp_t t = a; a = b; b = t; }
         const kp_t old = atomicMin(p + kp_id(a), b);
-        if (old == a || old == b) return;
+        if (old == a) { demoted(a); return; }
+        if (old == b) return;
         a = old;
     }
-    kuf_unite_vals(p, a, b);
-}
-__device__ inline void kuf_unite(kp_t *p, uint32_t ia, uint32_t ib) {
-    kuf_unite_vals(p, kuf_load(p, ia), kuf_load(p, ib));
+    kuf_unite_vals(p, a, b, demoted);
+}
+template <typename F>
+__device__ inline void kuf_unite(kp_t *p, uint32_t ia, uint32_t ib, F &&demoted) {
+    kuf_unite_vals(p, kuf_load(p, ia), kuf_load(p, ib), demoted);
 }
 
 __device__ inline uint32_t run_of_bit(uint64_t nm, uint32_t base, int p, int *start_out) {
@@ -607,6 +611,20 @@
     atomicOr((unsigned long long *)&job.key_bits[key >> 6], 1ull << (key & 63));
     atomicAdd(&job.mid_count[cell >> 2], 1u << ((cell & 3u) * 8u));
     atomicAdd(&job.fine_count[f >> 1], 1u << ((f & 1u) * 16u));
+}
+
+template <typename JobRef>
+__device__ __forceinline__ void flip_key(const JobRef &job, unsigned long long key, bool on) {
+    const uint32_t f = (uint32_t)((key >> 6) / KEY_FINE);
+    const uint32_t cell = (uint32_t)(key >> 8);
+    const uint32_t mu = 1u << ((cell & 3u) * 8u), fu = 1u << ((f & 1u) * 16u);
+    atomicXor((unsigned long long *)&job.key_bits[key >> 6], 1ull << (key & 63));
+    atomicAdd(&job.mid_count[cell >> 2], on ? mu : 0u - mu);
+    atomicAdd(&job.fine_count[f >> 1], on ? fu : 0u - fu);
+}
+__device__ __forceinline__ unsigned long long key_of_value(unsigned long long v, long long key_base1) {
+    const uint32_t key32 = (uint32_t)(v >> 32);
+    return (unsigned long long)((key32 >> 31) ? key_base1 : 0) + (key32 & 0x7fffffffu);
 }
 
 __global__ void __launch_bounds__(256) k_paint_keys(Job job) {
diff --git a/pdb_eda_amd/csrc/pdbeda_tile.h b/pdb_eda_amd/csrc/pdbeda_tile.h
--- a/pdb_eda_amd/csrc/pdbeda_tile.h
+++ b/pdb_eda_amd/csrc/pdbeda_tile.h
@@ -77,6 +77,19 @@
                  : "=&s"(d0), "=&s"(d1), "=&s"(d2), "=&s"(d3), "=&s"(d4), "=&s"(d5), "=&s"(d6), "=&s"(d7) : "s"(ka) : "memory");
 }
 static_assert(sizeof(Job) + sizeof(TileDims) + 16 > 0x1c0 && sizeof(Job) + sizeof(TileDims) + 16 <= 0x200, "eight 64-byte lines of kernel arguments");
+
+template <typename JobRef>
+__device__ inline void clear_key_tables(const JobRef &job, uint32_t tile, int tid, int nt) {
+    const int64_t key_words = job.key_words;
+    const int64_t lo = (int64_t)job.clear_bits * tile, hi = lo + job.clear_bits < key_words ? lo + job.clear_bits : key_words;
+    for (int64_t i = lo + tid; i < hi; i += nt) job.key_bits[i] = 0ull;
+    const int64_t nfc = job.n_fine_alloc / 2;
+    const int64_t clo = (int64_t)job.clear_fine * tile, chi = clo + job.clear_fine < nfc ? clo + job.clear_fine : nfc;
+    for (int64_t i = clo + tid; i < chi; i += nt) job.fine_count[i] = 0u;
+    const int64_t nmid = (key_words + KEY_FINE - 1) / KEY_FINE * (KEY_FINE / 16);
+    const int64_t mlo = (int64_t)job.clear_mid * tile, mhi = mlo + job.clear_mid < nmid ? mlo + job.clear_mid : nmid;
+    for (int64_t i = mlo + tid; i < mhi; i += nt) job.mid_count[i] = 0u;
+}
 
 template <int CW, typename JobRef>
 __device__ void unit_label_tile(const JobRef &job, const float *__restrict__ dens, const Geom *__restrict__ gp, const TileDims &td,
@@ -128,6 +141,7 @@
                 if ((starts >> lane) & 1ull) {
                     const uint32_t k = (uint32_t)popc64(starts & bits_below(lane));
                     job.comp_of_run[run0 + k] = comp0 + k;
+                    flip_key(job, (unsigned long long)(vd.key_base + ((int64_t)(c0 + lane) * vd.dim[1] + r) * vd.dim[2] + s), true);
                 }
             }
             __syncthreads();
@@ -303,6 +317,7 @@
         if (my_valid) { lj.mask[my_word] = m; lj.run_base[my_word] = 0u; }
         if (tid == 0) { lj.tile_mode[tile_id] = n_runs ? 1 : 0; lj.tile_runs[bid] = 0u; if (n_runs) { lj.unit_flag[0] = lj.epoch; lj.unit_flag[2] = lj.epoch; } }
         mark_comps_unused(lj, (uint32_t)bid * CCAP, 0u, tid, NT);
+        clear_key_tables(lj, bid, tid, NT);
         return;
     }
 
@@ -433,8 +448,10 @@
             if (my_valid) lj.run_base[my_word] = 0u;
             if (tid == 0) { lj.tile_mode[tile_id] = 3; lj.tile_runs[bid] = 0u; lj.unit_flag[0] = lj.epoch; lj.unit_flag[2] = lj.epoch; }
             mark_comps_unused(lj, cb, 0u, tid, NT);
+            clear_key_tables(lj, bid, tid, NT);
             return;
         }
+        if (tid == 0) { lj.wide_ids[2 * bid] = gb; lj.wide_ids[2 * bid + 1] = n_comp; }
     }
     uint32_t *comp_of_run = lj.comp_of_run + rb;
     uint8_t *word_comps = lj.word_comps + (size_t)bid * (2 * 256 * 8);
@@ -519,6 +536,7 @@
     }
     mark_comps_unused(lj, cb, wide ? 0u : n_comp, tid, NT);
     if (tid == 0) lj.tile_runs[bid] = n_runs;
+    clear_key_tables(lj, bid, tid, NT);
 }
 
 struct NbWords {
@@ -627,8 +645,8 @@
 constexpr int FM_THREADS = 384, FM_THREADS_WIDE = 512;
 constexpr int FACE_PAIRS = 46;
 
-template <typename JobRef>
-__device__ void unit_edges_word(const JobRef &job, const TileDims &td, const VolDesc &v0, int plane, int sl, int r, int wq, int which) {
+template <typename JobRef, typename F>
+__device__ void unit_edges_word(const JobRef &job, const TileDims &td, const VolDesc &v0, int plane, int sl, int r, int wq, int which, F &&demoted) {
     const int rw = v0.row_words;
     const int64_t w = (int64_t)plane * rw * v0.dim[1] * v0.dim[2] + ((int64_t)sl * v0.dim[1] + r) * rw + wq;
     const uint64_t m = job.mask[w];
@@ -636,7 +654,7 @@
     NbWords nw;
     uint32_t my_base;
     if (!load_cross_tile(job, td, w, m, nw, my_base, which)) return;
-    cross_tile_pairs(m, my_base, nw, [&](uint32_t a, uint32_t b) { kuf_unite(job.kpar, job.comp_of_run[a], job.comp_of_run[b]); });
+    cross_tile_pairs(m, my_base, nw, [&](uint32_t a, uint32_t b) { kuf_unite(job.kpar, job.comp_of_run[a], job.comp_of_run[b], demoted); });
 }
 
 template <int CW, int NTH>
@@ -698,24 +716,20 @@
         const uint32_t t5 = j == 0 ? tiles5[0] : (j == 1 ? tiles5[1] : (j == 2 ? tiles5[2] : (j == 3 ? tiles5[3] : tiles5[4])));
         kp_pre[k] = (e < 5 * KPH && t5 != 0xffffffffu) ? kuf_load(lj.kpar, t5 * (uint32_t)CCAP + (uint32_t)(e % KPH)) : KP_UNUSED;
     }
-    {
-        const int64_t key_words = lj.key_words;
-        const int64_t lo = (int64_t)lj.clear_bits * tile, hi = lo + lj.clear_bits < key_words ? lo + lj.clear_bits : key_words;
-        for (int64_t i = lo + tid; i < hi; i += NTH) lj.key_bits[i] = 0ull;
-        const int64_t nfc = lj.n_fine_alloc / 2;
-        const int64_t clo = (int64_t)lj.clear_fine * tile, chi = clo + lj.clear_fine < nfc ? clo + lj.clear_fine : nfc;
-        for (int64_t i = clo + tid; i < chi; i += NTH) lj.fine_count[i] = 0u;
-        const int64_t nmid = (key_words + KEY_FINE - 1) / KEY_FINE * (KEY_FINE / 16);
-        const int64_t mlo = (int64_t)lj.clear_mid * tile, mhi = mlo + lj.clear_mid < nmid ? mlo + lj.clear_mid : nmid;
-        for (int64_t i = mlo + tid; i < mhi; i += NTH) lj.mid_count[i] = 0u;
-        if (tid == 0) lj.inbox_count[(size_t)tile * INBOX_STRIDE] = 0u;
-    }
+    static_assert(NTH >= CCAP, "a thread per component id of the tile");
+    kp_t own_kp = KP_UNUSED;
+    unsigned long long own_key = 0ull;
+    if (tid < CCAP) { own_kp = kuf_load(lj.kpar, (uint32_t)tile * (uint32_t)CCAP + (uint32_t)tid); own_key = lj.r_key[(size_t)tile * CCAP + tid]; }
+    if (tid == 0) lj.inbox_count[(size_t)tile * INBOX_STRIDE] = 0u;
+    const long long key_base1 = td.n_planes > 1 ? (long long)td.uc * ur * us : INT64_MAX;
+    auto unpaint = [&](kp_t v) { flip_key(lj, key_of_value(v, key_base1), false); };
     for (int i = tid; i < pair_slots; i += NTH) s_set[i] = 0ull;
 #pragma unroll
     for (int k = 0; k < KPL; ++k) {
         const int e = tid + k * NTH;
         if (e < 5 * KPH) (&s_kp[0][0])[e] = kp_pre[k];
     }
+    if (own_kp != KP_UNUSED) flip_key(lj, own_key, true);
     lds_barrier();
     auto val_of = [&](uint32_t id) -> kp_t {
         const uint32_t t = id / (uint32_t)CCAP;
@@ -733,7 +747,7 @@
             const unsigned long long old = atomicCAS(&s_set[h], 0ull, key);
             if (old == 0ull || old == key) return;
         }
-        kuf_hook_vals(lj.kpar, val_of(lo), val_of(hi));
+        kuf_hook_vals(lj.kpar, val_of(lo), val_of(hi), unpaint);
     };
     {
         if (modes != 0u) { mA = 0ull; mB = 0ull; }
@@ -819,15 +833,19 @@
     for (int k = 0; k < NTH / 64; ++k) n_pairs += s_wsum[k];
     for (uint32_t k = tid; k < n_pairs; k += NTH) {
         const unsigned long long key = s_pairs[k];
-        kuf_hook_vals(lj.kpar, val_of((uint32_t)(key >> 32)), val_of((uint32_t)key));
+        kuf_hook_vals(lj.kpar, val_of((uint32_t)(key >> 32)), val_of((uint32_t)key), unpaint);
     }
     if (any_unit) {
         const VolDesc v0 = lj.vols[0];
+        if (lj.tile_mode[tile] == 2) {
+            const uint32_t first = lj.wide_ids[2 * tile], count = lj.wide_ids[2 * tile + 1];
+            for (uint32_t k = tid; k < count; k += NTH) flip_key(lj, lj.r_key[first + k], true);
+        }
         constexpr int NU = 64 * CW;
         for (int k = tid; k < td.n_planes * NU; k += NTH) {
             const int plane = k / NU, u = k % NU, wl = u % CW, rowl = u / CW;
             const int r = rt * TILE_R + (rowl & 7), s = st * TILE_S + (rowl >> 3), wq = w0 + wl;
-            if (r < ur && s < us && wq < row_words) unit_edges_word(lj, td, v0, plane, s, r, wq, PAIRS_WIDE);
+            if (r < ur && s < us && wq < row_words) unit_edges_word(lj, td, v0, plane, s, r, wq, PAIRS_WIDE, unpaint);
         }
         if (lj.unit_form == 0 && tid == 0 && lj.unit_flag[2] == lj.epoch) atomicOr(&lj.ctr->overflow, 4u);
     }
@@ -849,18 +867,26 @@
     const int ct = (int)blockIdx.x, rt = (int)blockIdx.y, st = (int)blockIdx.z;
     if (__hip_atomic_load(&lj.ctr->overflow, __ATOMIC_RELAXED, __HIP_MEMORY_SCOPE_AGENT) != 0u) return;
     const VolDesc v0 = lj.vols[0];
+    const long long key_base1 = td.n_planes > 1 ? (long long)td.uc * td.ur * td.us : INT64_MAX;
+    auto unpaint = [&](kp_t v) { flip_key(lj, key_of_value(v, key_base1), false); };
     constexpr int NU = 64 * CW;
     for (int k = tid; k < td.n_planes * NU; k += 512) {
         const int plane = k / NU, u = k % NU, wl = u % CW, rowl = u / CW;
         const int r = rt * TILE_R + (rowl & 7), s = st * TILE_S + (rowl >> 3), wq = ct * CW + wl;
-        if (r < td.ur && s < td.us && wq < td.row_words) unit_edges_word(lj, td, v0, plane, s, r, wq, PAIRS_UNIT);
+        if (r < td.ur && s < td.us && wq < td.row_words) unit_edges_word(lj, td, v0, plane, s, r, wq, PAIRS_UNIT, unpaint);
     }
 }
 
 constexpr int RSLOTS = 256;
-__global__ void __launch_bounds__(256) k_resolve_tiles(Job job, int n_tiles) {
+__global__ void __launch_bounds__(256) k_resolve_tiles(Job job, int n_tiles, long long key_base1 ) {
     static_assert(CCAP == 256, "one thread per component id of a tile");
     const int tid = threadIdx.x;
+    __shared__ uint32_t s_pre[KEY_GROUPS];
+    __shared__ uint32_t s_wave[4];
+    auto label_of_value = [&](kp_t v) -> int32_t {
+        const int32_t rank = (int32_t)rank_of_key(job, s_pre, key_of_value(v, key_base1));
+        return job.vol_sign[(int)(v >> 63)] > 0 ? 1 + rank : -1 - rank;
+    };
     auto fold = [&](uint32_t root, uint32_t n, const FixSums &sum, unsigned long long c, unsigned long long r, unsigned long long s) {
         atomicAdd(&job.r_n[root], n);
         fix_fold(job, root, sum);
@@ -868,7 +894,6 @@
         atomicAdd((unsigned long long *)&job.r_r[root], r);
         atomicAdd((unsigned long long *)&job.r_s[root], s);
     };
-    auto paint = [&](unsigned long long key) { paint_key(job, key); };
     __shared__ int s_root[RSLOTS];
     __shared__ FixSums s_f[RSLOTS];
     __shared__ unsigned long long s_i[3][RSLOTS];
@@ -896,14 +921,16 @@
     if ((int)blockIdx.x >= n_tiles) {
         if (job.ctr->overflow != 0u) return;
         const uint32_t n_comp = n_components(job), stride = (gridDim.x - (uint32_t)n_tiles) * 256u;
-        for (uint32_t base = (uint32_t)n_tiles * CCAP + (blockIdx.x - (uint32_t)n_tiles) * 256u; base < n_comp; base += stride) {
+        const uint32_t base0 = (uint32_t)n_tiles * CCAP + (blockIdx.x - (uint32_t)n_tiles) * 256u;
+        if (base0 < n_comp) rank_table_lds(job, s_pre, s_wave);
+        for (uint32_t base = base0; base < n_comp; base += stride) {
             clear_table();
             const uint32_t i = base + tid;
             int root = -1;
             if (i < n_comp) {
                 const kp_t rp = kuf_find_from(job.kpar, kuf_load(job.kpar, i));
-                if (kp_id(rp) == i) paint(job.r_key[i]);
-                else { root = (int)kp_id(rp); job.parent[i] = root; job.kpar[i] = rp; }
+                if (kp_id(rp) != i) { root = (int)kp_id(rp); job.parent[i] = root; job.kpar[i] = rp; }
+                job.label_of_comp[i] = label_of_value(rp);
             }
             __syncthreads();
             if (root >= 0)
@@ -917,33 +944,42 @@
     }
     const uint32_t i = (uint32_t)blockIdx.x * CCAP + tid;
     const kp_t p0 = kuf_load(job.kpar, i);
+    RankTableLoads<256> rt;
+    rank_table_issue<256>(job, rt);
     uint32_t n_i = 0;
     FixSums v_sum = fix_zero();
-    unsigned long long v_c = 0, v_r = 0, v_s = 0, v_key = 0;
+    unsigned long long v_c = 0, v_r = 0, v_s = 0;
     if (tid < 128 || p0 != KP_UNUSED) {
         n_i = job.r_n[i];
         v_sum = fix_load(job, i);
-        v_c = (unsigned long long)job.r_c[i]; v_r = (unsigned long long)job.r_r[i]; v_s = (unsigned long long)job.r_s[i]; v_key = job.r_key[i];
+        v_c = (unsigned long long)job.r_c[i]; v_r = (unsigned long long)job.r_r[i]; v_s = (unsigned long long)job.r_s[i];
     }
     __shared__ int s_any;
     clear_table();
     if (tid == 0) s_any = 0;
-    lds_barrier();
+    const uint32_t total_blobs = rank_table_finish<256>(rt, s_pre, s_wave);
+    if (blockIdx.x == 0 && tid == 255) {
+        const uint32_t below1 = key_base1 != INT64_MAX ? rank_of_key(job, s_pre, (unsigned long long)key_base1) : total_blobs;
+        job.ctr->n_blobs = total_blobs;
+        job.ctr->n_blobs_vol0 = below1;
+        if (total_blobs > job.blob_cap) atomicOr(&job.ctr->overflow, 2u);
+    }
     const bool used = n_i > 0u && p0 != KP_UNUSED;
     const bool is_root = used && kp_id(p0) == i;
     const bool member = used && !is_root;
     int root = (int)i;
+    kp_t rp = p0;
     if (member) {
-        const kp_t rp = kuf_find_from(job.kpar, p0);
+        rp = kuf_find_from(job.kpar, p0);
         root = (int)kp_id(rp);
         job.kpar[i] = rp;
     }
     job.parent[i] = root;
+    job.label_of_comp[i] = used ? label_of_value(rp) : 0;
     {
         const unsigned long long rbits = __ballot(is_root);
         if ((tid & 63) == 0) job.root_mask[(size_t)blockIdx.x * 4 + (tid >> 6)] = rbits;
     }
-    if (is_root) paint(v_key);
     if (member) { table_add(root, n_i, v_sum, v_c, v_r, v_s); s_any = 1; }
     lds_barrier();
     if (s_any == 0) return;
@@ -983,7 +1019,6 @@
     __shared__ unsigned long long s_acc[FUSED ? 10 : 1][FUSED ? CCAP : 1];
     __shared__ uint32_t s_accn[FUSED ? CCAP : 1];
     __shared__ uint32_t s_wave[NTL / 64];
-    __shared__ uint32_t s_vol0;
     const int tid = threadIdx.x, lane = tid & 63, wv = tid >> 6;
     const int wvs = __builtin_amdgcn_readfirstlane(wv);
     const int uc = td.uc, ur = td.ur, us = td.us, row_words = td.row_words;
@@ -999,19 +1034,13 @@
     for (int k = 0; k < CPRE; ++k) c_pre[k] = lj.comp_of_run[rb + tid + NTL * k];
     const uint32_t c_pack = ((c_pre[0] - cb) & 0xffu) | (((c_pre[1] - cb) & 0xffu) << 8);
     int32_t lab_pre = 0;
-    int32_t vol0 = 0;
-    if (!FUSED) {
-        lab_pre = tid < CCAP ? lj.label_of_comp[lj.parent[cb + tid]] : 0;
-        vol0 = lj.n_vols > 1 ? (int32_t)lj.ctr->n_blobs_vol0 : 0;
-    }
+    if (tid < CCAP) lab_pre = FUSED ? lj.label_of_comp[cb + tid] : lj.label_of_comp[lj.parent[cb + tid]];
+    const int32_t vol0 = lj.n_vols > 1 ? (int32_t)lj.ctr->n_blobs_vol0 : 0;
     kp_t kp = KP_UNUSED;
     const int64_t key_base1 = (FUSED && td.n_planes > 1) ? (int64_t)uc * ur * us : INT64_MAX;
     uint32_t n_in = 0;
     const uint32_t jd = cb + (uint32_t)(tid & 255);
-    uint32_t rec_n = 0;
-    FixSums rec_f = fix_zero();
-    long long rec_c = 0, rec_r = 0, rec_s = 0;
-    if (FUSED) {
+    if (FUSED && tid >= 256) {
         kp = kuf_load(lj.kpar, jd);
         n_in = lj.inbox_count[(size_t)bid * INBOX_STRIDE];
     }
@@ -1034,8 +1063,6 @@
             base[p] = has ? lj.run_base[pw + p * plane_words] : 0u;
         }
     }
-    uint32_t total_blobs = 0, blobs_vol0 = 0;
-    bool my_root = false;
     auto write_mask_tables = [&]() {
         if (tid < 256) {
             s_mh[2 * tid] = make_uint2((uint32_t)m[0], (uint32_t)m[1]);
@@ -1049,89 +1076,53 @@
             }
         }
     };
-    auto label_of_value = [&](kp_t v) -> int32_t {
-        const uint32_t key32 = (uint32_t)(v >> 32);
-        const int plane = (int)(key32 >> 31);
-        const unsigned long long key = (unsigned long long)(plane ? key_base1 : 0) + (key32 & 0x7fffffffu);
-        const int32_t rank = (int32_t)rank_of_key(lj, s_pre, key);
-        return lj.vol_sign[plane] > 0 ? 1 + rank : -1 - rank;
-    };
-    if (FUSED) {
-        static_assert(10 * CCAP == 5 * NTL, "five accumulator words per thread");
-#pragma unroll
-        for (int k = 0; k < 5; ++k) (&s_acc[0][0])[tid + NTL * k] = 0ull;
-        if (tid < CCAP) s_accn[tid] = 0u;
-        total_blobs = rank_table_lds<NTL>(lj, s_pre, s_wave);
-        n_in = min(n_in, (uint32_t)INBOX_CAP);
+    if (FUSED && tid >= 256) {
+        const int l = tid - 256;
+#pragma unroll
+        for (int k = 0; k < 10; ++k) s_acc[k][l] = 0ull;
+        s_accn[l] = 0u;
+    }
+    {
         write_mask_tables();
-        static_assert(INBOX_CAP <= 256, "an inbox entry per thread of the lower half");
-        const bool used = kp != KP_UNUSED;
-        static_assert(sizeof(InboxEntry) == 88, "eleven words");
-        const bool have = (uint32_t)(tid & 255) < n_in;
-        const unsigned long long *ew = reinterpret_cast<const unsigned long long *>(lj.inbox + (size_t)bid * INBOX_CAP + (tid & 255));
-        my_root = tid >= 256 && used && kp_id(kp) == jd;
-        if (tid < 256) {
-            unsigned long long e_head = 0ull, e_w[4] = {0ull, 0ull, 0ull, 0ull};
-            if (have) {
-                e_head = ew[0];
-#pragma unroll
-                for (int k = 0; k < 4; ++k) e_w[k] = ew[1 + k];
-            }
-            const bool vol0_lane = tid == 255 && key_base1 != INT64_MAX;
-            int32_t raw = 0;
-            if (used || vol0_lane) {
-                const uint32_t key32 = (uint32_t)(kp >> 32);
-                const int plane = used ? (int)(key32 >> 31) : 1;
-                const unsigned long long key = (unsigned long long)(plane ? key_base1 : 0) + (used ? (key32 & 0x7fffffffu) : 0u);
-                const int32_t rank = (int32_t)rank_of_key(lj, s_pre, key);
-                if (used) raw = lj.vol_sign[plane] > 0 ? 1 + rank : -1 - rank;
-                else s_vol0 = (uint32_t)rank;
-            }
-            if (vol0_lane && used) s_vol0 = rank_of_key(lj, s_pre, (unsigned long long)key_base1);
-            if (tid == 255 && key_base1 == INT64_MAX) s_vol0 = total_blobs;
-            s_lab[tid] = raw;
-            if (have) {
-                const uint32_t l = (uint32_t)e_head;
-                atomicAdd(&s_accn[l], (uint32_t)(e_head >> 32));
-#pragma unroll
-                for (int k = 0; k < 4; ++k) atomicAdd(&s_acc[k][l], e_w[k]);
-            }
-        } else {
-            unsigned long long e_head = 0ull, e_w[6] = {0ull, 0ull, 0ull, 0ull, 0ull, 0ull};
-            if (have) {
-                e_head = ew[0];
-#pragma unroll
-                for (int k = 0; k < 6; ++k) e_w[k] = ew[5 + k];
-            }
-            if (my_root) {
-                rec_n = lj.r_n[jd];
-                rec_f = fix_load(lj, jd);
-                rec_c = lj.r_c[jd]; rec_r = lj.r_r[jd]; rec_s = lj.r_s[jd];
-            }
-            if (have) {
-                const uint32_t l = (uint32_t)e_head;
-#pragma unroll
-                for (int k = 0; k < 6; ++k) atomicAdd(&s_acc[4 + k][l], e_w[k]);
-            }
-        }
-        __syncthreads();
-        blobs_vol0 = s_vol0;
-        vol0 = key_base1 != INT64_MAX ? (int32_t)blobs_vol0 : 0;
-    }
-    {
-        if (!FUSED) write_mask_tables();
-        if (tid < CCAP) s_lab[tid] = own_list(FUSED ? s_lab[tid] : lab_pre);
-        if (!FUSED || fast) {
-#pragma unroll
-            for (int k = 0; k < CPRE; ++k) s_comp8[tid + NTL * k] = (uint8_t)(c_pack >> (8 * k));
-        }
+        if (tid < CCAP) s_lab[tid] = own_list(lab_pre);
+#pragma unroll
+        for (int k = 0; k < CPRE; ++k) s_comp8[tid + NTL * k] = (uint8_t)(c_pack >> (8 * k));
         if (fast)
             for (uint32_t i = tid + CPRE * NTL; i < n_runs; i += NTL) s_comp8[i] = (uint8_t)(lj.comp_of_run[rb + i] - cb);
     }
     __syncthreads();
-    if (FUSED) {
+    if (FUSED && tid >= 256) {
+        const bool my_root = kp != KP_UNUSED && kp_id(kp) == jd;
+        const int l = tid - 256;
+        uint32_t rec_n = 0;
+        FixSums rec_f = fix_zero();
+        long long rec_c = 0, rec_r = 0, rec_s = 0;
         if (my_root) {
-            const int l = tid - 256;
+            rec_n = lj.r_n[jd];
+            rec_f = fix_load(lj, jd);
+            rec_c = lj.r_c[jd]; rec_r = lj.r_r[jd]; rec_s = lj.r_s[jd];
+        }
+        n_in = min(n_in, (uint32_t)INBOX_CAP);
+        static_assert(sizeof(InboxEntry) == 88, "eleven words");
+        const uint32_t own_lo = (uint32_t)(wvs - 4) * 64u;
+#pragma unroll 1
+        for (uint32_t e0 = 0; e0 < n_in; e0 += 64u) {
+            const uint32_t e = e0 + (uint32_t)lane;
+            if (e < n_in) {
+                const unsigned long long *ew = reinterpret_cast<const unsigned long long *>(lj.inbox + (size_t)bid * INBOX_CAP + e);
+                unsigned long long e_w[11];
+#pragma unroll
+                for (int k = 0; k < 11; ++k) e_w[k] = ew[k];
+                const uint32_t el = (uint32_t)e_w[0];
+                if (el - own_lo < 64u) {
+                    atomicAdd(&s_accn[el], (uint32_t)(e_w[0] >> 32));
+#pragma unroll
+                    for (int k = 0; k < 10; ++k) atomicAdd(&s_acc[k][el], e_w[1 + k]);
+                }
+            }
+        }
+        wave_lds_sync();
+        if (my_root) {
             if (n_in != 0u) {
                 rec_n += s_accn[l];
                 rec_f.rho += (long long)s_acc[0][l];
@@ -1140,15 +1131,8 @@
                 rec_f.s_lo += (long long)s_acc[5][l]; rec_f.s_hi += (long long)s_acc[6][l];
                 rec_c += (long long)s_acc[7][l]; rec_r += (long long)s_acc[8][l]; rec_s += (long long)s_acc[9][l];
             }
-            const uint32_t key32 = (uint32_t)(kp >> 32);
-            const unsigned long long key = (unsigned long long)((key32 >> 31) ? key_base1 : 0) + (key32 & 0x7fffffffu);
             const int32_t lab = s_lab[l];
-            emit_row_ranked(lj, *gp, true, key_base1, jd, rec_n, key, rec_f, rec_c, rec_r, rec_s, (uint32_t)(lab > 0 ? lab - 1 : vol0 - 1 - lab));
-        }
-        if (bid == 0 && tid == 0) {
-            lj.ctr->n_blobs = total_blobs;
-            lj.ctr->n_blobs_vol0 = blobs_vol0;
-            if (total_blobs > lj.blob_cap) atomicOr(&lj.ctr->overflow, 2u);
+            emit_row_ranked(lj, *gp, true, key_base1, jd, rec_n, key_of_value(kp, key_base1), rec_f, rec_c, rec_r, rec_s, (uint32_t)(lab > 0 ? lab - 1 : vol0 - 1 - lab));
         }
     }
     const int hsel = lane >> 3, sh = (lane & 7) * 4;
@@ -1159,7 +1143,7 @@
     auto label_of_run = [&](uint32_t run) -> int32_t {
         if (ids_ran_out) return 0;
         const uint32_t comp = lj.comp_of_run[run];
-        if (FUSED) return own_list(label_of_value(kuf_load(lj.kpar, comp)));
+        if (FUSED) return own_list(lj.label_of_comp[comp]);
         return own_list(lj.label_of_comp[lj.parent[comp]]);
     };
     auto rows = [&](auto fast_tag, auto inside_tag) {
```

Measured after the change: 190,900 Mvoxels/s. 0.835x the previous value.
